# waicool20/BoofCV

Measured on AMD Instinct MI355X. Metric: 1080p frames/sec detect+describe+associate, higher is better.
Workload: dtype f32 detect / f64 describe / associate: fp16 MFMA candidate filter + exact fp64 re-score; 1 GPU; batch of 256 1920x1080 GrayF32 per GPU: Fast-Hessian detect + SURF-64 (stable) describe + greedy L2 associate with the next frame; batch_per_gpu=256, width=1920, height=1080, ranks_seen=1

## Files before the change

boofcv_amd/build.py:

```python
import glob
import os
import subprocess
import sys

HERE = os.path.dirname(os.path.abspath(__file__))
CSRC = os.path.join(HERE, "csrc")
LIB = os.path.join(HERE, "libboofhip.so")
LIB_EXPERIMENTS = os.path.join(HERE, "libboofhip_exp.so")
ARCH = "gfx950"

FLAGS = ["-O3", "-std=c++17", "-fPIC", "-ffp-contract=off", "-fhip-fp32-correctly-rounded-divide-sqrt", "-fno-fast-math",
         "-Wall", "-Wno-unused-function", "-Wno-unused-result"]


def sources():
    return sorted(glob.glob(os.path.join(CSRC, "*.hip"))) + sorted(glob.glob(os.path.join(CSRC, "*.cpp")))


def common_deps():
    return glob.glob(os.path.join(CSRC, "*.h")) + [os.path.join(HERE, "..", "include", "boofhip.h"), os.path.abspath(__file__)]


def needs_build(lib=LIB):
    if not os.path.exists(lib):
        return True
    t = os.path.getmtime(lib)
    return any(os.path.getmtime(d) > t for d in sources() + common_deps())


def build(force=False, verbose=False, experiments=False):
    lib = LIB_EXPERIMENTS if experiments else LIB
    extra = []
    if experiments and os.environ.get("BHIP_EXP_DEFS"):
        extra = os.environ["BHIP_EXP_DEFS"].split()
        lib = os.path.join(HERE, "libboofhip_exp_%s.so" % os.environ.get("BHIP_EXP_TAG", "variant"))
        force = True
    if not force and not needs_build(lib):
        return lib
    hipcc = os.environ.get("HIPCC", "/opt/rocm/bin/hipcc")
    objs = []
    objdir = os.path.join(HERE, ("build_exp_" + os.environ.get("BHIP_EXP_TAG", "variant")) if extra else "build_exp" if experiments else "build")
    os.makedirs(objdir, exist_ok=True)
    procs = []
    newest = max(os.path.getmtime(d) for d in common_deps())
    for src in sources():
        obj = os.path.join(objdir, os.path.basename(src) + ".o")
        objs.append(obj)
        if not force and os.path.exists(obj) and os.path.getmtime(obj) > max(newest, os.path.getmtime(src)):
            continue
        cmd = [hipcc, "--offload-arch=" + ARCH] + FLAGS + (["-DBHIP_EXPERIMENTS"] if experiments else []) + extra + ["-c", src, "-o", obj]
        if src.endswith(".cpp"):
            cmd.insert(1, "-x")
            cmd.insert(2, "hip")
        if verbose:
            print(" ".join(cmd), file=sys.stderr)
        procs.append((src, subprocess.Popen(cmd, stdout=subprocess.PIPE, stderr=subprocess.STDOUT)))
    for src, p in procs:
        out, _ = p.communicate()
        if p.returncode != 0:
            raise RuntimeError("hipcc failed on %s:\n%s" % (src, out.decode(errors="replace")))
        if verbose and out:
            print(out.decode(errors="replace"), file=sys.stderr)
    cmd = [hipcc, "--offload-arch=" + ARCH, "-shared", "-fPIC", "-o", lib] + objs
    subprocess.check_call(cmd)
    return lib


if __name__ == "__main__":
    print(build(force="--force" in sys.argv, verbose=True, experiments="--experiments" in sys.argv))
```

boofcv_amd/csrc/cabi.h:

```cpp
#pragma once
#include "common.h"
#include <cmath>
#include <cfloat>
#include <algorithm>
#include <atomic>
#include <memory>
#include <mutex>
#include <unordered_map>
#include <unordered_set>

#pragma GCC visibility push(hidden)

struct CtxScratch {
	DevBuf in0, in1, out0, out1, tmp0, tmp1;
	DevBuf work, assocCol, nmsBitmap, nmsPrefix, nmsPos, ipTmp, ipKernel, fast, disparity, distortMap, templ, flow, threshold;
	long long flowPixels = 0;
	DevBuf thresholdTaps;
	int thresholdTapsRadius = 0;
	AssocMfmaWork mfma;
	int assocExactOnly = -1;
};
inline CtxScratch* scratchOf(bhip_ctx* ctx);

struct bhip_ctx_full : bhip_ctx {
	CtxScratch scratch;
};
inline CtxScratch* scratchOf(bhip_ctx* ctx) { return &static_cast<bhip_ctx_full*>(ctx)->scratch; }

using OrphanFn = void (*)(void* child, bhip_ctx* ctx);
struct HandleRegistry {
	std::mutex m;
	std::unordered_set<bhip_ctx*> ctxs;
	std::unordered_map<void*, OrphanFn> children;
	std::atomic<bool> exiting{false};
};
HandleRegistry& registry();

template <class Dev>
struct CtxChild : Dev {
	using Device = Dev;
	bhip_ctx* ctx = nullptr;
	void onRelease() {}
};
template <class X>
void releaseDevice(X* x) {
	if (!x->ctx) return;
	(void)hipSetDevice(x->ctx->device);
	(void)hipStreamSynchronize(x->ctx->stream);
	x->onRelease();
	static_cast<typename X::Device&>(*x) = typename X::Device();
	x->ctx = nullptr;
}
template <class X>
void orphanIfOn(void* child, bhip_ctx* ctx) {
	if (static_cast<X*>(child)->ctx == ctx) releaseDevice(static_cast<X*>(child));
}
template <class X, class Build>
int createChild(bhip_ctx* ctx, X** out, Build build) {
	HandleRegistry& R = registry();
	std::lock_guard<std::mutex> lock(R.m);
	if (!ctx || !R.ctxs.count(ctx)) return BHIP_ERR_INVALID;
	std::unique_ptr<X> x;
	BHIP_TRY(build(x));
	R.children.emplace(x.get(), &orphanIfOn<X>);
	*out = x.release();
	return BHIP_OK;
}
template <class X>
int destroyChild(X* x) {
	if (!x) return BHIP_OK;
	HandleRegistry& R = registry();
	std::lock_guard<std::mutex> lock(R.m);
	if (R.exiting) return BHIP_OK;
	auto it = R.children.find(x);
	if (it == R.children.end() || it->second != &orphanIfOn<X>) return BHIP_ERR_INVALID;
	R.children.erase(it);
	releaseDevice(x);
	delete x;
	return BHIP_OK;
}

#define CHECK_CTX(ctx)                                   \
	do {                                                 \
		if (!(ctx)) return BHIP_ERR_INVALID;             \
		BHIP_HIP((ctx), hipSetDevice((ctx)->device));    \
	} while (0)

template <class T>
struct HostImg {
	T* data;
	int start, stride, width, height;
	static constexpr int batch = 1;
};

#define CHECK_IMG(ctx, v)                                                                                         \
	do {                                                                                                          \
		if (!(v).data || (v).width <= 0 || (v).height <= 0 || (v).batch <= 0 || (v).stride < (v).width)          \
			return bhip_fail((ctx), BHIP_ERR_INVALID, "bad image");                                               \
	} while (0)

template <class T>
int upload(bhip_ctx* ctx, T* dev, int pitch, const T* in, int start, int stride, int w, int h, hipStream_t st) {
	if (pitch == w && stride == w) BHIP_HIP(ctx, hipMemcpyAsync(dev, in + start, sizeof(T) * w * h, hipMemcpyHostToDevice, st));
	else BHIP_HIP(ctx, hipMemcpy2DAsync(dev, sizeof(T) * pitch, in + start, sizeof(T) * stride, sizeof(T) * w, h, hipMemcpyHostToDevice, st));
	return BHIP_OK;
}
template <class T>
int download(bhip_ctx* ctx, T* out, int start, int stride, const T* dev, int pitch, int w, int h, hipStream_t st) {
	if (pitch == w && stride == w) BHIP_HIP(ctx, hipMemcpyAsync(out + start, dev, sizeof(T) * w * h, hipMemcpyDeviceToHost, st));
	else BHIP_HIP(ctx, hipMemcpy2DAsync(out + start, sizeof(T) * stride, dev, sizeof(T) * pitch, sizeof(T) * w, h, hipMemcpyDeviceToHost, st));
	return BHIP_OK;
}

template <class T>
int stageIn(bhip_ctx* ctx, DevBuf& slot, HostImg<T> h, int pitch, DevImg<std::remove_const_t<T>>& dev, bool copy = true) {
	using E = std::remove_const_t<T>;
	BHIP_TRY(slot.reserve(ctx, (size_t)pitch * h.height * sizeof(E)));
	dev = bhip_img_over<E>(slot, pitch, h.width, h.height, 1);
	return copy ? upload<E>(ctx, dev.data, pitch, h.data, h.start, h.stride, h.width, h.height, ctx->stream) : BHIP_OK;
}
template <class T>
int stageOut(bhip_ctx* ctx, HostImg<T> h, DevImg<T> dev) {
	return download<T>(ctx, h.data, h.start, h.stride, dev.data, dev.stride, h.width, h.height, ctx->stream);
}
inline int pitch4(int w) { return (w + 3) & ~3; }

template <class TI, class TO, class Run>
int hostInOut(bhip_ctx* ctx, HostImg<const TI> in, HostImg<TO> out, bool pitched, bool keepOut, const char* argError, Run run) {
	CHECK_CTX(ctx);
	CHECK_IMG(ctx, in);
	CHECK_IMG(ctx, out);
	if (argError) return bhip_fail(ctx, BHIP_ERR_INVALID, argError);
	CtxScratch* sc = scratchOf(ctx);
	DevImg<TI> din;
	DevImg<TO> dout;
	BHIP_TRY(stageIn(ctx, sc->in0, in, pitched ? pitch4(in.width) : in.width, din));
	BHIP_TRY(stageIn(ctx, sc->out0, out, pitched ? pitch4(out.width) : out.width, dout, keepOut));
	BHIP_TRY(run(din, dout));
	BHIP_TRY(stageOut(ctx, out, dout));
	return bhip_ctx_synchronize(ctx);
}

int nonmaxDevice(bhip_ctx* ctx, DevImg<const float> img, int radius, float threshold, int border, int16_t* dev_xy, int cap, int* dev_n,
				 bool minimum = false);
template <class T>
int cornerImpl(bhip_ctx* ctx, bool weighted, int kind, int radius, float kappa, DevImg<const T> dx, DevImg<const T> dy, DevImg<float> intensity);
template <class T> struct PyrTraits;
template <> struct PyrTraits<float> {
	using Kernel = float;
	static constexpr bool fusedLayer = true;
	static constexpr bool clearLayer0 = true;
	static constexpr const char* copyTag = "pyramid_copy";
	static constexpr double copyBytes = 8.0;
};
template <> struct PyrTraits<uint8_t> {
	using Kernel = int32_t;
	static constexpr bool fusedLayer = false;
	static constexpr bool clearLayer0 = false;
	static constexpr const char* copyTag = "pyramid_copy_u8";
	static constexpr double copyBytes = 2.0;
};
template <class T>
int pyramidImpl(bhip_ctx* ctx, const typename PyrTraits<T>::Kernel* kernel, int kw, const int* scales, int n, DevImg<const T> in, T* out,
				bool layer0Present = false);
bool briefPatchOk(const int32_t* samplePoints, int nSamples, int radius);
int gaussianImpl(bhip_ctx* ctx, double sigma, int radius, DevImg<const float> in, DevImg<float> out);

#pragma GCC visibility pop
```

boofcv_amd/csrc/cabi.hip:

```cpp
#include "cabi.h"

HandleRegistry& registry() {
	static HandleRegistry* r = [] {
		HandleRegistry* p = new HandleRegistry();
		atexit([] { registry().exiting = true; });
		return p;
	}();
	return *r;
}

static int ctxCreate(int device, void* stream, bool useGiven, bhip_ctx** out) {
	if (!out) return BHIP_ERR_INVALID;
	*out = nullptr;
	int count = 0;
	if (hipGetDeviceCount(&count) != hipSuccess || count <= 0) return BHIP_ERR_HIP;
	if (device < 0 || device >= count) return BHIP_ERR_INVALID;
	if (hipSetDevice(device) != hipSuccess) return BHIP_ERR_HIP;
	std::unique_ptr<bhip_ctx_full> ctx(new (std::nothrow) bhip_ctx_full());
	if (!ctx) return BHIP_ERR_NOMEM;
	ctx->device = device;
	if (useGiven) {
		ctx->stream = (hipStream_t)stream;
	} else {
		if (hipStreamCreateWithFlags(&ctx->ownedStream.h, hipStreamNonBlocking) != hipSuccess) return BHIP_ERR_HIP;
		ctx->stream = ctx->ownedStream;
	}
	if (ctx->hostScratch.reserve(ctx.get(), 1 << 20) != BHIP_OK) return BHIP_ERR_HIP;
	HandleRegistry& R = registry();
	std::lock_guard<std::mutex> lock(R.m);
	R.ctxs.insert(ctx.get());
	*out = ctx.release();
	return BHIP_OK;
}

struct FhLevelPlan {
	DetectLevelParams p;
	int level;
};
struct FhOctavePlan {
	int skip, w, h, nlevels;
	int sizes[BHIP_MAX_LEVELS];
	std::vector<FhLevelPlan> mids;
	bool fused = false, fixed = false;
	int shareFrom[BHIP_MAX_LEVELS];
	bool onDemand[BHIP_MAX_LEVELS];
	int exportSlot[BHIP_MAX_LEVELS];
	int nexport = 0;
	size_t intenOff = 0, expOff = 0;
	long long intenImageStride = 0, expImageStride = 0;
};

struct FhDetector {
	bhip_fh_cfg cfg;
	int W = 0, H = 0, batch = 0, cap = 0;
	bool plannedInt = false;
	std::vector<FhOctavePlan> plan;
	int bitmapWords = 0;
	DevBuf inten, bitmap, prefix, cand, sorted, count, selKey, selIdx, selLevels;
	bool nBest() const { return cfg.maxFeaturesPerScale > 0; }
	std::vector<int> counts;
	long long total = 0;

	static bool unfusedOnly() { return bhip_env_flag("BHIP_DETECT_UNFUSED"); }
	int makePlan(bhip_ctx* ctx, int width, int height) {
		plan.clear();
		if (cfg.numberScalesPerOctave > BHIP_MAX_LEVELS || cfg.numberScalesPerOctave < 1) return bhip_fail(ctx, BHIP_ERR_UNSUPPORTED, "numberScalesPerOctave out of range");
		if (cfg.extractRadius < 1) return bhip_fail(ctx, BHIP_ERR_INVALID, "Search radius must be >= 1");
		if (cfg.initialSampleSize < 1 || cfg.initialSize < 3) return bhip_fail(ctx, BHIP_ERR_INVALID, "bad sample size / initial size");
		if (width >= 32768 || height >= 32768) return bhip_fail(ctx, BHIP_ERR_UNSUPPORTED, "image too large for Point2D_I16");
		int skip = cfg.initialSampleSize, sizeStep = cfg.scaleStepSize, octaveSize = cfg.initialSize;
		unsigned int bits = 0;
		const int step = cfg.extractRadius + 1;
		for (int octave = 0; octave < cfg.numberOfOctaves; octave++) {
			FhOctavePlan o;
			o.nlevels = cfg.numberScalesPerOctave;
			for (int i = 0; i < o.nlevels; i++) o.sizes[i] = octaveSize + i * sizeStep;
			const int maxSize = o.sizes[o.nlevels - 1];
			if (maxSize > width || maxSize > height) break;
			o.skip = skip;
			o.w = width / skip;
			o.h = height / skip;
			for (int i = 2; i < o.nlevels; i++) {
				FhLevelPlan m;
				m.level = i - 1;
				DetectLevelParams& p = m.p;
				p.skip = skip; p.w = o.w; p.h = o.h;
				p.sizeLower = o.sizes[m.level - 1]; p.sizeMid = o.sizes[m.level]; p.sizeUpper = o.sizes[m.level + 1];
				p.border = p.sizeMid / (2 * skip);
				const int rw = p.w - 2 * p.border, rh = p.h - 2 * p.border;
				p.nbx = rw > 0 ? (rw + step - 1) / step : 0;
				p.nby = rh > 0 ? (rh + step - 1) / step : 0;
				p.bitBase = bits;
				bits += (unsigned)p.nbx * (unsigned)p.nby;
				o.mids.push_back(m);
			}
			plan.push_back(o);
			skip += skip;
			octaveSize += sizeStep;
			sizeStep += sizeStep;
		}
		bitmapWords = (int)((bits + 31) / 32) + 1;
		return BHIP_OK;
	}

	static bool noShare() { return bhip_env_flag("BHIP_DETECT_NOSHARE"); }
	static bool denseOuter() { return bhip_env_flag("BHIP_DETECT_DENSE"); }
	void planExecution() {
		for (auto& o : plan) {
			int ftx, fty, flds;
			o.fused = !unfusedOnly() && !nBest() && !o.mids.empty() && bhip_fused_plan(o.skip, o.nlevels, o.sizes, cfg.extractRadius, &ftx, &fty, &flds);
			o.fixed = o.fused && bhip_fused_is_fixed(o.skip, o.nlevels, o.sizes, cfg.extractRadius);
			if (plannedInt && !o.fixed) o.fused = false;
			o.nexport = 0;
			for (int i = 0; i < BHIP_MAX_LEVELS; i++) { o.shareFrom[i] = -1; o.exportSlot[i] = -1; o.onDemand[i] = false; }
		}
		const bool sparseOuter = !denseOuter() && !nBest();
		for (size_t k = 0; k < plan.size(); k++) {
			FhOctavePlan& c = plan[k];
			if (k > 0 && !noShare()) shareLevels(c, plan[k - 1]);
			if (!c.fused && sparseOuter && c.nlevels >= 3)
				for (int i : {0, c.nlevels - 1})
					if (c.shareFrom[i] < 0) c.onDemand[i] = true;
		}
	}
	void shareLevels(FhOctavePlan& c, FhOctavePlan& p) {
		{
			if (c.fused || c.skip != 2 * p.skip) return;
			if (p.fused && !p.fixed) return;
			for (int i = 0; i < c.nlevels; i++) {
				const int size = c.sizes[i];
				if (size % 3 != 0 || size % 2 != 1) continue;
				for (int j = 0; j < p.nlevels; j++) {
					if (p.sizes[j] != size) continue;
					if (!p.fused && p.onDemand[j]) break;
					if (p.fused) {
						if (p.exportSlot[j] < 0) {
							if (p.nexport >= 2) break;
							p.exportSlot[j] = p.nexport++;
						}
					}
					c.shareFrom[i] = j;
					break;
				}
			}
		}
	}

	template <class T>
	int prepare(bhip_ctx* ctx, int width, int height, int batch_) {
		constexpr bool isInt = std::is_same<T, int32_t>::value;
		if (width != W || height != H || plannedInt != isInt) { BHIP_TRY(makePlan(ctx, width, height)); plannedInt = isInt; planExecution(); }
		W = width; H = height; batch = batch_;
		if (cap == 0) cap = BHIP_SURF_INITIAL_CAPACITY;
		return allocate(ctx);
	}
	int allocate(bhip_ctx* ctx) {
		size_t intenFloats = 0;
		for (size_t k = 0; k < plan.size(); k++) {
			FhOctavePlan& o = plan[k];
			if (!o.fused) {
				o.intenImageStride = (long long)o.nlevels * o.w * o.h;
				o.intenOff = intenFloats;
				intenFloats += (size_t)o.intenImageStride * batch;
			}
		}
		BHIP_TRY(inten.reserve(ctx, intenFloats * 4 + 16));
		BHIP_TRY(bitmap.reserve(ctx, (size_t)bitmapWords * 4 * batch));
		BHIP_TRY(prefix.reserve(ctx, (size_t)bitmapWords * 4 * batch));
		BHIP_TRY(cand.reserve(ctx, (size_t)cap * sizeof(KeyPoint) * batch));
		BHIP_TRY(sorted.reserve(ctx, (size_t)cap * sizeof(KeyPoint) * batch));
		BHIP_TRY(count.reserve(ctx, (size_t)batch * 4 * 2));
		if (nBest()) {
			size_t nlv = 0;
			for (auto& o : plan) nlv += o.mids.size();
			BHIP_TRY(selKey.reserve(ctx, (size_t)cap * 4 * batch));
			BHIP_TRY(selIdx.reserve(ctx, (size_t)cap * 4 * batch));
			BHIP_TRY(selLevels.reserve(ctx, std::max<size_t>(nlv, 1) * 4 * 2 * batch));
		}
		return BHIP_OK;
	}

	DevImg<float> level(const FhOctavePlan& o, int l) const { return {inten.as<float>() + o.intenOff + (size_t)l * o.w * o.h, o.intenImageStride, o.w, o.w, o.h, batch}; }
	template <class T>
	int runStandAlone(bhip_ctx* ctx, DevImg<const T> ii, size_t k0, size_t k1) {
		std::vector<HessLevelSource> from((k1 - k0) * BHIP_MAX_LEVELS);
		std::vector<HessOctave> octs;
		std::vector<NmsLevelArgs> nms;
		for (size_t k = k0; k < k1; k++) {
			const FhOctavePlan& o = plan[k];
			HessLevelSource* f = &from[(k - k0) * BHIP_MAX_LEVELS];
			for (int i = 0; i < o.nlevels; i++) {
				f[i] = HessLevelSource{nullptr, 0, 0, 1, 0};
				const int j = o.shareFrom[i];
				if (j < 0 || k == 0) continue;
				const FhOctavePlan& p = plan[k - 1];
				if (p.fused) f[i] = HessLevelSource{level(o, i).data, o.intenImageStride, o.w, 1, 1};
				else f[i] = HessLevelSource{level(p, j).data, p.intenImageStride, p.w, 2, 0};
			}
			unsigned int skipMask = 0;
			for (int i = 0; i < o.nlevels; i++)
				if (o.onDemand[i]) skipMask |= 1u << i;
			octs.push_back(HessOctave{o.skip, o.nlevels, o.sizes, level(o, 0), (long long)o.w * o.h, f, skipMask});
			auto held = [&](int l) { DevImg<const float> v = level(o, l); if (o.onDemand[l]) v.data = nullptr; return v; };
			for (auto& m : o.mids) nms.push_back(NmsLevelArgs{held(m.level - 1), level(o, m.level), held(m.level + 1), m.p});
		}
		BHIP_TRY(bhip_launch_hessian_octaves(ctx, ii, (int)octs.size(), octs.data()));
		if (nBest()) {
			for (auto& a : nms)
				BHIP_TRY(bhip_launch_nms_scalespace(ctx, a.lower, a.mid, a.upper, a.p, cfg.extractRadius, cfg.detectThreshold, bitmap.as<unsigned int>(), bitmapWords,
													cand.as<KeyPoint>(), count.as<int>(), cap, true, ii));
			return BHIP_OK;
		}
		return bhip_launch_nms_scalespace_levels(ctx, (int)nms.size(), nms.data(), cfg.extractRadius, cfg.detectThreshold, bitmap.as<unsigned int>(), bitmapWords,
												 cand.as<KeyPoint>(), count.as<int>(), cap, ii);
	}
	template <class T>
	int run(bhip_ctx* ctx, DevImg<const T> ii) {
		for (int attempt = 0; attempt < 8; attempt++) {
			BHIP_HIP(ctx, hipMemsetAsync(bitmap.p, 0, (size_t)bitmapWords * 4 * batch, ctx->stream));
			BHIP_HIP(ctx, hipMemsetAsync(count.p, 0, (size_t)batch * 4 * 2, ctx->stream));
			for (size_t k = 0; k < plan.size(); k++) {
				FhOctavePlan& o = plan[k];
				if (o.fused) {
					DetectLevelParams mp[BHIP_MAX_LEVELS];
					int ml[BHIP_MAX_LEVELS];
					for (size_t q = 0; q < o.mids.size(); q++) { mp[q] = o.mids[q].p; ml[q] = o.mids[q].level; }
					FusedExport ex{0, {0, 0}, nullptr, 0, 0, 0, {0, 0}};
					if (o.nexport > 0 && k + 1 < plan.size()) {
						const FhOctavePlan& c = plan[k + 1];
						ex.n = o.nexport;
						for (int j = 0; j < o.nlevels; j++) if (o.exportSlot[j] >= 0) ex.level[o.exportSlot[j]] = j;
						ex.out = level(c, 0).data; ex.w = c.w; ex.h = c.h; ex.imageStride = c.intenImageStride;
						for (int i = 0; i < c.nlevels; i++) {
							const int j = c.shareFrom[i];
							if (j >= 0 && o.exportSlot[j] >= 0) ex.slotOffset[o.exportSlot[j]] = (long long)i * c.w * c.h;
						}
					}
					BHIP_TRY(bhip_launch_detect_fused(ctx, ii, o.skip, o.nlevels, o.sizes, (int)o.mids.size(), mp, ml, cfg.extractRadius,
													  cfg.detectThreshold, bitmap.as<unsigned int>(), bitmapWords, cand.as<KeyPoint>(), count.as<int>(), cap,
													  ex.n > 0 ? &ex : nullptr));
					continue;
				}
				size_t end = k + 1;
				while (!nBest() && end < plan.size() && !plan[end].fused) end++;
				BHIP_TRY(runStandAlone(ctx, ii, k, end));
				k = end - 1;
			}
			BHIP_TRY(bhip_launch_word_prefix(ctx, bitmap.as<unsigned int>(), bitmapWords, batch, prefix.as<unsigned int>(), count.as<int>() + batch));
			counts.resize(batch);
			if ((size_t)batch * 4 <= (1u << 20)) {
				BHIP_HIP(ctx, hipMemcpyAsync(ctx->hostScratch.p, count.p, (size_t)batch * 4, hipMemcpyDeviceToHost, ctx->stream));
				BHIP_HIP(ctx, hipStreamSynchronize(ctx->stream));
				memcpy(counts.data(), ctx->hostScratch.p, (size_t)batch * 4);
			} else {
				BHIP_HIP(ctx, hipMemcpyAsync(counts.data(), count.p, (size_t)batch * 4, hipMemcpyDeviceToHost, ctx->stream));
				BHIP_HIP(ctx, hipStreamSynchronize(ctx->stream));
			}
			int maxCount = 0;
			total = 0;
			for (int c : counts) { maxCount = std::max(maxCount, c); total += c; }
			if (maxCount <= cap) {
				BHIP_TRY(bhip_launch_rank_scatter(ctx, bitmap.as<unsigned int>(), bitmapWords, prefix.as<unsigned int>(), cand.as<KeyPoint>(), count.as<int>(),
												  cap, batch, sorted.as<KeyPoint>()));
				if (nBest()) BHIP_TRY(selectNBest(ctx));
				return BHIP_OK;
			}
			cap = maxCount + maxCount / 4 + 64;
			BHIP_TRY(allocate(ctx));
		}
		return bhip_fail(ctx, BHIP_ERR_CAPACITY, "key point list kept overflowing");
	}
	int selectNBest(bhip_ctx* ctx) {
		int nlv = 0;
		for (auto& o : plan) nlv += (int)o.mids.size();
		int* levelStart = selLevels.as<int>();
		int* levelCount = levelStart + (size_t)std::max(nlv, 1) * batch;
		int li = 0;
		for (auto& o : plan)
			for (auto& m : o.mids) {
				BHIP_TRY(bhip_launch_select_nbest(ctx, level(o, m.level - 1), level(o, m.level), level(o, m.level + 1), m.p, cfg.extractRadius,
												  cfg.maxFeaturesPerScale, bitmap.as<unsigned int>(), prefix.as<unsigned int>(), bitmapWords, sorted.as<KeyPoint>(),
												  cap, selKey.as<float>(), selIdx.as<int>(), cand.as<KeyPoint>(), levelStart, levelCount, li, nlv));
				li++;
			}
		BHIP_TRY(bhip_launch_compact_levels(ctx, cand.as<KeyPoint>(), cap, levelStart, levelCount, nlv, batch, sorted.as<KeyPoint>(), count.as<int>()));
		BHIP_HIP(ctx, hipMemcpyAsync(counts.data(), count.p, (size_t)batch * 4, hipMemcpyDeviceToHost, ctx->stream));
		BHIP_HIP(ctx, hipStreamSynchronize(ctx->stream));
		total = 0;
		for (int c : counts) total += c;
		return BHIP_OK;
	}
};

struct SurfDevice {
	FhDetector det;
	DevBuf tabBuf, inBuf, iiBuf, startBuf, angBuf, descBuf, whiteBuf, xysBuf, tmpKp, tmpAng, tmpDesc, tmpWhite, permBuf;
	DevBuf briefTab, wordsBuf;
	PinnedBuf startsPinned;
	std::unique_ptr<bhip_surf> worker;
	HipStream copyStream;
	const int* briefBorrow = nullptr;
};

struct bhip_surf : CtxChild<SurfDevice> {
	void onRelease() {
		if (copyStream) (void)hipStreamSynchronize(copyStream);
		haveResult = false;
	}
	int stable = 1;
	bhip_surf_cfg sd;
	bhip_ori_cfg ori;
	SurfTables tables;
	std::vector<int> starts;
	int W = 0, H = 0, batch = 0;
	bool haveResult = false;
	bool iiInt = false;
	int planarBands = 0;
	int dofOut() const { return tables.dof * (planarBands > 0 ? planarBands : 1); }
	DescPlanar planar() const {
		const long long px = (long long)W * H;
		return planarBands > 0 ? DescPlanar{iiBuf.as<float>() + px, px * (1 + planarBands), px, planarBands} : DescPlanar{};
	}
	const DevBuf* iiOwner = nullptr; int iiFirst = 0;
	bool brief = false;
	int briefRadius = 0, briefPoints = 0, briefWords = 0;
	bool briefPatch = false;
	const int* briefSample() const { return briefBorrow ? briefBorrow : briefTab.as<int>(); }
	const int* briefCompare() const { return briefSample() + briefCompareOff; }
	size_t briefCompareOff = 0;
};

template <class F>
static int withIntegral(const bhip_surf* s, F f) {
	return s->iiInt ? f(bhip_img_over<const int32_t>(s->iiBuf, s->W, s->W, s->H, s->batch)) : f(bhip_img_over<const float>(s->iiBuf, s->W, s->W, s->H, s->batch));
}
template <class T> struct SurfTraits;
template <> struct SurfTraits<float> { using II = float; };
template <> struct SurfTraits<uint8_t> { using II = int32_t; };
constexpr int GREY = 0;
enum class SurfReturn { SYNCHRONIZED, QUEUED };

static int buildTables(bhip_surf* s) {
	bhip_ctx* ctx = s->ctx;
	SurfTables& t = s->tables;
	memset(&t, 0, sizeof(t));
	const bhip_surf_cfg& c = s->sd;
	const bhip_ori_cfg& o = s->ori;
	if (c.widthLargeGrid < 1 || c.widthSubRegion < 1 || c.widthSample < 1 || c.overLap < 0) return bhip_fail(ctx, BHIP_ERR_INVALID, "bad SURF config");
	if (o.radius < 1 || o.radius > 10) return bhip_fail(ctx, BHIP_ERR_UNSUPPORTED, "orientation radius out of range (1..10 on the GPU)");
	std::vector<double> all;
	auto push = [&](const std::vector<double>& v) { size_t off = all.size(); all.insert(all.end(), v.begin(), v.end()); return off; };
	t.oriStable = s->stable;
	t.oriRadius = o.radius;
	t.oriWidth = 2 * o.radius + 1;
	t.oriKernelWidth = o.sampleWidth;
	t.oriHasWeights = o.weightSigma != 0 ? 1 : 0;
	t.oriPeriod = o.samplePeriod;
	t.oriWindow = o.windowSize;
	t.oriRadiusToScale = o.objectRadiusToScale;
	size_t offOri = 0, offSub = 0, offGrid = 0, offFast = 0;
	if (t.oriHasWeights) offOri = push(bhip_gaussian2d_f64(o.weightSigma, o.radius));
	t.stable = s->stable;
	t.widthLargeGrid = c.widthLargeGrid; t.widthSubRegion = c.widthSubRegion; t.widthSample = c.widthSample; t.overLap = c.overLap;
	t.dof = c.widthLargeGrid * c.widthLargeGrid * 4;
	const int regionSize = c.widthLargeGrid * c.widthSubRegion;
	if (s->stable) {
		std::vector<double> wg = bhip_gaussian_width(c.sigmaLargeGrid, c.widthLargeGrid);
		std::vector<double> ws = bhip_gaussian_width(c.sigmaSubRegion, c.widthSubRegion + 2 * c.overLap);
		const int gw = c.widthLargeGrid, sw = c.widthSubRegion + 2 * c.overLap;
		double div = wg[(size_t)(gw / 2) * gw + gw / 2];
		for (double& v : wg) v /= div;
		div = ws[(size_t)(sw / 2) * sw + sw / 2];
		for (double& v : ws) v /= div;
		offGrid = push(wg);
		offSub = push(ws);
		t.radiusDescriptor = regionSize / 2 + c.overLap;
	} else {
		const int radius = regionSize / 2;
		std::vector<double> w = bhip_gaussian_width(c.weightSigma, radius * 2);
		if ((int)w.size() != regionSize * regionSize) return bhip_fail(ctx, BHIP_ERR_INVALID, "Weighting kernel has an unexpected size");
		const double div = w[(size_t)radius * (radius * 2) + radius];
		for (double& v : w) v /= div;
		offFast = push(w);
		t.radiusDescriptor = regionSize / 2;
	}
	BHIP_TRY(s->tabBuf.reserve(ctx, all.size() * 8 + 8));
	BHIP_HIP(ctx, hipMemcpyAsync(s->tabBuf.p, all.data(), all.size() * 8, hipMemcpyHostToDevice, ctx->stream));
	BHIP_HIP(ctx, hipStreamSynchronize(ctx->stream));
	const double* base = s->tabBuf.as<double>();
	t.oriWeights = t.oriHasWeights ? base + offOri : nullptr;
	t.weightSub = s->stable ? base + offSub : nullptr;
	t.weightGrid = s->stable ? base + offGrid : nullptr;
	t.weightFast = s->stable ? nullptr : base + offFast;
	return BHIP_OK;
}

template <class T>
static int surfRun(bhip_surf* s, DevImg<const T> in, int bands, SurfReturn ret) {
	using II = typename SurfTraits<T>::II;
	bhip_ctx* ctx = s->ctx;
	const int W = in.width, H = in.height, batch = bands > 0 ? 1 : in.batch;
	const long long px = (long long)W * H;
	s->haveResult = false;
	BHIP_TRY(s->det.prepare<II>(ctx, W, H, batch));
	if (!s->iiOwner) BHIP_TRY(s->iiBuf.reserve(ctx, (size_t)px * 4 * in.batch));
	II* iiBase = s->iiOwner ? s->iiOwner->as<II>() + px * s->iiFirst : s->iiBuf.as<II>();
	s->W = W; s->H = H; s->batch = batch;
	s->iiInt = std::is_same<II, int32_t>::value; s->planarBands = bands;
	const DevImg<II> iiAll{iiBase, px, W, W, H, in.batch};
	if constexpr (std::is_same<T, uint8_t>::value) BHIP_TRY(bhip_launch_integral_u8(ctx, in, iiAll));
	else BHIP_TRY(bhip_launch_integral(ctx, in, iiAll));
	const DevImg<const II> ii{iiBase, px, W, W, H, batch};
	BHIP_TRY(s->det.run(ctx, ii));
	s->starts.assign(batch + 1, 0);
	for (int i = 0; i < batch; i++) s->starts[i + 1] = s->starts[i] + s->det.counts[i];
	const long long total = s->det.total;
	if (total > 0x7fffffffLL) return bhip_fail(ctx, BHIP_ERR_CAPACITY, "more than 2^31 key points in one batch");
	BHIP_TRY(s->startBuf.reserve(ctx, (size_t)(batch + 1) * 4));
	{
		const size_t need = (size_t)(batch + 1) * 4;
		if (need > s->startsPinned.cap) BHIP_TRY(s->startsPinned.reserve(ctx, need * 2));
		memcpy(s->startsPinned.p, s->starts.data(), need);
		BHIP_HIP(ctx, hipMemcpyAsync(s->startBuf.p, s->startsPinned.p, need, hipMemcpyHostToDevice, ctx->stream));
	}
	if (s->brief) {
		if (bands > 0) return bhip_fail(ctx, BHIP_ERR_UNSUPPORTED, "BRIEF runs on single-band frames");
		BHIP_TRY(s->angBuf.reserve(ctx, (size_t)std::max<long long>(total, 1) * 8));
		BHIP_TRY(s->whiteBuf.reserve(ctx, (size_t)std::max<long long>(total, 1)));
		BHIP_TRY(s->wordsBuf.reserve(ctx, (size_t)std::max<long long>(total, 1) * 4 * s->briefWords));
		if (total > 0) {
			BHIP_HIP(ctx, hipMemsetAsync(s->angBuf.p, 0, (size_t)total * 8, ctx->stream));
			BHIP_HIP(ctx, hipMemsetAsync(s->whiteBuf.p, 0, (size_t)total, ctx->stream));
			int maxCount = 0;
			for (int c : s->det.counts) maxCount = std::max(maxCount, c);
			BHIP_TRY(bhip_launch_brief(ctx, in, s->briefRadius, s->briefPoints, s->briefSample(), s->briefCompare(), (const double*)s->det.sorted.p, (int)total,
									   s->wordsBuf.as<int>(), s->startBuf.as<int>(), maxCount, (int)(sizeof(KeyPoint) / 8),
									   (long long)s->det.cap * (long long)(sizeof(KeyPoint) / 8), s->briefPatch));
		}
		BHIP_HIP(ctx, hipStreamSynchronize(ctx->stream));
		s->haveResult = true;
		return BHIP_OK;
	}
	const int dof = s->dofOut();
	BHIP_TRY(s->angBuf.reserve(ctx, (size_t)std::max<long long>(total, 1) * 8));
	BHIP_TRY(s->descBuf.reserve(ctx, (size_t)std::max<long long>(total, 1) * 8 * dof));
	BHIP_TRY(s->whiteBuf.reserve(ctx, (size_t)std::max<long long>(total, 1)));
	const int* perm = nullptr;
	{
#ifdef BHIP_EXPERIMENTS
		const bool noOrder = bhip_env_flag("BHIP_DESCRIBE_NOORDER");
#else
		const bool noOrder = false;
#endif
		int maxCount = 0;
		for (int c : s->det.counts) maxCount = std::max(maxCount, c);
		if (!noOrder && total > 0) {
			BHIP_TRY(s->permBuf.reserve(ctx, (size_t)total * 4 + (size_t)batch * 64 * 4));
			int* hist = s->permBuf.as<int>() + total;
			BHIP_TRY(bhip_launch_kp_spatial_order(ctx, s->det.sorted.as<KeyPoint>(), s->det.cap, s->startBuf.as<int>(), batch, maxCount, W, H, hist,
												  s->permBuf.as<int>()));
			perm = s->permBuf.as<int>();
		}
	}
	BHIP_TRY(bhip_launch_describe_ex(ctx, ii, s->det.sorted.as<KeyPoint>(), s->det.cap, s->startBuf.as<int>(), 0, total, s->tables, nullptr,
									 s->angBuf.as<double>(), s->descBuf.as<double>(), s->whiteBuf.as<uint8_t>(), perm, s->planar()));
	if (ret == SurfReturn::SYNCHRONIZED) BHIP_HIP(ctx, hipStreamSynchronize(ctx->stream));
	s->haveResult = true;
	return BHIP_OK;
}

static int surfCreateUnregistered(bhip_ctx* ctx, const bhip_fh_cfg* fh, const bhip_surf_cfg* surf, const bhip_ori_cfg* ori, int stable,
								  std::unique_ptr<bhip_surf>& out);

static int growKeep(bhip_ctx* ctx, DevBuf& b, size_t bytes, size_t keep) {
	if (bytes <= b.cap) return BHIP_OK;
	DevBuf n;
	BHIP_TRY(n.reserve(ctx, bytes + bytes / 4));
	if (b.p && keep) BHIP_HIP(ctx, hipMemcpyAsync(n.p, b.p, keep, hipMemcpyDeviceToDevice, ctx->stream));
	if (b.p) BHIP_HIP(ctx, hipStreamSynchronize(ctx->stream));
	b = std::move(n);
	return BHIP_OK;
}

#define SURF_CHUNK 32

template <class T, class Upload>
static int surfRunChunked(bhip_surf* s, int width, int height, int batch, Upload upload, bool* done) {
	using II = typename SurfTraits<T>::II;
	bhip_ctx* ctx = s->ctx;
	*done = false;
	int chunk = SURF_CHUNK;
	{ const char* e = getenv("BHIP_SURF_CHUNK"); if (e && atoi(e) > 0) chunk = atoi(e); }
	if (batch < 2 * chunk) return BHIP_OK;
	if (!s->worker) {
		BHIP_TRY(surfCreateUnregistered(ctx, &s->det.cfg, &s->sd, &s->ori, s->stable, s->worker));
		if (s->brief) {
			bhip_surf* w0 = s->worker.get();
			w0->brief = true; w0->briefRadius = s->briefRadius; w0->briefPoints = s->briefPoints; w0->briefWords = s->briefWords;
			w0->briefBorrow = s->briefTab.as<int>(); w0->briefCompareOff = s->briefCompareOff; w0->briefPatch = s->briefPatch;
		}
		BHIP_HIP(ctx, hipStreamCreateWithFlags(&s->copyStream.h, hipStreamNonBlocking));
	}
	bhip_surf* w = s->worker.get();
	const size_t px = (size_t)width * height;
	s->haveResult = false;
	BHIP_TRY(s->det.prepare<II>(ctx, width, height, batch));
	BHIP_TRY(s->iiBuf.reserve(ctx, px * 4 * batch));
	const int nchunks = (batch + chunk - 1) / chunk;
	std::vector<HipEvent> events(nchunks + 1);
	HipEvent& ev = events[nchunks];
	HipEvent* arrived = events.data();
	BHIP_HIP(ctx, hipEventCreateWithFlags(&ev.h, hipEventDisableTiming));
	BHIP_HIP(ctx, hipEventRecord(ev, ctx->stream));
	BHIP_HIP(ctx, hipStreamWaitEvent(s->copyStream, ev, 0));
	int status = BHIP_OK;
	for (int c = 0; c < nchunks && status == BHIP_OK; c++) {
		const int a = c * chunk, n = std::min(chunk, batch - a);
		for (int i = a; i < a + n && status == BHIP_OK; i++) status = upload(i, s->inBuf.as<T>() + px * i, s->copyStream);
		if (status == BHIP_OK && (hipEventCreateWithFlags(&arrived[c].h, hipEventDisableTiming) != hipSuccess || hipEventRecord(arrived[c], s->copyStream) != hipSuccess))
			status = bhip_fail(ctx, BHIP_ERR_HIP, "event");
	}
	const int dof = s->tables.dof;
	s->starts.assign(batch + 1, 0);
	s->det.counts.assign(batch, 0);
	long long total = 0;
	bool fits = true;
	for (int c = 0; c < nchunks && status == BHIP_OK && fits; c++) {
		const int a = c * chunk, n = std::min(chunk, batch - a);
		if (hipStreamWaitEvent(ctx->stream, arrived[c], 0) != hipSuccess) { status = bhip_fail(ctx, BHIP_ERR_HIP, "wait"); break; }
		w->iiOwner = &s->iiBuf; w->iiFirst = a;
		status = surfRun(w, DevImg<const T>{s->inBuf.as<T>() + px * a, (long long)px, width, width, height, n}, GREY, SurfReturn::SYNCHRONIZED);
		if (status != BHIP_OK) break;
		int maxCount = 0;
		for (int i = 0; i < n; i++) maxCount = std::max(maxCount, w->det.counts[i]);
		if (maxCount > s->det.cap) { fits = false; break; }
		const long long ct = w->det.total;
		status = growKeep(ctx, s->angBuf, (size_t)std::max<long long>(total + ct, 1) * 8, (size_t)total * 8);
		if (status == BHIP_OK && !s->brief) status = growKeep(ctx, s->descBuf, (size_t)std::max<long long>(total + ct, 1) * 8 * dof, (size_t)total * 8 * dof);
		if (status == BHIP_OK) status = growKeep(ctx, s->whiteBuf, (size_t)std::max<long long>(total + ct, 1), (size_t)total);
		if (status == BHIP_OK && s->brief) status = growKeep(ctx, s->wordsBuf, (size_t)std::max<long long>(total + ct, 1) * 4 * s->briefWords, (size_t)total * 4 * s->briefWords);
		if (status != BHIP_OK) break;
		hipError_t e = hipSuccess;
		if (maxCount > 0)
			e = hipMemcpy2DAsync(s->det.sorted.as<KeyPoint>() + (long long)a * s->det.cap, (size_t)s->det.cap * sizeof(KeyPoint), w->det.sorted.p,
								 (size_t)w->det.cap * sizeof(KeyPoint), (size_t)maxCount * sizeof(KeyPoint), n, hipMemcpyDeviceToDevice, ctx->stream);
		if (e == hipSuccess && ct > 0) e = hipMemcpyAsync(s->angBuf.as<double>() + total, w->angBuf.p, (size_t)ct * 8, hipMemcpyDeviceToDevice, ctx->stream);
		if (e == hipSuccess && ct > 0 && !s->brief) e = hipMemcpyAsync(s->descBuf.as<double>() + total * dof, w->descBuf.p, (size_t)ct * 8 * dof, hipMemcpyDeviceToDevice, ctx->stream);
		if (e == hipSuccess && ct > 0 && s->brief) e = hipMemcpyAsync(s->wordsBuf.as<int>() + total * s->briefWords, w->wordsBuf.p, (size_t)ct * 4 * s->briefWords, hipMemcpyDeviceToDevice, ctx->stream);
		if (e == hipSuccess && ct > 0) e = hipMemcpyAsync(s->whiteBuf.as<uint8_t>() + total, w->whiteBuf.p, (size_t)ct, hipMemcpyDeviceToDevice, ctx->stream);
		if (e != hipSuccess) { status = bhip_fail(ctx, BHIP_ERR_HIP, hipGetErrorString(e)); break; }
		for (int i = 0; i < n; i++) {
			s->det.counts[a + i] = w->det.counts[i];
			s->starts[a + i + 1] = s->starts[a + i] + w->det.counts[i];
		}
		total += ct;
	}
	(void)hipStreamSynchronize(s->copyStream);
	(void)hipStreamSynchronize(ctx->stream);
	w->iiOwner = nullptr;
	if (status != BHIP_OK) return status;
	if (!fits) {
		*done = true;
		return surfRun(s, bhip_img_over<const T>(s->inBuf, width, width, height, batch), GREY, SurfReturn::SYNCHRONIZED);
	}
	if (total > 0x7fffffffLL) return bhip_fail(ctx, BHIP_ERR_CAPACITY, "more than 2^31 key points in one batch");
	s->det.total = total;
	s->W = width; s->H = height; s->batch = batch;
	s->iiInt = std::is_same<II, int32_t>::value;
	s->planarBands = 0;
	BHIP_TRY(s->startBuf.reserve(ctx, (size_t)(batch + 1) * 4));
	BHIP_HIP(ctx, hipMemcpyAsync(s->startBuf.p, s->starts.data(), (size_t)(batch + 1) * 4, hipMemcpyHostToDevice, ctx->stream));
	BHIP_HIP(ctx, hipStreamSynchronize(ctx->stream));
	s->haveResult = true;
	*done = true;
	return BHIP_OK;
}

static int surfCreateUnregistered(bhip_ctx* ctx, const bhip_fh_cfg* fh, const bhip_surf_cfg* surf, const bhip_ori_cfg* ori, int stable,
								  std::unique_ptr<bhip_surf>& out) {
	std::unique_ptr<bhip_surf> s(new (std::nothrow) bhip_surf());
	if (!s) return bhip_fail(ctx, BHIP_ERR_NOMEM, "out of host memory");
	s->ctx = ctx;
	s->stable = stable ? 1 : 0;
	if (fh) s->det.cfg = *fh; else bhip_fh_cfg_default(&s->det.cfg);
	if (surf) s->sd = *surf; else bhip_surf_cfg_default(&s->sd);
	if (ori) s->ori = *ori; else bhip_ori_cfg_default(&s->ori, s->stable);
	BHIP_TRY(buildTables(s.get()));
	out = std::move(s);
	return BHIP_OK;
}

template <class T>
static int surfDetectHost(bhip_surf* s, const T* const* img, const int* startIndex, const int* stride, int width, int height, int batch) {
	if (!s) return BHIP_ERR_INVALID;
	bhip_ctx* ctx = s->ctx;
	CHECK_CTX(ctx);
	if (!img || width <= 0 || height <= 0 || batch <= 0) return bhip_fail(ctx, BHIP_ERR_INVALID, "bad image batch");
	const size_t px = (size_t)width * height;
	BHIP_TRY(s->inBuf.reserve(ctx, px * sizeof(T) * batch));
	for (int i = 0; i < batch; i++)
		if (!img[i] || (stride ? stride[i] : width) < width) return bhip_fail(ctx, BHIP_ERR_INVALID, "bad image (null or stride < width)");
	auto put = [&](int i, T* dst, hipStream_t st) {
		return upload(ctx, dst, width, img[i], startIndex ? startIndex[i] : 0, stride ? stride[i] : width, width, height, st);
	};
	bool done = false;
	BHIP_TRY(surfRunChunked<T>(s, width, height, batch, put, &done));
	if (done) return BHIP_OK;
	for (int i = 0; i < batch; i++) BHIP_TRY(put(i, s->inBuf.as<T>() + px * i, ctx->stream));
	return surfRun(s, bhip_img_over<const T>(s->inBuf, width, width, height, batch), GREY, SurfReturn::SYNCHRONIZED);
}

template <class Match>
static int assocSurf(bhip_surf* s, int count, const int* srcImage, const int* dstImage, int* pairs, double* fit, Match match) {
	bhip_ctx* ctx = s->ctx;
	if (!s->haveResult) return bhip_fail(ctx, BHIP_ERR_INVALID, "no detect result");
	if (count < 0 || (count > 0 && (!srcImage || !dstImage || !pairs || !fit))) return bhip_fail(ctx, BHIP_ERR_INVALID, "bad problem table");
	if (count == 0) return BHIP_OK;
	const long long total = s->det.total;
	std::vector<long long> so(count), doff(count);
	std::vector<int> ns(count), nd(count);
	std::vector<char> used(s->batch, 0);
	for (int p = 0; p < count; p++) {
		const int a = srcImage[p], b = dstImage[p];
		if (a < 0 || a >= s->batch || b < 0 || b >= s->batch) return bhip_fail(ctx, BHIP_ERR_INVALID, "image index outside the last batch");
		if (used[a]) return bhip_fail(ctx, BHIP_ERR_INVALID, "an image may be the source of one problem per call");
		used[a] = 1;
		so[p] = s->starts[a]; ns[p] = s->det.counts[a];
		doff[p] = s->starts[b]; nd[p] = s->det.counts[b];
	}
	if (total == 0) return BHIP_OK;
	CtxScratch* sc = scratchOf(ctx);
	BHIP_TRY(sc->out0.reserve(ctx, (size_t)total * 4));
	BHIP_TRY(sc->out1.reserve(ctx, (size_t)total * 8));
	BHIP_HIP(ctx, hipMemsetAsync(sc->out0.p, 0xff, (size_t)total * 4, ctx->stream));
	BHIP_HIP(ctx, hipMemsetAsync(sc->out1.p, 0, (size_t)total * 8, ctx->stream));
	BHIP_TRY(match(so.data(), ns.data(), doff.data(), nd.data(), sc->out0.as<int>(), sc->out1.as<double>()));
	BHIP_HIP(ctx, hipMemcpyAsync(pairs, sc->out0.p, (size_t)total * 4, hipMemcpyDeviceToHost, ctx->stream));
	BHIP_HIP(ctx, hipMemcpyAsync(fit, sc->out1.p, (size_t)total * 8, hipMemcpyDeviceToHost, ctx->stream));
	return bhip_ctx_synchronize(ctx);
}

template <class T>
static int fhDetect(bhip_ctx* ctx, const bhip_fh_cfg* cfg, HostImg<const T> hin, double* xy_scale, int cap, int* n) {
	CHECK_CTX(ctx);
	CHECK_IMG(ctx, hin);
	if (!n || cap < 0 || (cap > 0 && !xy_scale)) return bhip_fail(ctx, BHIP_ERR_INVALID, "bad output");
	*n = 0;
	FhDetector det;
	if (cfg) det.cfg = *cfg; else bhip_fh_cfg_default(&det.cfg);
	CtxScratch* sc = scratchOf(ctx);
	DevImg<T> din;
	int status = stageIn(ctx, sc->in0, hin, hin.width, din);
	if (status == BHIP_OK) status = det.prepare<T>(ctx, hin.width, hin.height, 1);
	if (status == BHIP_OK) status = det.run(ctx, DevImg<const T>(din));
	if (status == BHIP_OK) {
		*n = det.counts[0];
		const int ncopy = std::min(*n, cap);
		if (ncopy > 0) {
			std::vector<KeyPoint> kps(ncopy);
			hipError_t e = hipMemcpyAsync(kps.data(), det.sorted.p, (size_t)ncopy * sizeof(KeyPoint), hipMemcpyDeviceToHost, ctx->stream);
			if (e == hipSuccess) e = hipStreamSynchronize(ctx->stream);
			if (e != hipSuccess) status = bhip_fail(ctx, BHIP_ERR_HIP, hipGetErrorString(e));
			else for (int i = 0; i < ncopy; i++) { xy_scale[3 * i] = kps[i].x; xy_scale[3 * i + 1] = kps[i].y; xy_scale[3 * i + 2] = kps[i].scale; }
		}
	}
	(void)hipStreamSynchronize(ctx->stream);
	return status;
}

extern "C" {

const char* bhip_version(void) { return "boofhip 0.1 (gfx950)"; }

void bhip_fh_cfg_default(bhip_fh_cfg* c) {
	c->detectThreshold = 1; c->extractRadius = 2; c->maxFeaturesPerScale = -1; c->initialSampleSize = 1; c->initialSize = 9;
	c->numberScalesPerOctave = 4; c->numberOfOctaves = 4; c->scaleStepSize = 6;
}
void bhip_klt_cfg_default(bhip_klt_cfg* c) {
	c->forbiddenBorder = 0; c->maxPerPixelError = 25; c->maxIterations = 15; c->minDeterminant = 0.001f; c->minPositionDelta = 0.01f;
}
void bhip_bg_basic_cfg_default(bhip_bg_basic_cfg* c) { c->learnRate = 0.05f; c->threshold = 0; c->unknownValue = 0; }
void bhip_bg_gaussian_cfg_default(bhip_bg_gaussian_cfg* c) {
	c->learnRate = 0.05f; c->threshold = 0; c->initialVariance = FLT_TRUE_MIN; c->minimumDifference = 0; c->unknownValue = 0;
}
void bhip_bg_gmm_cfg_default(bhip_bg_gmm_cfg* c) {
	c->learningPeriod = 1000.0f; c->initialVariance = 400; c->decayCoefient = 0.005f; c->maxDistance = 3; c->numberOfGaussian = 5; c->significantWeight = 0.01f;
	c->unknownValue = 0;
}
void bhip_disparity_bm_cfg_default(bhip_disparity_bm_cfg* c) {
	c->minDisparity = 0; c->rangeDisparity = 100; c->regionRadiusX = 3; c->regionRadiusY = 3; c->maxPerPixelError = 0; c->validateRtoL = 1; c->texture = 0.15;
}
void bhip_surf_cfg_default(bhip_surf_cfg* c) {
	c->widthLargeGrid = 4; c->widthSubRegion = 5; c->widthSample = 3; c->weightSigma = 4.5; c->overLap = 2; c->sigmaLargeGrid = 2.5;
	c->sigmaSubRegion = 2.5;
}
void bhip_ori_cfg_default(bhip_ori_cfg* c, int stable) {
	c->objectRadiusToScale = 1.0 / 2.0;
	c->weightSigma = -1;
	c->sampleWidth = 6;
	if (stable) { c->samplePeriod = 0.65; c->windowSize = M_PI / 3.0; c->radius = 8; }
	else { c->samplePeriod = 1; c->windowSize = 0; c->radius = 6; }
}

int bhip_ctx_create(int device, bhip_ctx** out) { return ctxCreate(device, nullptr, false, out); }
int bhip_ctx_create_on_stream(int device, void* hip_stream, bhip_ctx** out) { return ctxCreate(device, hip_stream, true, out); }
int bhip_ctx_destroy(bhip_ctx* c) {
	if (!c) return BHIP_OK;
	HandleRegistry& R = registry();
	std::lock_guard<std::mutex> lock(R.m);
	if (R.exiting) return BHIP_OK;
	if (!R.ctxs.count(c)) return BHIP_ERR_INVALID;
	R.ctxs.erase(c);
	(void)hipSetDevice(c->device);
	(void)hipStreamSynchronize(c->stream);
	for (auto& child : R.children) child.second(child.first, c);
	delete static_cast<bhip_ctx_full*>(c);
	return BHIP_OK;
}
int bhip_ctx_synchronize(bhip_ctx* ctx) {
	if (!ctx) return BHIP_ERR_INVALID;
	BHIP_HIP(ctx, hipStreamSynchronize(ctx->stream));
	return BHIP_OK;
}
const char* bhip_last_error(bhip_ctx* ctx) { return ctx ? ctx->error.c_str() : "null context"; }
int bhip_host_alloc(bhip_ctx* ctx, long long bytes, uint8_t** host_mem) {
	if (!ctx || !host_mem) return BHIP_ERR_INVALID;
	*host_mem = nullptr;
	if (bytes <= 0) return bhip_fail(ctx, BHIP_ERR_INVALID, "bhip_host_alloc: size must be positive");
	BHIP_HIP(ctx, hipSetDevice(ctx->device));
	void* p = nullptr;
	const hipError_t e = hipHostMalloc(&p, (size_t)bytes, hipHostMallocDefault);
	if (e != hipSuccess) { (void)hipGetLastError(); return bhip_fail(ctx, BHIP_ERR_NOMEM, "bhip_host_alloc: out of page-locked memory"); }
	*host_mem = (uint8_t*)p;
	return BHIP_OK;
}
int bhip_host_free(void* host_mem) {
	if (!host_mem) return BHIP_OK;
	if (registry().exiting) return BHIP_OK;
	return hipHostFree(host_mem) == hipSuccess ? BHIP_OK : BHIP_ERR_HIP;
}

int bhip_surf_create(bhip_ctx* ctx, const bhip_fh_cfg* fh, const bhip_surf_cfg* surf, const bhip_ori_cfg* ori, int stable, bhip_surf** out) {
	return createChild(ctx, out, [&](std::unique_ptr<bhip_surf>& s) -> int {
		CHECK_CTX(ctx);
		if (!out) return bhip_fail(ctx, BHIP_ERR_INVALID, "null output");
		*out = nullptr;
		return surfCreateUnregistered(ctx, fh, surf, ori, stable, s);
	});
}

int bhip_surf_destroy(bhip_surf* s) { return destroyChild(s); }

int bhip_surf_dof(bhip_surf* s) { return s ? s->dofOut() : 0; }

int bhip_surf_detect_dev_f32(bhip_surf* s, const float* dev_images, long long imageStride, int stride, int width, int height, int batch) {
	if (!s) return BHIP_ERR_INVALID;
	bhip_ctx* ctx = s->ctx;
	CHECK_CTX(ctx);
	if (!dev_images || width <= 0 || height <= 0 || batch <= 0 || stride < width) return bhip_fail(ctx, BHIP_ERR_INVALID, "bad image batch");
	return surfRun(s, DevImg<const float>{dev_images, imageStride, stride, width, height, batch}, GREY, SurfReturn::QUEUED);
}

int bhip_surf_detect_f32(bhip_surf* s, const float* const* img, const int* startIndex, const int* stride, int width, int height, int batch) {
	return surfDetectHost(s, img, startIndex, stride, width, height, batch);
}

int bhip_surf_detect_planar_f32(bhip_surf* s, const float* const* bands, int numBands, int startIndex, int stride, int width, int height) {
	if (!s) return BHIP_ERR_INVALID;
	bhip_ctx* ctx = s->ctx;
	CHECK_CTX(ctx);
	if (!bands || numBands < 1 || numBands > 16 || width <= 0 || height <= 0 || stride < width) return bhip_fail(ctx, BHIP_ERR_INVALID, "bad planar image");
	const size_t px = (size_t)width * height;
	BHIP_TRY(s->inBuf.reserve(ctx, px * 4 * (1 + numBands)));
	for (int b = 0; b < numBands; b++) {
		if (!bands[b]) return bhip_fail(ctx, BHIP_ERR_INVALID, "null band");
		BHIP_TRY(upload(ctx, s->inBuf.as<float>() + px * (1 + b), width, bands[b], startIndex, stride, width, height, ctx->stream));
	}
	BHIP_TRY(bhip_launch_planar_average(ctx, s->inBuf.as<float>() + px, (long long)px, numBands, (long long)px, s->inBuf.as<float>()));
	return surfRun(s, bhip_img_over<const float>(s->inBuf, width, width, height, 1 + numBands), numBands, SurfReturn::SYNCHRONIZED);
}

int bhip_surf_detect_u8(bhip_surf* s, const uint8_t* const* img, const int* startIndex, const int* stride, int width, int height, int batch) {
	return surfDetectHost(s, img, startIndex, stride, width, height, batch);
}

int bhip_surf_count(bhip_surf* s, int image, int* n) {
	if (!s || !n) return BHIP_ERR_INVALID;
	if (!s->haveResult || image < 0 || image >= s->batch) return bhip_fail(s->ctx, BHIP_ERR_INVALID, "no detect result for that image");
	*n = s->det.counts[image];
	return BHIP_OK;
}
int bhip_surf_counts(bhip_surf* s, int* counts, int capacity) {
	if (!s || !counts) return BHIP_ERR_INVALID;
	if (!s->haveResult || capacity < s->batch) return bhip_fail(s->ctx, BHIP_ERR_INVALID, "no detect result / counts array too short");
	for (int i = 0; i < s->batch; i++) counts[i] = s->det.counts[i];
	return BHIP_OK;
}
int bhip_surf_total(bhip_surf* s, long long* n) {
	if (!s || !n) return BHIP_ERR_INVALID;
	*n = s->haveResult ? s->det.total : 0;
	return BHIP_OK;
}

int bhip_surf_fetch(bhip_surf* s, int image, double* xy_scale, double* angle, uint8_t* white, double* desc) {
	if (!s) return BHIP_ERR_INVALID;
	bhip_ctx* ctx = s->ctx;
	CHECK_CTX(ctx);
	if (!s->haveResult || image < 0 || image >= s->batch) return bhip_fail(ctx, BHIP_ERR_INVALID, "no detect result for that image");
	if (desc && s->brief) return bhip_fail(ctx, BHIP_ERR_INVALID, "this object describes with BRIEF: fetch the words with bhip_surf_fetch_brief");
	const int n = s->det.counts[image];
	if (n == 0) return BHIP_OK;
	const long long off = s->starts[image];
	const int dof = s->dofOut();
	std::vector<KeyPoint> kps;
	if (xy_scale) {
		kps.resize(n);
		BHIP_HIP(ctx, hipMemcpyAsync(kps.data(), s->det.sorted.as<KeyPoint>() + (long long)image * s->det.cap, (size_t)n * sizeof(KeyPoint),
									 hipMemcpyDeviceToHost, ctx->stream));
	}
	if (angle) BHIP_HIP(ctx, hipMemcpyAsync(angle, s->angBuf.as<double>() + off, (size_t)n * 8, hipMemcpyDeviceToHost, ctx->stream));
	if (white) BHIP_HIP(ctx, hipMemcpyAsync(white, s->whiteBuf.as<uint8_t>() + off, (size_t)n, hipMemcpyDeviceToHost, ctx->stream));
	if (desc) BHIP_HIP(ctx, hipMemcpyAsync(desc, s->descBuf.as<double>() + off * dof, (size_t)n * 8 * dof, hipMemcpyDeviceToHost, ctx->stream));
	BHIP_HIP(ctx, hipStreamSynchronize(ctx->stream));
	if (xy_scale)
		for (int i = 0; i < n; i++) { xy_scale[3 * i] = kps[i].x; xy_scale[3 * i + 1] = kps[i].y; xy_scale[3 * i + 2] = kps[i].scale; }
	return BHIP_OK;
}

int bhip_surf_fetch_all(bhip_surf* s, double* xy_scale, double* angle, uint8_t* white, double* desc) {
	if (!s) return BHIP_ERR_INVALID;
	bhip_ctx* ctx = s->ctx;
	CHECK_CTX(ctx);
	if (!s->haveResult) return bhip_fail(ctx, BHIP_ERR_INVALID, "no detect result");
	if (desc && s->brief) return bhip_fail(ctx, BHIP_ERR_INVALID, "this object describes with BRIEF: fetch the words with bhip_surf_fetch_brief");
	const long long total = s->det.total;
	if (total == 0) return BHIP_OK;
	const int dof = s->dofOut();
	if (xy_scale) {
		BHIP_TRY(s->xysBuf.reserve(ctx, (size_t)total * 24));
		for (int i = 0; i < s->batch; i++) {
			const int n = s->det.counts[i];
			if (n > 0)
				BHIP_HIP(ctx, hipMemcpy2DAsync((char*)s->xysBuf.p + (size_t)s->starts[i] * 24, 24, s->det.sorted.as<KeyPoint>() + (long long)i * s->det.cap,
											   sizeof(KeyPoint), 24, (size_t)n, hipMemcpyDeviceToDevice, ctx->stream));
		}
		BHIP_HIP(ctx, hipMemcpyAsync(xy_scale, s->xysBuf.p, (size_t)total * 24, hipMemcpyDeviceToHost, ctx->stream));
	}
	if (angle) BHIP_HIP(ctx, hipMemcpyAsync(angle, s->angBuf.p, (size_t)total * 8, hipMemcpyDeviceToHost, ctx->stream));
	if (white) BHIP_HIP(ctx, hipMemcpyAsync(white, s->whiteBuf.p, (size_t)total, hipMemcpyDeviceToHost, ctx->stream));
	if (desc) BHIP_HIP(ctx, hipMemcpyAsync(desc, s->descBuf.p, (size_t)total * 8 * dof, hipMemcpyDeviceToHost, ctx->stream));
	BHIP_HIP(ctx, hipStreamSynchronize(ctx->stream));
	return BHIP_OK;
}

int bhip_surf_dev_view(bhip_surf* s, int image, const double** dev_desc, const double** dev_xy_scale, const uint8_t** dev_white, int* n) {
	if (!s) return BHIP_ERR_INVALID;
	if (!s->haveResult || image < 0 || image >= s->batch) return bhip_fail(s->ctx, BHIP_ERR_INVALID, "no detect result for that image");
	const long long off = s->starts[image];
	if (dev_desc) *dev_desc = s->descBuf.as<double>() + off * s->dofOut();
	if (dev_xy_scale) *dev_xy_scale = (const double*)(s->det.sorted.as<KeyPoint>() + (long long)image * s->det.cap);
	if (dev_white) *dev_white = s->whiteBuf.as<uint8_t>() + off;
	if (n) *n = s->det.counts[image];
	return BHIP_OK;
}

int bhip_surf_create_brief(bhip_ctx* ctx, const bhip_fh_cfg* fh, int radius, int numPoints, const int32_t* samplePoints, const int32_t* compare, bhip_surf** out) {
	return createChild(ctx, out, [&](std::unique_ptr<bhip_surf>& s) -> int {
		CHECK_CTX(ctx);
		if (!out) return bhip_fail(ctx, BHIP_ERR_INVALID, "null output");
		*out = nullptr;
		if (radius < 0 || numPoints <= 0 || !samplePoints || !compare) return bhip_fail(ctx, BHIP_ERR_INVALID, "bad BRIEF definition");
		int maxIdx = 0;
		for (int i = 0; i < 2 * numPoints; i++) {
			if (compare[i] < 0) return bhip_fail(ctx, BHIP_ERR_INVALID, "negative sample index");
			maxIdx = std::max(maxIdx, compare[i]);
		}
		BHIP_TRY(surfCreateUnregistered(ctx, fh, nullptr, nullptr, 0, s));
		s->brief = true;
		s->briefRadius = radius; s->briefPoints = numPoints; s->briefWords = (numPoints + 31) / 32;
		const size_t nSample = (size_t)(maxIdx + 1) * 2, nCompare = (size_t)numPoints * 2;
		s->briefCompareOff = nSample;
		s->briefPatch = briefPatchOk(samplePoints, maxIdx + 1, radius);
		BHIP_TRY(s->briefTab.reserve(ctx, (nSample + nCompare) * 4));
		if (hipMemcpy(s->briefTab.p, samplePoints, nSample * 4, hipMemcpyHostToDevice) != hipSuccess) return bhip_fail(ctx, BHIP_ERR_HIP, "BRIEF table upload");
		if (hipMemcpy(s->briefTab.as<int>() + nSample, compare, nCompare * 4, hipMemcpyHostToDevice) != hipSuccess) return bhip_fail(ctx, BHIP_ERR_HIP, "BRIEF table upload");
		return BHIP_OK;
	});
}

int bhip_surf_fetch_brief(bhip_surf* s, int image, int32_t* words) {
	if (!s || !words) return BHIP_ERR_INVALID;
	bhip_ctx* ctx = s->ctx;
	CHECK_CTX(ctx);
	if (!s->brief) return bhip_fail(ctx, BHIP_ERR_INVALID, "not a BRIEF detect+describe object");
	if (!s->haveResult || image < -1 || image >= s->batch) return bhip_fail(ctx, BHIP_ERR_INVALID, "no detect result for that image");
	const long long off = image < 0 ? 0 : s->starts[image];
	const long long n = image < 0 ? s->det.total : s->det.counts[image];
	if (n == 0) return BHIP_OK;
	BHIP_HIP(ctx, hipMemcpyAsync(words, s->wordsBuf.as<int>() + off * s->briefWords, (size_t)n * 4 * s->briefWords, hipMemcpyDeviceToHost, ctx->stream));
	BHIP_HIP(ctx, hipStreamSynchronize(ctx->stream));
	return BHIP_OK;
}
int bhip_surf_dev_view_brief(bhip_surf* s, int image, const int32_t** dev_words, int* words, int* n) {
	if (!s) return BHIP_ERR_INVALID;
	if (!s->brief) return bhip_fail(s->ctx, BHIP_ERR_INVALID, "not a BRIEF detect+describe object");
	if (!s->haveResult || image < 0 || image >= s->batch) return bhip_fail(s->ctx, BHIP_ERR_INVALID, "no detect result for that image");
	if (dev_words) *dev_words = s->wordsBuf.as<int>() + (long long)s->starts[image] * s->briefWords;
	if (words) *words = s->briefWords;
	if (n) *n = s->det.counts[image];
	return BHIP_OK;
}

int bhip_surf_fetch_integral(bhip_surf* s, int image, float* out) {
	if (!s || !out) return BHIP_ERR_INVALID;
	bhip_ctx* ctx = s->ctx;
	CHECK_CTX(ctx);
	if (!s->haveResult || image < 0 || image >= s->batch) return bhip_fail(ctx, BHIP_ERR_INVALID, "no detect result for that image");
	BHIP_HIP(ctx, hipMemcpyAsync(out, s->iiBuf.as<float>() + (long long)image * s->W * s->H, (size_t)s->W * s->H * 4, hipMemcpyDeviceToHost, ctx->stream));
	BHIP_HIP(ctx, hipStreamSynchronize(ctx->stream));
	return BHIP_OK;
}

int bhip_surf_describe_points(bhip_surf* s, int image, const double* xy_scale, int n, double* angle, uint8_t* white, double* desc) {
	if (!s) return BHIP_ERR_INVALID;
	bhip_ctx* ctx = s->ctx;
	CHECK_CTX(ctx);
	if (!s->haveResult || image < 0 || image >= s->batch) return bhip_fail(ctx, BHIP_ERR_INVALID, "no detect result for that image");
	if (s->brief) return bhip_fail(ctx, BHIP_ERR_INVALID, "this object describes with BRIEF");
	if (n < 0 || (n > 0 && !xy_scale)) return bhip_fail(ctx, BHIP_ERR_INVALID, "bad point list");
	if (n == 0) return BHIP_OK;
	std::vector<KeyPoint> kps(n);
	for (int i = 0; i < n; i++) { kps[i].x = xy_scale[3 * i]; kps[i].y = xy_scale[3 * i + 1]; kps[i].scale = xy_scale[3 * i + 2]; kps[i].key = 0; kps[i].pad = 0; }
	const int dof = s->dofOut();
	BHIP_TRY(s->tmpKp.reserve(ctx, (size_t)n * sizeof(KeyPoint)));
	BHIP_TRY(s->tmpAng.reserve(ctx, (size_t)n * 8));
	BHIP_TRY(s->tmpDesc.reserve(ctx, (size_t)n * 8 * dof));
	BHIP_TRY(s->tmpWhite.reserve(ctx, (size_t)n));
	BHIP_HIP(ctx, hipMemcpyAsync(s->tmpKp.p, kps.data(), (size_t)n * sizeof(KeyPoint), hipMemcpyHostToDevice, ctx->stream));
	BHIP_TRY(withIntegral(s, [&](auto ii) {
		return bhip_launch_describe_ex(ctx, ii, s->tmpKp.as<KeyPoint>(), 0, nullptr, image, n, s->tables, nullptr, s->tmpAng.as<double>(),
									   s->tmpDesc.as<double>(), s->tmpWhite.as<uint8_t>(), nullptr, s->planar());
	}));
	if (angle) BHIP_HIP(ctx, hipMemcpyAsync(angle, s->tmpAng.p, (size_t)n * 8, hipMemcpyDeviceToHost, ctx->stream));
	if (white) BHIP_HIP(ctx, hipMemcpyAsync(white, s->tmpWhite.p, (size_t)n, hipMemcpyDeviceToHost, ctx->stream));
	if (desc) BHIP_HIP(ctx, hipMemcpyAsync(desc, s->tmpDesc.p, (size_t)n * 8 * dof, hipMemcpyDeviceToHost, ctx->stream));
	BHIP_HIP(ctx, hipStreamSynchronize(ctx->stream));
	return BHIP_OK;
}

int bhip_fh_detect_f32(bhip_ctx* ctx, const bhip_fh_cfg* cfg, const float* ii, int iiStart, int iiStride, int width, int height, double* xy_scale,
					   int cap, int* n) {
	return fhDetect<float>(ctx, cfg, {ii, iiStart, iiStride, width, height}, xy_scale, cap, n);
}
int bhip_fh_detect_s32(bhip_ctx* ctx, const bhip_fh_cfg* cfg, const int32_t* ii, int iiStart, int iiStride, int width, int height, double* xy_scale,
					   int cap, int* n) {
	return fhDetect<int32_t>(ctx, cfg, {ii, iiStart, iiStride, width, height}, xy_scale, cap, n);
}

int bhip_assoc_hamming_surf(bhip_surf* s, int count, const int* srcImage, const int* dstImage, double maxErr, int backwards, int* pairs, double* fit) {
	if (!s) return BHIP_ERR_INVALID;
	bhip_ctx* ctx = s->ctx;
	CHECK_CTX(ctx);
	if (!s->brief) return bhip_fail(ctx, BHIP_ERR_INVALID, "not a BRIEF detect+describe object");
	const int32_t* W = s->wordsBuf.as<int32_t>();
	return assocSurf(s, count, srcImage, dstImage, pairs, fit, [&](const long long* so, const int* ns, const long long* doff, const int* nd, int* dp, double* df) {
		return bhip_assoc_hamming_batched(ctx, W, W, s->briefWords, count, so, ns, doff, nd, maxErr, backwards, dp, df, scratchOf(ctx)->work);
	});
}

int bhip_assoc_l2_surf(bhip_surf* s, int count, const int* srcImage, const int* dstImage, double maxErr, int backwards, int* pairs, double* fit) {
	if (!s) return BHIP_ERR_INVALID;
	bhip_ctx* ctx = s->ctx;
	CHECK_CTX(ctx);
	if (s->brief) return bhip_fail(ctx, BHIP_ERR_INVALID, "this object describes with BRIEF: use bhip_assoc_hamming_surf");
	const double* D = s->descBuf.as<double>();
	return assocSurf(s, count, srcImage, dstImage, pairs, fit, [&](const long long* so, const int* ns, const long long* doff, const int* nd, int* dp, double* df) {
		return bhip_assoc_l2_dev_batched(ctx, D, D, s->dofOut(), count, so, ns, doff, nd, maxErr, backwards, dp, df);
	});
}

}
```

boofcv_amd/csrc/common.h:

```cpp
#pragma once
#include <hip/hip_runtime.h>
#include <cstdint>
#include <cstdio>
#include <cstring>
#include <cstdlib>
#include <string>
#include <type_traits>
#include <vector>
#include <new>
#include <utility>
#include "../../include/boofhip.h"

#define BHIP_WAVE 64

static inline bool bhip_env_flag(const char* name) {
	const char* e = getenv(name);
	return e && e[0] == '1';
}
#ifdef BHIP_EXPERIMENTS
#define BHIP_ABLATE(P, bits) ((P).ablate & (bits))
#else
#define BHIP_ABLATE(P, bits) 0
#endif


template <class H, hipError_t (*Destroy)(H)>
struct HipHandle {
	H h = nullptr;
	HipHandle() = default;
	HipHandle(HipHandle&& o) noexcept : h(o.h) { o.h = nullptr; }
	HipHandle& operator=(HipHandle&& o) noexcept { std::swap(h, o.h); return *this; }
	~HipHandle() { if (h) (void)Destroy(h); }
	operator H() const { return h; }
};
using HipStream = HipHandle<hipStream_t, hipStreamDestroy>;
using HipEvent = HipHandle<hipEvent_t, hipEventDestroy>;

struct PinnedBuf {
	void* p = nullptr;
	size_t cap = 0;
	PinnedBuf() = default;
	PinnedBuf(PinnedBuf&& o) noexcept : p(o.p), cap(o.cap) { o.p = nullptr; o.cap = 0; }
	PinnedBuf& operator=(PinnedBuf&& o) noexcept { std::swap(p, o.p); std::swap(cap, o.cap); return *this; }
	~PinnedBuf() { if (p) (void)hipHostFree(p); }
	int reserve(bhip_ctx* ctx, size_t bytes);
	template <class T> T* as() const { return (T*)p; }
};

struct ProfRecord {
	const char* tag;
	double algBytes;
	double algFlops;
	HipEvent start, stop;
};

struct bhip_ctx {
	int device = 0;
	hipStream_t stream = nullptr;
	HipStream ownedStream;
	std::string error;
	PinnedBuf hostScratch;
	bool profiling = false;
	std::vector<ProfRecord> profRecords;
	std::vector<HipEvent> eventPool;
	size_t integralLdsAttr = 0;
};

struct ProfScope {
	bhip_ctx* ctx;
	int idx = -1;
	ProfScope(bhip_ctx* c, const char* tag, double algBytes = 0, double algFlops = 0);
	~ProfScope();
};

static inline int bhip_fail(bhip_ctx* ctx, int code, const std::string& msg) {
	if (ctx) ctx->error = msg;
	return code;
}

#define BHIP_HIP(ctx, expr)                                                                                                      \
	do {                                                                                                                         \
		hipError_t _e = (expr);                                                                                                  \
		if (_e != hipSuccess) return bhip_fail((ctx), _e == hipErrorOutOfMemory ? BHIP_ERR_NOMEM : BHIP_ERR_HIP,                 \
											   std::string(#expr) + ": " + hipGetErrorString(_e));                               \
	} while (0)

#define BHIP_TRY(expr)                 \
	do {                               \
		int _s = (expr);               \
		if (_s != BHIP_OK) return _s;  \
	} while (0)

struct DevBuf {
	void* p = nullptr;
	size_t cap = 0;
	DevBuf() = default;
	DevBuf(DevBuf&& o) noexcept : p(o.p), cap(o.cap) { o.p = nullptr; o.cap = 0; }
	DevBuf& operator=(DevBuf&& o) noexcept { std::swap(p, o.p); std::swap(cap, o.cap); return *this; }
	~DevBuf() { if (p) (void)hipFree(p); }
	int reserve(bhip_ctx* ctx, size_t bytes) {
		if (bytes <= cap) return BHIP_OK;
		if (p) { BHIP_HIP(ctx, hipStreamSynchronize(ctx->stream)); BHIP_HIP(ctx, hipFree(p)); p = nullptr; cap = 0; }
		size_t want = bytes + bytes / 8;
		BHIP_HIP(ctx, hipMalloc(&p, want));
		cap = want;
		return BHIP_OK;
	}
	template <class T> T* as() const { return (T*)p; }
};

inline int PinnedBuf::reserve(bhip_ctx* ctx, size_t bytes) {
	if (bytes <= cap) return BHIP_OK;
	if (p) { BHIP_HIP(ctx, hipStreamSynchronize(ctx->stream)); (void)hipHostFree(p); p = nullptr; cap = 0; }
	if (hipHostMalloc(&p, bytes, hipHostMallocDefault) != hipSuccess) { (void)hipGetLastError(); p = nullptr; return bhip_fail(ctx, BHIP_ERR_NOMEM, "page-locked staging buffer"); }
	cap = bytes;
	return BHIP_OK;
}

struct AssocMfmaWork {
	DevBuf Fs, Fd, nrmS, nrmD, probs, blocks, keys, thr, best, args, cand, flags;
};

struct ImgView {
	const float* data;
	long long imageStride;
	int stride;
	int width, height;
};
struct ImgViewW {
	float* data;
	long long imageStride;
	int stride;
	int width, height;
};

template <class T>
struct DevImg {
	T* data;
	long long imageStride;
	int stride, width, height, batch;
	operator DevImg<const T>() const { return {data, imageStride, stride, width, height, batch}; }
};
template <class T>
static inline ImgView bhip_kernel_view(DevImg<const T> v) {
	static_assert(sizeof(T) == 4, "ImgView carries 32-bit elements");
	return {reinterpret_cast<const float*>(v.data), v.imageStride, v.stride, v.width, v.height};
}
template <class T>
static inline DevImg<T> bhip_img_over(const DevBuf& buf, int pitch, int width, int height, int batch) {
	return {buf.as<T>(), (long long)pitch * height, pitch, width, height, batch};
}
template <class T>
static inline DevImg<T> bhip_pyr_layer(T* base, long long total, const int* dims, const long long* offs, int l, int batch) {
	return {base + offs[l], total, dims[2 * l], dims[2 * l], dims[2 * l + 1], batch};
}

#define BHIP_MAX_OCTAVES 8
#define BHIP_MAX_LEVELS 8

struct KeyPoint {
	double x, y, scale;
	unsigned int key;
	unsigned int pad;
};

struct SurfTables {
	int oriStable;
	int oriRadius;
	int oriWidth;
	int oriKernelWidth;
	int oriHasWeights;
	double oriPeriod;
	double oriWindow;
	double oriRadiusToScale;
	const double* oriWeights;
	int stable;
	int widthLargeGrid, widthSubRegion, widthSample, overLap;
	int dof;
	int radiusDescriptor;
	const double* weightSub;
	const double* weightGrid;
	const double* weightFast;
};

std::vector<double> bhip_gaussian2d_f64(double sigma, int radius);
std::vector<double> bhip_gaussian_width(double sigma, int width);
std::vector<float> bhip_gaussian1d_f32(double sigma, int radius);
std::vector<int32_t> bhip_gaussian1d_s32(int radius);

int bhip_launch_integral(bhip_ctx* ctx, DevImg<const float> in, DevImg<float> out);
struct FusedExport {
	int n;
	int level[2];
	float* out;
	int w, h;
	long long imageStride;
	long long slotOffset[2];
};
struct HessLevelSource {
	const float* src;
	long long imageStride;
	int stride;
	int step;
	int inPlace;
};
template <class T>
int bhip_launch_hessian(bhip_ctx* ctx, DevImg<const T> ii, int skip, int nlevels, const int* sizes, DevImg<float> level0, long long levelStride,
						const HessLevelSource* from, unsigned int skipMask);
struct HessOctave {
	int skip, nlevels;
	const int* sizes;
	DevImg<float> level0;
	long long levelStride;
	const HessLevelSource* from;
	unsigned int skipMask;
};
template <class T>
int bhip_launch_hessian_octaves(bhip_ctx* ctx, DevImg<const T> ii, int noct, const HessOctave* octs);

struct DescPlanar {
	const float* data;
	long long imageStride, bandStride;
	int nBands;
};
struct DetectLevelParams {
	int skip, w, h;
	int sizeLower, sizeMid, sizeUpper;
	int border;
	int nbx, nby;
	unsigned int bitBase;
};
template <class T>
int bhip_launch_nms_scalespace(bhip_ctx* ctx, DevImg<const float> lower, DevImg<const float> mid, DevImg<const float> upper, DetectLevelParams p, int radius,
							   float threshold, unsigned int* bitmap, int bitmapWords, KeyPoint* cand, int* candCount, int cap, bool listOnly,
							   DevImg<const T> ii);
struct NmsLevelArgs {
	DevImg<const float> lower, mid, upper;
	DetectLevelParams p;
};
template <class T>
int bhip_launch_nms_scalespace_levels(bhip_ctx* ctx, int n, const NmsLevelArgs* lv, int radius, float threshold, unsigned int* bitmap, int bitmapWords,
									  KeyPoint* cand, int* candCount, int cap, DevImg<const T> ii);
int bhip_launch_select_nbest(bhip_ctx* ctx, DevImg<const float> lower, DevImg<const float> mid, DevImg<const float> upper, DetectLevelParams p, int radius,
							 int target, const unsigned int* bitmap, const unsigned int* prefix, int bitmapWords, const KeyPoint* nms, int cap, float* keyBuf,
							 int* idxBuf, KeyPoint* out, int* levelStart, int* levelCount, int levelIndex, int nlv);
int bhip_launch_select_nbest_xy(bhip_ctx* ctx, DevImg<const float> img, const int16_t* xy, int n, int target, bool positive, float* key, int* idx, int16_t* out);
int bhip_launch_compact_levels(bhip_ctx* ctx, const KeyPoint* src, int cap, const int* levelStart, const int* levelCount, int nlv, int batch, KeyPoint* dst,
							   int* totals);
int bhip_launch_rank_scatter(bhip_ctx* ctx, const unsigned int* bitmap, int bitmapWords, unsigned int* wordPrefix, const KeyPoint* cand,
							 const int* candCount, int cap, int batch, KeyPoint* sorted);
int bhip_launch_word_prefix(bhip_ctx* ctx, const unsigned int* bitmap, int bitmapWords, int batch, unsigned int* wordPrefix, int* totals);

template <class T>
int bhip_launch_describe_ex(bhip_ctx* ctx, DevImg<const T> ii, const KeyPoint* kps, int cap, const int* imageStart, int singleImage, long long total,
							SurfTables t, const double* anglesIn, double* angles, double* desc, uint8_t* white, const int* perm, DescPlanar planar);
int bhip_launch_kp_spatial_order(bhip_ctx* ctx, const KeyPoint* kps, int cap, const int* start, int batch, int maxCount, int W, int H, int* hist, int* perm);
struct ColTop {
	double min1, min2;
	int idx1, pad;
};
struct RowBest {
	double best;
	int idx, pad;
};
int bhip_assoc_phase1_l2(bhip_ctx* ctx, const double* src, int nsLocal, int srcBegin, const double* dst, int nd, int dof, double maxErr, int sqrtScore,
						 int* pairs, double* fit, void* colTop, DevBuf& work);
int bhip_assoc_phase1_ham(bhip_ctx* ctx, const int32_t* src, int nsLocal, int srcBegin, const int32_t* dst, int nd, int words, double maxErr, int* pairs,
						  double* fit, void* colTop, DevBuf& work);
int bhip_assoc_phase2(bhip_ctx* ctx, const void* colAll, int nranks, int nd, int nsLocal, int srcBegin, int* pairs, double* fit);
int bhip_assoc_coltop_size();
int bhip_ham_expand(bhip_ctx* ctx, const int* D, long long rows, int words, unsigned char* bytes, int* pop);
int bhip_ham_mfma_splits(int nU, int nV);
int bhip_ham_mfma_scan(bhip_ctx* ctx, bool colMode, const unsigned char* Ub, const int* Up, int nU, const unsigned char* Vb, const int* Vp, int nV, int words,
						 int vBase, double maxErr, void* partial, int splits);
int bhip_assoc_hamming_batched(bhip_ctx* ctx, const int32_t* src, const int32_t* dst, int words, int count, const long long* srcOff, const int* ns,
							   const long long* dstOff, const int* nd, double maxErr, int backwards, int* pairs, double* fit, DevBuf& work);

int bhip_assoc_l2_mfma_batched(bhip_ctx* ctx, AssocMfmaWork& W, const double* dev_src, const double* dev_dst, int count, const long long* srcOff,
								 const int* ns, const long long* dstOff, const int* nd, double maxErr, int backwards, int* dev_pairs, double* dev_fit,
								 int* usedMfma);

bool bhip_fused_plan(int skip, int nlevels, const int* sizes, int radius, int* TX, int* TY, int* ldsBytes);
bool bhip_fused_is_fixed(int skip, int nlevels, const int* sizes, int radius);
template <class T>
int bhip_launch_detect_fused(bhip_ctx* ctx, DevImg<const T> ii, int skip, int nlevels, const int* sizes, int nmid, const DetectLevelParams* mids,
							 const int* midLevels, int radius, float threshold, unsigned int* bitmap, int bitmapWords, KeyPoint* cand, int* candCount,
							 int cap, const FusedExport* exp);

int bhip_launch_conv(bhip_ctx* ctx, bool vertical, bool normalized, const float* kernel, int kw, int koff, DevImg<const float> in, DevImg<float> out);
int bhip_launch_blur_fused(bhip_ctx* ctx, const float* kernel, int kw, DevImg<const float> in, DevImg<float> out, bool* done);
int bhip_launch_pyr_layer_fused(bhip_ctx* ctx, const float* kernel, int kw, DevImg<const float> in, DevImg<float> out, int skip, bool* done);
int bhip_launch_conv_down(bhip_ctx* ctx, bool vertical, const float* kernel, int kw, DevImg<const float> in, DevImg<float> out, int skip);
int bhip_launch_conv_down(bhip_ctx* ctx, bool vertical, const int32_t* kernel, int kw, DevImg<const uint8_t> in, DevImg<uint8_t> out, int skip);
int bhip_launch_copy_images(bhip_ctx* ctx, DevImg<const float> in, DevImg<float> out);
int bhip_launch_copy_images(bhip_ctx* ctx, DevImg<const uint8_t> in, DevImg<uint8_t> out);
int bhip_launch_planar_average(bhip_ctx* ctx, const float* bands, long long bandStride, int numBands, long long n, float* out);
int bhip_launch_gradient(bhip_ctx* ctx, int kind, DevImg<const float> in, DevImg<float> dx, DevImg<float> dy, int border);
int bhip_launch_gradient(bhip_ctx* ctx, int kind, DevImg<const uint8_t> in, DevImg<int16_t> dx, DevImg<int16_t> dy, int border);
int bhip_launch_grad_intensity(bhip_ctx* ctx, int kind, DevImg<const float> dx, DevImg<const float> dy, DevImg<float> out);
int bhip_launch_corner_intensity(bhip_ctx* ctx, int kind, int radius, float kappa, DevImg<const float> dx, DevImg<const float> dy, DevImg<float> intensity,
								 float* scratch);
size_t bhip_corner_box_s16_scratch(int radius, int width, int height, int batch);
int bhip_launch_corner_box_s16(bhip_ctx* ctx, int kind, int radius, float kappa, DevImg<const int16_t> dx, DevImg<const int16_t> dy, DevImg<float> intensity,
							   void* scratch);
int bhip_corner_weighted_max_radius();
int bhip_launch_corner_weighted(bhip_ctx* ctx, int kind, int radius, float kappa, DevImg<const float> dx, DevImg<const float> dy, DevImg<float> intensity);
int bhip_launch_corner_weighted(bhip_ctx* ctx, int kind, int radius, float kappa, DevImg<const int16_t> dx, DevImg<const int16_t> dy, DevImg<float> intensity);
int bhip_launch_brief(bhip_ctx* ctx, DevImg<const float> img, int radius, int numPoints, const int* samplePoints, const int* compare, const double* xy, int n,
					  int* out, const int* start, int maxCount, int xyStride, long long xyImageStride, bool patchOk);
int bhip_launch_brief(bhip_ctx* ctx, DevImg<const uint8_t> img, int radius, int numPoints, const int* samplePoints, const int* compare, const double* xy, int n,
					  int* out, const int* start, int maxCount, int xyStride, long long xyImageStride, bool patchOk);
int bhip_launch_mean(bhip_ctx* ctx, bool vertical, DevImg<const float> in, DevImg<float> out, int radius);
int bhip_launch_conv2d(bhip_ctx* ctx, const float* kernel, int kw, int koff, DevImg<const float> in, DevImg<float> out);
int bhip_launch_median(bhip_ctx* ctx, DevImg<const float> in, DevImg<float> out, int radius);
int bhip_launch_integral_u8(bhip_ctx* ctx, DevImg<const uint8_t> in, DevImg<int32_t> out);
int bhip_launch_nonmax_blocks(bhip_ctx* ctx, DevImg<const float> img, int radius, float threshold, int border, unsigned int* bitmap, int bitmapWords,
							  unsigned short* posInBlock, int nbx, int nby);
int bhip_launch_blocks_to_xy(bhip_ctx* ctx, const unsigned int* bitmap, const unsigned int* wordPrefix, int bitmapWords, const unsigned short* posInBlock,
							 int nbx, int nby, int batch, int radius, int border, int16_t* xy, int cap);
int bhip_launch_nonmin_blocks(bhip_ctx* ctx, DevImg<const float> img, int radius, float threshold, int border, unsigned int* bitmap, int bitmapWords,
							  unsigned short* posInBlock, int nbx, int nby);

template <class T> struct FastTol;
template <> struct FastTol<uint8_t> { using type = int; };
template <> struct FastTol<float> { using type = float; };
size_t bhip_fast_scratch(int width, int height, int batch);
template <class T>
int bhip_launch_fast(bhip_ctx* ctx, DevImg<const T> img, typename FastTol<T>::type tol, int minContinuous, int maxFeatures, DevImg<float> inten, void* scratch,
					 int16_t* xyLow, int* nLow, int16_t* xyHigh, int* nHigh, int cap);

#define BHIP_DISP_MAX_RADIUS 7
#define BHIP_DISP_MAX_RANGE 256
struct DispBmParams {
	int minD, range, rx, ry;
	int maxError, rtolTol, textureThr;
};
size_t bhip_disparity_scratch(int width, int height, int batch);
template <class OutT>
int bhip_launch_disparity_bm(bhip_ctx* ctx, DevImg<const uint8_t> left, DevImg<const uint8_t> right, const DispBmParams& c, uint8_t* scratch, DevImg<OutT> out);

#define BHIP_CENSUS_MAX_SAMPLES 64
#define BHIP_CENSUS_MAX_OFFSET 7
struct CensusSamples {
	int n = 0, radius = 0;
	signed char dx[32] = {}, dy[32] = {};
};
int bhip_census_samples(const int* samplesXY, int nSamples, CensusSamples& s);
int bhip_census_variant_list(int variant, int* samplesXY);
template <class OutT>
int bhip_launch_census(bhip_ctx* ctx, DevImg<const uint8_t> in, int denseRadius, const CensusSamples* s, DevImg<OutT> out);
size_t bhip_disparity_census_scratch(int width, int height, int batch, int wordBytes);
template <class OutT>
int bhip_launch_disparity_bm_census(bhip_ctx* ctx, DevImg<const uint8_t> left, DevImg<const uint8_t> right, const DispBmParams& c, int wordBytes,
									const CensusSamples* s, uint8_t* scratch, DevImg<OutT> out);
template <class OutT>
int bhip_launch_disparity_bm5(bhip_ctx* ctx, DevImg<const uint8_t> left, DevImg<const uint8_t> right, const DispBmParams& c, uint8_t* scratch, DevImg<OutT> out);
template <class OutT>
int bhip_launch_disparity_bm5_census(bhip_ctx* ctx, DevImg<const uint8_t> left, DevImg<const uint8_t> right, const DispBmParams& c, int wordBytes,
									 const CensusSamples* s, uint8_t* scratch, DevImg<OutT> out);

struct DistortCoords {
	int model;
	const float* map;
	long long mapImageStride;
	const float* coeff;
};
struct DistortCrop {
	int x0, y0, x1, y1;
};
template <class T>
int bhip_launch_distort(bhip_ctx* ctx, DevImg<const T> src, const DistortCoords& co, const DistortCrop& crop, int interp, int border, int renderAll, DevImg<T> dst,
						DevImg<uint8_t> mask);
int bhip_launch_distort_build_map(bhip_ctx* ctx, int model, const float* coeff, int dw, int dh, float* map);

#define BHIP_BG_MAX_BANDS 4
#define BHIP_BG_MAX_GAUSSIANS 8
struct BgShape {
	int alg, bands, maxGaussians, width, height, streams;
};
struct BgConfig {
	float learnRate, threshold, initialVariance, minimumDifference;
	float learningPeriod, decay, maxDistance, significantWeight;
	int unknownValue;
};
template <class T>
struct BgFrames {
	T* data;
	long long streamStride, frameStride, bandStride;
	int stride, numFrames;
};
int bhip_bg_components(const BgShape& sh);
double bhip_bg_bytes(const BgShape& sh, int pixelBytes, int numFrames, bool masks, bool segment);
template <class T>
int bhip_launch_background(bhip_ctx* ctx, const BgShape& sh, const BgConfig& cfg, const BgFrames<const T>& f, const BgFrames<uint8_t>& m, float* model,
						   const int* state, bool segment);

size_t bhip_template_scratch(int batch);
template <class T>
int bhip_launch_template_intensity(bhip_ctx* ctx, int score, DevImg<const T> img, DevImg<const T> tpl, DevImg<const T> mask, float* stats, DevImg<float> out);
int bhip_launch_template_select(bhip_ctx* ctx, DevImg<const float> img, const int16_t* xy, const int* n, int cap, int maxMatches, bool maximize, float* key,
								int* idx, int16_t* outXY, float* outScore, int* outN);

#define BHIP_KLT_MAX_LAYERS 8
#define BHIP_KLT_MAX_RADIUS 7
#define BHIP_KLT_MAX_LEN ((2 * BHIP_KLT_MAX_RADIUS + 1) * (2 * BHIP_KLT_MAX_RADIUS + 1))

template <class TI, class TD>
struct KltPyrT {
	const TI* img;
	const TD* dx;
	const TD* dy;
	long long frameStride;
	long long off[BHIP_KLT_MAX_LAYERS];
	int w[BHIP_KLT_MAX_LAYERS], h[BHIP_KLT_MAX_LAYERS], stride[BHIP_KLT_MAX_LAYERS];
	float scale[BHIP_KLT_MAX_LAYERS];
	int numLayers;
	int frameW, frameH;
};
using KltPyr = KltPyrT<float, float>;
using KltPyrU8 = KltPyrT<uint8_t, int16_t>;

struct KltTab {
	int cap, batch, L, r, len;
	int *act, *drp, *spw, *freeL;
	int *nAct, *nDrp, *nSpw, *nFree;
	long long* total;
	long long* id;
	float *x, *y;
	float *tx, *ty;
	float* err;
	int* fault;
	int* keep;
	int* iters;
	float *lx, *ly, *gxx, *gxy, *gyy;
	float* tmpl;
};

int bhip_launch_klt_init(bhip_ctx* ctx, KltTab T, int firstSlot);
int bhip_launch_klt_begin(bhip_ctx* ctx, KltTab T);
int bhip_launch_klt_track(bhip_ctx* ctx, KltPyr P, KltTab T, bhip_klt_cfg cfg, int maxActive);
int bhip_launch_klt_describe(bhip_ctx* ctx, KltPyr P, KltTab T, bhip_klt_cfg cfg, int mode, const int* count, int maxCount);
int bhip_launch_klt_track(bhip_ctx* ctx, KltPyrU8 P, KltTab T, bhip_klt_cfg cfg, int maxActive);
int bhip_launch_klt_describe(bhip_ctx* ctx, KltPyrU8 P, KltTab T, bhip_klt_cfg cfg, int mode, const int* count, int maxCount);
int bhip_launch_klt_compact(bhip_ctx* ctx, KltTab T, int toUnused);
int bhip_launch_klt_mark_exclude(bhip_ctx* ctx, KltTab T, float scale0, DevImg<float> intensity, int maxActive);
int bhip_launch_klt_spawn_place(bhip_ctx* ctx, KltTab T, const int16_t* xy, int xyCap, const int* count, float scale0, int maxCount);
int bhip_launch_klt_spawn_commit(bhip_ctx* ctx, KltTab T, const int* count);
int bhip_launch_klt_add(bhip_ctx* ctx, KltTab T, const int* seq, const double* xy, int n, int frameW, int frameH, unsigned char* ok, int* list);
int bhip_launch_klt_match_drop(bhip_ctx* ctx, KltTab T, const int* seq, const long long* id, int n, unsigned char* ok, int maxActive);
int bhip_launch_klt_drop_all(bhip_ctx* ctx, KltTab T, int resetTotal);
int bhip_launch_klt_stats(bhip_ctx* ctx, KltTab T, unsigned long long* out);
int bhip_launch_klt_gather(bhip_ctx* ctx, KltTab T, int which, int seq, int n, long long* id, float* xy, int* fault, float* err);
int bhip_launch_klt_gather_templates(bhip_ctx* ctx, KltTab T, int which, int seq, int layer, int n, float* tmpl, float* G);

struct FlowRec {
	int fault;
	float error, dx, dy;
};
#define BHIP_FLOW_LANE_MAX_RADIUS 3
int bhip_launch_flow_track_wave(bhip_ctx* ctx, KltPyr P, const float* dst, int r, bhip_klt_cfg cfg, int batch, FlowRec* rec, unsigned long long* stats);
int bhip_launch_flow_track_wave(bhip_ctx* ctx, KltPyrU8 P, const uint8_t* dst, int r, bhip_klt_cfg cfg, int batch, FlowRec* rec, unsigned long long* stats);
int bhip_launch_flow_track_lane(bhip_ctx* ctx, KltPyr P, const float* dst, int r, bhip_klt_cfg cfg, int batch, FlowRec* rec, unsigned long long* stats);
int bhip_launch_flow_track_lane(bhip_ctx* ctx, KltPyrU8 P, const uint8_t* dst, int r, bhip_klt_cfg cfg, int batch, FlowRec* rec, unsigned long long* stats);
int bhip_launch_flow_reduce(bhip_ctx* ctx, const FlowRec* rec, int r, DevImg<float> flow);

#define BHIP_THRESH_FUSED_MAX_RADIUS 16
enum { BHIP_CMP_LE = 0, BHIP_CMP_GT = 1, BHIP_CMP_NOT_LE = 2 };
int bhip_launch_threshold_global(bhip_ctx* ctx, DevImg<const uint8_t> in, DevImg<uint8_t> out, int thr, const int* imageThr, int mode);
int bhip_launch_threshold_global(bhip_ctx* ctx, DevImg<const float> in, DevImg<uint8_t> out, float thr, const int* imageThr, int mode);
int bhip_launch_hist_u8(bhip_ctx* ctx, DevImg<const uint8_t> in, int* hist);
int bhip_launch_otsu_global(bhip_ctx* ctx, const int* hist, int batch, int totalPixels, double scale, int* thr);
template <class T>
int bhip_launch_local_compare(bhip_ctx* ctx, DevImg<const T> in, DevImg<const T> blur, DevImg<uint8_t> out, float scale, bool down);
int bhip_launch_blur_u8_pass(bhip_ctx* ctx, bool vertical, const int32_t* devTaps, int radius, DevImg<const uint8_t> in, DevImg<uint8_t> out);
int bhip_launch_blur_u8_fused(bhip_ctx* ctx, const int32_t* hostTaps, int radius, DevImg<const uint8_t> in, DevImg<uint8_t> out, bool compare, float scale, bool down);
struct ThreshBlocks {
	int kind;
	int bw, bh, nbx, nby;
	int local, down, useOtsu2;
	double scale, minimumSpread, tuning;
};
size_t bhip_block_threshold_scratch(int kind, int nbx, int nby, int images);
template <class T>
int bhip_launch_block_threshold(bhip_ctx* ctx, const ThreshBlocks& c, DevImg<const T> in, DevImg<uint8_t> out, void* scratch, int chunk);
```

boofcv_amd/csrc/describe.hip:

```cpp
#include "common.h"
#include <algorithm>
#include <type_traits>

struct DescParams {
	ImgView ii;
	const KeyPoint* kps;
	int cap;
	const int* imageStart;
	int batch;
	int singleImage;
	long long total;
	SurfTables t;
	const double* anglesIn;
	double* angles;
	double* desc;
	uint8_t* white;
	const int* perm;
	const float* bandData;
	long long bandImageStride, bandStride;
	int nBands;
	double oriRadiusFactor;
	int ldsPerWave;
	unsigned long long* stamps;
	int sort64;
	int serialOnly;
#ifdef BHIP_EXPERIMENTS
	int stopAfter;
	int windowStop;
#endif
};

#define ORI_EPL_MAX 8
#define DESC_ROW_MAX 16
#define DESC_BATCH 3

__device__ __forceinline__ int gradRadius(double width) {
	int r = ((int)(width + 0.5)) / 2;
	if (r <= 0) r = 1;
	return r;
}
template <class T>
struct __attribute__((packed, aligned(4))) Pair2 { T x, y; };
template <class T>
struct TapBases {
	const char *a0, *a1, *a3, *c10, *c13, *c20, *c23, *b0, *b1, *b3;
	unsigned int r1;
	unsigned int spanX;
	unsigned int spanY;
	unsigned int pitch4;
	bool anyInside;
};
__device__ __forceinline__ unsigned int uniformU32(unsigned int v) { return (unsigned int)__builtin_amdgcn_readfirstlane((int)v); }
template <class T>
__device__ __forceinline__ TapBases<T> makeBases(const T* d, int r, int stride, int W, int H, const void* safe8) {
	TapBases<T> B;
	r = (int)uniformU32((unsigned)r);
	B.anyInside = (2 * r + 2 <= W) && (2 * r + 2 <= H);
	const long long st = B.anyInside ? stride : 0, rr = B.anyInside ? r : 0, w = B.anyInside ? 2 * r + 1 : 0;
	const T* a = d;
	const T* c1 = a + rr * st;
	const T* c2 = c1 + st;
	const T* b = c2 + rr * st;
	B.a0 = (const char*)a; B.a1 = B.anyInside ? (const char*)(a + rr) : (const char*)safe8; B.a3 = (const char*)(a + w);
	B.c10 = (const char*)c1; B.c13 = (const char*)(c1 + w);
	B.c20 = (const char*)c2; B.c23 = (const char*)(c2 + w);
	B.b0 = (const char*)b; B.b1 = B.anyInside ? (const char*)(b + rr) : (const char*)safe8; B.b3 = (const char*)(b + w);
	B.r1 = (unsigned)(r + 1);
	B.spanX = B.anyInside ? (unsigned)(W - 2 * r - 1) : 0u;
	B.spanY = B.anyInside ? (unsigned)(H - 2 * r - 1) : 0u;
	B.pitch4 = (unsigned)st * 4u;
	return B;
}
template <class T>
struct GradTaps {
	T p0, p1, p2, p3, p4, p5, p6, p7, p8, p9, p10, p11;
	bool inb;
};
template <class T>
__device__ __forceinline__ T tapAt(const char* base, unsigned int off) { return *(const T*)(base + off); }
template <class T>
__device__ __forceinline__ void gradFetch(const TapBases<T>& B, int x, int y, bool on, GradTaps<T>& t) {
	const unsigned int ux = (unsigned)x - B.r1, uy = (unsigned)y - B.r1;
	const bool inb = on && ux < B.spanX && uy < B.spanY;
	unsigned int off = inb ? __umul24(uy, B.pitch4) + ux * 4u : 0u;
	asm volatile("" : "+v"(off));
	t.p0 = tapAt<T>(B.a0, off);
	const Pair2<T> a = *(const Pair2<T>*)(B.a1 + off);
	t.p1 = a.x; t.p2 = a.y;
	t.p3 = tapAt<T>(B.a3, off);
	__builtin_amdgcn_sched_barrier(0);
	t.p11 = tapAt<T>(B.c10, off); t.p4 = tapAt<T>(B.c13, off);
	__builtin_amdgcn_sched_barrier(0);
	t.p10 = tapAt<T>(B.c20, off); t.p5 = tapAt<T>(B.c23, off);
	__builtin_amdgcn_sched_barrier(0);
	t.p9 = tapAt<T>(B.b0, off);
	const Pair2<T> b = *(const Pair2<T>*)(B.b1 + off);
	t.p8 = b.x; t.p7 = b.y;
	t.p6 = tapAt<T>(B.b3, off);
	t.inb = inb;
}
template <class T>
__device__ __forceinline__ void gradFinish(const GradTaps<T>& t, T& gx, T& gy) {
	const T left = t.p8 - t.p9 - t.p1 + t.p0;
	const T right = t.p6 - t.p7 - t.p3 + t.p2;
	const T top = t.p4 - t.p11 - t.p3 + t.p0;
	const T bottom = t.p6 - t.p9 - t.p5 + t.p10;
	gx = t.inb ? right - left : T(0);
	gy = t.inb ? bottom - top : T(0);
}

__device__ __forceinline__ double angleDist(double a, double b) {
	double diff = a - b;
	if (diff > M_PI) diff = diff - 2.0 * M_PI;
	else if (diff < -M_PI) diff = 2.0 * M_PI + diff;
	return fabs(diff);
}

__device__ __forceinline__ void waveSync() {
	__builtin_amdgcn_fence(__ATOMIC_RELEASE, "wavefront");
	__builtin_amdgcn_wave_barrier();
	__builtin_amdgcn_fence(__ATOMIC_ACQUIRE, "wavefront");
}

struct OriSortOut {
	double* dX; double* dY; double* sA;
	float* sF;
};
template <int EPLT, class T>
__device__ __forceinline__ void permuteSorted(const T* gX, const T* gY, const unsigned short* srcI, const double (&a)[EPLT], const double* weights,
											   OriSortOut o, int p0, int cnt) {
	double x[EPLT], y[EPLT];
#pragma unroll
	for (int e = 0; e < EPLT; e++) {
		x[e] = 0.0; y[e] = 0.0;
		if (e < cnt) {
			const int i = srcI[p0 + e];
			x[e] = (double)gX[i]; y[e] = (double)gY[i];
			if (weights) { const double w = weights[i]; x[e] *= w; y[e] *= w; }
		}
	}
	waveSync();
#pragma unroll
	for (int e = 0; e < EPLT; e++)
		if (e < cnt) { o.dX[p0 + e] = x[e]; o.dY[p0 + e] = y[e]; o.sA[p0 + e] = a[e]; o.sF[p0 + e] = (float)a[e]; }
	waveSync();
}

template <int EPLT, class T>
__device__ __forceinline__ void sortSamplesByAngle(const T* gX, const T* gY, double* keyA, double* keyB, unsigned short* idxA, unsigned short* idxB,
													const double* weights, OriSortOut out, int n, int lane) {
	const int EPL = (n + 63) >> 6;
	const int p0 = lane * EPL;
	const int cnt = max(0, min(EPL, n - p0));
	{
		double k[EPLT];
		unsigned short id[EPLT];
#pragma unroll
		for (int e = 0; e < EPLT; e++) {
			k[e] = e < cnt ? keyA[p0 + e] : 0.0;
			id[e] = (unsigned short)(p0 + e);
		}
#pragma unroll
		for (int e = 1; e < EPLT; e++) {
#pragma unroll
			for (int f = e; f >= 1; f--) {
				if (f < cnt && k[f - 1] > k[f]) {
					const double tk = k[f]; k[f] = k[f - 1]; k[f - 1] = tk;
					const unsigned short ti = id[f]; id[f] = id[f - 1]; id[f - 1] = ti;
				}
			}
		}
		waveSync();
#pragma unroll
		for (int e = 0; e < EPLT; e++)
			if (e < cnt) { keyA[p0 + e] = k[e]; idxA[p0 + e] = id[e]; }
	}
	waveSync();
	double* srcK = keyA; double* dstK = keyB;
	unsigned short* srcI = idxA; unsigned short* dstI = idxB;
	for (int L = EPL; L < n; L <<= 1) {
		double key[EPLT];
		int lo[EPLT], hi[EPLT], base[EPLT];
		bool right[EPLT];
#pragma unroll
		for (int e = 0; e < EPLT; e++) {
			const int p = p0 + e;
			const int q = p / L;
			const int runStart = q * L;
			right[e] = q & 1;
			const int sibStart = right[e] ? runStart - L : runStart + L;
			lo[e] = min(sibStart, n);
			hi[e] = min(sibStart + L, n);
			key[e] = e < cnt ? srcK[p] : 0.0;
			base[e] = (right[e] ? sibStart : runStart) + (p - runStart) - min(sibStart, n);
			if (e >= cnt) hi[e] = lo[e];
		}
		for (int span = L; span > 0; span >>= 1) {
			double v[EPLT];
#pragma unroll
			for (int e = 0; e < EPLT; e++) {
				const int mid = (lo[e] + hi[e]) >> 1;
				v[e] = lo[e] < hi[e] ? srcK[mid] : 0.0;
			}
#pragma unroll
			for (int e = 0; e < EPLT; e++) {
				if (lo[e] < hi[e]) {
					const int mid = (lo[e] + hi[e]) >> 1;
					const bool before = right[e] ? (v[e] <= key[e]) : (v[e] < key[e]);
					if (before) lo[e] = mid + 1; else hi[e] = mid;
				}
			}
		}
#pragma unroll
		for (int e = 0; e < EPLT; e++) {
			if (e < cnt) {
				const int dst = base[e] + lo[e];
				dstK[dst] = key[e];
				dstI[dst] = srcI[p0 + e];
			}
		}
		waveSync();
		double* tk = srcK; srcK = dstK; dstK = tk;
		unsigned short* ti = srcI; srcI = dstI; dstI = ti;
	}
	{
		double a[EPLT];
#pragma unroll
		for (int e = 0; e < EPLT; e++) a[e] = e < cnt ? srcK[p0 + e] : 0.0;
		permuteSorted<EPLT, T>(gX, gY, srcI, a, weights, out, p0, cnt);
	}
}

__device__ __forceinline__ unsigned int angleKey32(double a) {
	const float f = (float)a + 0.0f;
	const unsigned int u = __float_as_uint(f);
	return (u & 0x80000000u) ? ~u : (u | 0x80000000u);
}
template <int EPLT, class T>
__device__ __forceinline__ bool sortSamplesFast32(const T* gX, const T* gY, const double* ang, unsigned int* keyA, unsigned int* keyB,
												   unsigned short* idxA, unsigned short* idxB, const double* weights, OriSortOut out, int n, int lane) {
	const int EPL = (n + 63) >> 6;
	const int p0 = lane * EPL;
	const int cnt = max(0, min(EPL, n - p0));
	{
		unsigned int k[EPLT];
		unsigned short id[EPLT];
#pragma unroll
		for (int e = 0; e < EPLT; e++) {
			k[e] = e < cnt ? angleKey32(ang[p0 + e]) : 0xffffffffu;
			id[e] = (unsigned short)(p0 + e);
		}
#pragma unroll
		for (int e = 1; e < EPLT; e++) {
#pragma unroll
			for (int f = e; f >= 1; f--) {
				if (f < cnt && k[f - 1] > k[f]) {
					const unsigned int tk = k[f]; k[f] = k[f - 1]; k[f - 1] = tk;
					const unsigned short ti = id[f]; id[f] = id[f - 1]; id[f - 1] = ti;
				}
			}
		}
#pragma unroll
		for (int e = 0; e < EPLT; e++)
			if (e < cnt) { keyA[p0 + e] = k[e]; idxA[p0 + e] = id[e]; }
	}
	waveSync();
	unsigned int* srcK = keyA; unsigned int* dstK = keyB;
	unsigned short* srcI = idxA; unsigned short* dstI = idxB;
	for (int L = EPL; L < n; L <<= 1) {
		const int s = (p0 / (2 * L)) * (2 * L);
		const int a0 = s, b0 = s + L;
		const int lenA = cnt > 0 ? min(L, n - s) : 0;
		const int lenB = cnt > 0 ? max(0, min(L, n - b0)) : 0;
		const int d = p0 - s;
		int lo = max(0, d - lenB), hi = min(d, lenA);
		for (int span = L; span > 0; span >>= 1) {
			const int mid = (lo + hi) >> 1;
			const bool on = lo < hi;
			const unsigned int ka = on ? srcK[a0 + mid] : 0u;
			const unsigned int kb = on ? srcK[b0 + d - 1 - mid] : 0u;
			if (on) { if (ka <= kb) lo = mid + 1; else hi = mid; }
		}
		int i = lo, j = d - lo;
		unsigned int ka = i < lenA ? srcK[a0 + i] : 0xffffffffu;
		unsigned int kb = j < lenB ? srcK[b0 + j] : 0xffffffffu;
		unsigned int outK[EPLT];
		int sp[EPLT];
#pragma unroll
		for (int e = 0; e < EPLT; e++) {
			const bool takeA = ka <= kb;
			outK[e] = takeA ? ka : kb;
			sp[e] = takeA ? a0 + i : b0 + j;
			i += takeA ? 1 : 0;
			j += takeA ? 0 : 1;
			const int nxt = takeA ? a0 + i : b0 + j;
			const int lim = takeA ? a0 + lenA : b0 + lenB;
			const unsigned int nk = (e + 1 < EPLT && nxt < lim) ? srcK[nxt] : 0xffffffffu;
			if (takeA) ka = nk; else kb = nk;
		}
		unsigned short outI[EPLT];
#pragma unroll
		for (int e = 0; e < EPLT; e++) outI[e] = e < cnt ? srcI[sp[e]] : (unsigned short)0;
#pragma unroll
		for (int e = 0; e < EPLT; e++)
			if (e < cnt) { dstK[p0 + e] = outK[e]; dstI[p0 + e] = outI[e]; }
		waveSync();
		unsigned int* tk = srcK; srcK = dstK; dstK = tk;
		unsigned short* ti = srcI; srcI = dstI; dstI = ti;
	}
	double a[EPLT];
	bool bad = false;
	{
		int id[EPLT], idn[EPLT];
		double an[EPLT];
#pragma unroll
		for (int e = 0; e < EPLT; e++) {
			id[e] = e < cnt ? srcI[p0 + e] : 0;
			idn[e] = (e < cnt && p0 + e + 1 < n) ? srcI[p0 + e + 1] : -1;
		}
#pragma unroll
		for (int e = 0; e < EPLT; e++) {
			a[e] = ang[id[e]];
			an[e] = idn[e] >= 0 ? ang[idn[e]] : 0.0;
		}
#pragma unroll
		for (int e = 0; e < EPLT; e++)
			if (idn[e] >= 0 && (a[e] > an[e] || (a[e] == an[e] && id[e] > idn[e]))) bad = true;
	}
	if (__any(bad)) return false;
	permuteSorted<EPLT, T>(gX, gY, srcI, a, weights, out, p0, cnt);
	return true;
}

#define ORI_BINS 1024
#define ORI_BIN_MAX 8
__device__ __forceinline__ int angleBin(double a) {
	const float f = ((float)a + 3.14159274f) * ((float)ORI_BINS / 6.28318548f);
	return min(max((int)f, 0), ORI_BINS - 1);
}
__device__ __forceinline__ int binOffset(const unsigned int* bins, int b) { return (int)((bins[b >> 1] >> ((b & 1) * 16)) & 0xffffu); }

template <int EPLT>
__device__ __forceinline__ bool countingSortScatter(const double (&a)[EPLT], const double (&dx)[EPLT], const double (&dy)[EPLT], int n, int lane,
													 unsigned int* bins, double* tmpA, unsigned short* tmpI, double* dX, double* dY, double* sA) {
	static_assert(ORI_BINS == 1024, "two 16-byte stores per lane clear the counters");
	{
		const uint4 z = make_uint4(0, 0, 0, 0);
		reinterpret_cast<uint4*>(bins)[2 * lane] = z;
		reinterpret_cast<uint4*>(bins)[2 * lane + 1] = z;
	}
	waveSync();
	int bin[EPLT], r[EPLT];
#pragma unroll
	for (int e = 0; e < EPLT; e++) {
		bin[e] = angleBin(a[e]);
		r[e] = 0;
		if (lane + 64 * e < n) {
			const int sh = (bin[e] & 1) * 16;
			const unsigned int old = atomicAdd(&bins[bin[e] >> 1], 1u << sh);
			r[e] = (int)((old >> sh) & 0xffffu);
		}
	}
	waveSync();
	int cnt[EPLT];
	int mx = 0;
#pragma unroll
	for (int e = 0; e < EPLT; e++) {
		cnt[e] = lane + 64 * e < n ? binOffset(bins, bin[e]) : 0;
		mx = max(mx, cnt[e]);
	}
#pragma unroll
	for (int o = 32; o >= 1; o >>= 1) mx = max(mx, __shfl_xor(mx, o, 64));
	if (mx > ORI_BIN_MAX) return false;
	waveSync();
	{
		const uint4 w0 = reinterpret_cast<const uint4*>(bins)[2 * lane], w1 = reinterpret_cast<const uint4*>(bins)[2 * lane + 1];
		const unsigned int w[8] = {w0.x, w0.y, w0.z, w0.w, w1.x, w1.y, w1.z, w1.w};
		unsigned int pre[16];
		unsigned int run = 0;
#pragma unroll
		for (int i = 0; i < 8; i++) {
			pre[2 * i] = run; run += w[i] & 0xffffu;
			pre[2 * i + 1] = run; run += w[i] >> 16;
		}
		unsigned int sc = run;
#pragma unroll
		for (int o = 1; o < 64; o <<= 1) {
			const unsigned int t = __shfl_up(sc, o, 64);
			if (lane >= o) sc += t;
		}
		const unsigned int base = sc - run;
		unsigned int ow[8];
#pragma unroll
		for (int i = 0; i < 8; i++) ow[i] = (base + pre[2 * i]) | ((base + pre[2 * i + 1]) << 16);
		reinterpret_cast<uint4*>(bins)[2 * lane] = make_uint4(ow[0], ow[1], ow[2], ow[3]);
		reinterpret_cast<uint4*>(bins)[2 * lane + 1] = make_uint4(ow[4], ow[5], ow[6], ow[7]);
	}
	waveSync();
	int off[EPLT];
#pragma unroll
	for (int e = 0; e < EPLT; e++) {
		off[e] = 0;
		if (lane + 64 * e < n) {
			off[e] = binOffset(bins, bin[e]);
			tmpA[off[e] + r[e]] = a[e];
			tmpI[off[e] + r[e]] = (unsigned short)(lane + 64 * e);
		}
	}
	waveSync();
	int rank[EPLT];
#pragma unroll
	for (int e = 0; e < EPLT; e++) rank[e] = 0;
	if (mx > 1) {
		for (int k = 0; k < mx; k++) {
			double ak[EPLT];
			int ik[EPLT];
#pragma unroll
			for (int e = 0; e < EPLT; e++) {
				const bool on = k < cnt[e];
				ak[e] = on ? tmpA[off[e] + k] : 0.0;
				ik[e] = on ? (int)tmpI[off[e] + k] : 0;
			}
#pragma unroll
			for (int e = 0; e < EPLT; e++)
				if (k < cnt[e] && (ak[e] < a[e] || (ak[e] == a[e] && ik[e] < lane + 64 * e))) rank[e]++;
		}
	}
	waveSync();
#pragma unroll
	for (int e = 0; e < EPLT; e++)
		if (lane + 64 * e < n) {
			const int f = off[e] + rank[e];
			dX[f] = dx[e]; dY[f] = dy[e]; sA[f] = a[e];
		}
	waveSync();
	return true;
}

template <int EPLT>
__device__ __forceinline__ bool slidingWindowFast(double* dX, double* dY, const double* sA, const float* sF, const unsigned int* bins, unsigned int* marks, int n,
												   double window, int lane, double& bestX, double& bestY, unsigned long long* st , int wstop = -1) {
#ifdef BHIP_EXPERIMENTS
#define WSTAMP(i) do { if (st && lane == 0) st[i] = __builtin_readcyclecounter(); if (wstop == (i)) { bestX = 1.0; bestY = 0.0; return true; } } while (0)
#else
#define WSTAMP(i) do { if (st && lane == 0) st[i] = __builtin_readcyclecounter(); } while (0)
#endif
	const int EPL = (n + 63) >> 6;
	const int p0 = lane * EPL;
	const int cnt = max(0, min(EPL, n - p0));
	bool abnormal = false;
	int valE[EPLT];
	int runMax = 0;
	{
		const float winLo = (float)window - 4.0e-6f;
		const float twoPiF = 6.28318530717958647692f;
		if (!(winLo > 0.0f)) return false;
		float fa[EPLT];
		int lo[EPLT], hi[EPLT];
		if (bins) {
#pragma unroll
			for (int e = 0; e < EPLT; e++) {
				lo[e] = 0;
				if (e < cnt) {
					const int a = p0 + e;
					const double T = sA[a] + (window - 1.0e-9);
					const bool wrap = T >= M_PI;
					const int below = binOffset(bins, angleBin(wrap ? T - 2.0 * M_PI : T));
					const int c0 = (wrap ? n + below : below) - (a + 1);
					lo[e] = min(max(c0, 0), n - 1);
				}
			}
		} else {
#pragma unroll
		for (int e = 0; e < EPLT; e++) {
			fa[e] = e < cnt ? sF[p0 + e] : 0.0f;
			lo[e] = 0;
			hi[e] = e < cnt ? n : 1;
		}
		for (int span = n; span > 1; span = (span + 1) >> 1) {
			float fk[EPLT];
#pragma unroll
			for (int e = 0; e < EPLT; e++) {
				const int mid = (lo[e] + hi[e]) >> 1;
				const int kabs = p0 + e + mid;
				const int k = kabs >= n ? kabs - n : kabs;
				fk[e] = (hi[e] - lo[e] > 1) ? sF[k] : 0.0f;
			}
#pragma unroll
			for (int e = 0; e < EPLT; e++) {
				if (hi[e] - lo[e] > 1) {
					const int mid = (lo[e] + hi[e]) >> 1;
					const int kabs = p0 + e + mid;
					const float fo = (fk[e] - fa[e]) + (kabs >= n ? twoPiF : 0.0f);
					if (fo <= winLo) lo[e] = mid; else hi[e] = mid;
				}
			}
		}
		}
		double ta[EPLT], nxt[EPLT];
		int cc[EPLT];
		bool act[EPLT];
#pragma unroll
		for (int e = 0; e < EPLT; e++) {
			ta[e] = e < cnt ? sA[p0 + e] : 0.0;
			cc[e] = lo[e];
			act[e] = e < cnt && lo[e] < n - 1;
			const int kabs = p0 + e + lo[e] + 1;
			const int k = kabs >= n ? kabs - n : kabs;
			nxt[e] = act[e] ? sA[k] : 0.0;
			if (e < cnt && !act[e]) abnormal = true;
		}
		for (int guard = 0; guard < 18; guard++) {
			bool any = false;
#pragma unroll
			for (int e = 0; e < EPLT; e++) {
				if (act[e]) {
					const bool wrapped = p0 + e + cc[e] + 1 >= n;
					const double d1 = nxt[e] - ta[e];
					const double fo = wrapped ? d1 + 2.0 * M_PI : d1;
					if (!(fo <= window)) {
						const double behind = wrapped ? -d1 : fabs(2.0 * M_PI + (-d1));
						if (behind <= window) abnormal = true;
						act[e] = false;
					} else {
						cc[e]++;
						if (cc[e] >= n - 1) { abnormal = true; act[e] = false; }
						else if (guard == 17) { abnormal = true; act[e] = false; }
					}
				}
			}
#pragma unroll
			for (int e = 0; e < EPLT; e++) {
				if (act[e]) {
					const int k2abs = p0 + e + cc[e] + 1;
					nxt[e] = sA[k2abs >= n ? k2abs - n : k2abs];
					any = true;
				}
			}
			if (!__any(any)) break;
		}
#pragma unroll
		for (int e = 0; e < EPLT; e++) {
			valE[e] = 0;
			if (e < cnt) {
				valE[e] = p0 + e + cc[e] + 1;
				runMax = max(runMax, valE[e]);
			}
		}
	}
	WSTAMP(8);
	int scan = runMax;
#pragma unroll
	for (int o = 1; o < 64; o <<= 1) {
		const int t = __shfl_up(scan, o, 64);
		if (lane >= o) scan = max(scan, t);
	}
	int prevE = __shfl_up(scan, 1, 64);
	if (lane == 0) prevE = 1;
	prevE = max(prevE, 1);
	int lastE = 1;
	int Ereg[EPLT];
	{
		int pe = prevE;
		double chk[EPLT];
		bool need[EPLT];
#pragma unroll
		for (int e = 0; e < EPLT; e++) {
			need[e] = false;
			chk[e] = 0.0;
			Ereg[e] = 0;
			if (e < cnt) {
				const int a = p0 + e;
				const int Ea = max(pe, valE[e]);
				if (pe > valE[e] - 1 && pe > a && pe < a + n) {
					const int k = pe >= n ? pe - n : pe;
					need[e] = true;
					chk[e] = sA[k];
				}
				if (Ea >= a + n) abnormal = true;
				pe = Ea;
				Ereg[e] = Ea;
			}
		}
#pragma unroll
		for (int e = 0; e < EPLT; e++)
			if (need[e] && angleDist(sA[p0 + e], chk[e]) <= window) abnormal = true;
		lastE = pe;
	}
	if (__any(abnormal)) return false;
	lastE = __shfl(lastE, (n - 1) / EPL, 64);
	WSTAMP(9);
	double vx[EPLT], vy[EPLT];
	{
		double lx[EPLT], ly[EPLT];
#pragma unroll
		for (int e = 0; e < EPLT; e++) {
			vx[e] = e < cnt ? dX[p0 + e] : 0.0;
			vy[e] = e < cnt ? dY[p0 + e] : 0.0;
		}
		double tx = 0, ty = 0;
#pragma unroll
		for (int e = 0; e < EPLT; e++) {
			tx += vx[e]; ty += vy[e];
			lx[e] = tx; ly[e] = ty;
		}
		double ox = tx, oy = ty;
#pragma unroll
		for (int o = 1; o < 64; o <<= 1) {
			const double ux = __shfl_up(ox, o, 64), uy = __shfl_up(oy, o, 64);
			if (lane >= o) { ox += ux; oy += uy; }
		}
		ox -= tx; oy -= ty;
		waveSync();
#pragma unroll
		for (int e = 0; e < EPLT; e++)
			if (e < cnt) { dX[p0 + e] = ox + lx[e]; dY[p0 + e] = oy + ly[e]; }
	}
	waveSync();
	const double totX = dX[n - 1], totY = dY[n - 1];
	WSTAMP(10);
	double bMag = -1.0, bMag2 = -1.0, bX = 0, bY = 0;
	int bPos = 0x7fffffff;
	if (lane == 0) { bX = dX[0]; bY = dY[0]; bMag = bX * bX + bY * bY; bPos = 0; }
	{
#pragma unroll
		for (int e = 0; e < EPLT; e++) marks[lane * EPLT + e] = 0u;
		waveSync();
#pragma unroll
		for (int e = 0; e < EPLT; e++)
			if (e < cnt && p0 + e <= n - 2) atomicAdd(&marks[Ereg[e] >> 1], 1u << ((Ereg[e] & 1) * 16));
		waveSync();
		{
			unsigned int w[EPLT], pre[2 * EPLT];
			unsigned int run = 0;
#pragma unroll
			for (int e = 0; e < EPLT; e++) w[e] = marks[lane * EPLT + e];
#pragma unroll
			for (int e = 0; e < EPLT; e++) {
				run += w[e] & 0xffffu; pre[2 * e] = run;
				run += w[e] >> 16; pre[2 * e + 1] = run;
			}
			unsigned int sc = run;
#pragma unroll
			for (int o = 1; o < 64; o <<= 1) {
				const unsigned int t = __shfl_up(sc, o, 64);
				if (lane >= o) sc += t;
			}
			const unsigned int base = sc - run;
#pragma unroll
			for (int e = 0; e < EPLT; e++) marks[lane * EPLT + e] = (base + pre[2 * e]) | ((base + pre[2 * e + 1]) << 16);
		}
		waveSync();
		const unsigned short* owner = (const unsigned short*)marks;
		for (int E0 = 1; E0 < lastE; E0 += 64) {
			const int E = E0 + lane;
			if (E < lastE) {
				const int a = owner[E];
				const int ke = E >= n ? E - n : E;
				const double ax = a > 0 ? dX[a - 1] : 0.0, ay = a > 0 ? dY[a - 1] : 0.0;
				const double ex = dX[ke], ey = dY[ke];
				double sx, sy;
				if (E < n) { sx = ex - ax; sy = ey - ay; }
				else { sx = (totX - ax) + ex; sy = (totY - ay) + ey; }
				const double mag = sx * sx + sy * sy;
				if (mag > bMag) { bMag2 = bMag; bMag = mag; bX = sx; bY = sy; bPos = E; }
				else if (mag > bMag2) bMag2 = mag;
			}
		}
	}
	WSTAMP(11);
	double m = bMag;
#pragma unroll
	for (int o = 32; o >= 1; o >>= 1) m = fmax(m, __shfl_xor(m, o, 64));
	int pos = (bMag == m) ? bPos : 0x7fffffff;
#pragma unroll
	for (int o = 32; o >= 1; o >>= 1) pos = min(pos, __shfl_xor(pos, o, 64));
	const unsigned long long owner = __ballot(bMag == m && bPos == pos);
	const int src = __ffsll((long long)owner) - 1;
	bestX = __shfl(bX, src, 64);
	bestY = __shfl(bY, src, 64);
	const double tieFloor = m - m * 1.0e-9;
	if (__popcll(__ballot(bMag >= tieFloor)) + __popcll(__ballot(bMag2 >= tieFloor)) > 1) {
		waveSync();
#pragma unroll
		for (int e = 0; e < EPLT; e++)
			if (e < cnt) { dX[p0 + e] = vx[e]; dY[p0 + e] = vy[e]; }
		waveSync();
		return false;
	}
	WSTAMP(12);
	return true;
#undef WSTAMP
}

#ifdef BHIP_EXPERIMENTS
#define DSTAMP(i) do { if (STAMP && lane == 0) P.stamps[g * 16 + (i)] = __builtin_readcyclecounter(); if (P.stopAfter == (i)) return; } while (0)
#else
#define DSTAMP(i) do { if (STAMP && lane == 0) P.stamps[g * 16 + (i)] = __builtin_readcyclecounter(); } while (0)
#endif

template <bool STAMP, int EPLT, int TWT, class TAP, int CFG = 0>
__global__ __launch_bounds__(256) void k_describe(DescParams P) {
	extern __shared__ __attribute__((aligned(16))) unsigned char ldsAll[];
	const int wave = __builtin_amdgcn_readfirstlane((int)(threadIdx.x >> 6));
	const int lane = threadIdx.x & 63;
	const long long nblk = (P.total + 3) >> 2;
	const long long chunk = (nblk + 7) >> 3;
	const long long blk = (long long)(blockIdx.x & 7) * chunk + (blockIdx.x >> 3);
	if ((long long)(blockIdx.x >> 3) >= chunk) return;
	const long long slot = blk * 4 + wave;
	if (slot >= P.total) return;
	const long long g = P.perm ? (long long)P.perm[slot] : slot;
	unsigned char* lds = ldsAll + (size_t)wave * P.ldsPerWave;

	int img, local;
	if (P.imageStart) {
		int lo = 0, hi = P.batch;
		while (hi - lo > 1) {
			const int m = (lo + hi) >> 1;
			if ((long long)P.imageStart[m] <= g) lo = m; else hi = m;
		}
		img = lo;
		local = (int)(g - P.imageStart[img]);
	} else {
		img = P.singleImage;
		local = (int)g;
	}
	img = (int)uniformU32((unsigned)img);
	local = (int)uniformU32((unsigned)local);
	const KeyPoint kp = P.imageStart ? P.kps[(long long)img * P.cap + local] : P.kps[local];
	const TAP* __restrict__ d = (const TAP*)P.ii.data + (long long)img * P.ii.imageStride;
	const int stride = P.ii.stride, W = P.ii.width, H = P.ii.height;
	const SurfTables& T = P.t;

	DSTAMP(0);
	double angle;
	double dirX = 0.0, dirY = 0.0;
	if (P.anglesIn) {
		angle = P.anglesIn[g];
	} else {
		const double radius = kp.scale * P.oriRadiusFactor;
		const double oscale = radius * T.oriRadiusToScale;
		const TapBases<TAP> G = makeBases<TAP>(d, gradRadius(oscale * T.oriKernelWidth), stride, W, H, P.kps);
		const double period = oscale * T.oriPeriod;
		double tl_x = kp.x - T.oriRadius * period;
		double tl_y = kp.y - T.oriRadius * period;
		tl_x += 0.5;
		tl_y += 0.5;
		const bool oriSliding = CFG == 1 ? true : CFG == 2 ? false : (T.oriStable != 0);
		const int sw = CFG == 1 ? 17 : CFG == 2 ? 13 : T.oriWidth, n = sw * sw;
		TAP* gX = (TAP*)lds;
		TAP* gY = gX + n;
		double* ang = (double*)(lds + (size_t)8 * n);
		double* keyB = (double*)(lds + (size_t)16 * n);
		double* dX = (double*)lds;
		double* dY = dX + n;
		TAP gx[EPLT], gy[EPLT];
		double dxr[EPLT], dyr[EPLT], ar[EPLT];
		{
			GradTaps<TAP> tp[EPLT];
#pragma unroll
			for (int e = 0; e < EPLT; e++) {
				const int idx = lane + 64 * e;
				const int sy = idx / sw, sx = idx - sy * sw;
				const int xx = (int)(tl_x + sx * period);
				const int yy = (int)(tl_y + sy * period);
				gradFetch<TAP>(G, xx, yy, idx < n, tp[e]);
			}
#pragma unroll
			for (int e = 0; e < EPLT; e++) gradFinish<TAP>(tp[e], gx[e], gy[e]);
		}
#pragma unroll
		for (int e = 0; e < EPLT; e++) {
			const int idx = lane + 64 * e;
			dxr[e] = 0.0; dyr[e] = 0.0; ar[e] = 0.0;
			if (idx < n) {
				double dx = (double)gx[e], dy = (double)gy[e];
				if (oriSliding) {
					if (T.oriHasWeights) {
						const double w = T.oriWeights[idx];
						dx *= w;
						dy *= w;
					}
					dxr[e] = dx; dyr[e] = dy;
					ar[e] = atan2(dy, dx);
				} else {
					if (T.oriHasWeights) {
						const double w = T.oriWeights[idx];
						dX[idx] = w * dx;
						dY[idx] = w * dy;
					} else {
						dX[idx] = dx;
						dY[idx] = dy;
					}
				}
			}
		}
		waveSync();
		DSTAMP(1);
		if (oriSliding) {
			unsigned short* idxA = (unsigned short*)(lds + (size_t)24 * n);
			unsigned short* idxB = idxA + n;
			double bestX = 0, bestY = 0;
			bool needSerial = true;
			const OriSortOut so{dX, dY, dY + n, (float*)(lds + (size_t)28 * n)};
			const double* wts = T.oriHasWeights ? T.oriWeights : nullptr;
			unsigned int* bins = (unsigned int*)(lds + (((size_t)28 * n + 15) & ~(size_t)15));
			const bool counted = !P.sort64 && countingSortScatter<EPLT>(ar, dxr, dyr, n, lane, bins, (double*)lds, (unsigned short*)(lds + (size_t)8 * n), dX, dY, dY + n);
			if (!counted) {
#pragma unroll
				for (int e = 0; e < EPLT; e++) {
					const int idx = lane + 64 * e;
					if (idx < n) { gX[idx] = gx[e]; gY[idx] = gy[e]; ang[idx] = ar[e]; }
				}
				waveSync();
				bool sorted = false;
				if (!P.sort64) sorted = sortSamplesFast32<EPLT, TAP>(gX, gY, ang, (unsigned int*)keyB, (unsigned int*)keyB + n, idxA, idxB, wts, so, n, lane);
				if (!sorted) sortSamplesByAngle<EPLT, TAP>(gX, gY, ang, keyB, idxA, idxB, wts, so, n, lane);
			}
			ang = so.sA;
			DSTAMP(2);
			if (T.oriWindow < 3.0 && !P.serialOnly) needSerial = !slidingWindowFast<EPLT>(dX, dY, ang, so.sF, counted ? bins : nullptr, (unsigned int*)(lds + (size_t)24 * n), n, T.oriWindow, lane, bestX, bestY, STAMP ? P.stamps + g * 16 : nullptr
#ifdef BHIP_EXPERIMENTS
																				  , P.windowStop
#endif
																				  );
			if (needSerial) {
				if (lane == 0) {
					const int total = n;
					int start = 0, end = 1;
					double sumX = dX[0], sumY = dY[0];
					double best = sumX * sumX + sumY * sumY;
					bestX = sumX;
					bestY = sumY;
					double endAngle = ang[end];
					const double window = T.oriWindow;
					while (start != total) {
						const double startAngle = ang[start];
						while (angleDist(startAngle, endAngle) <= window) {
							sumX += dX[end];
							sumY += dY[end];
							const double mag = sumX * sumX + sumY * sumY;
							if (mag > best) { best = mag; bestX = sumX; bestY = sumY; }
							end++;
							if (end >= total) end = 0;
							endAngle = ang[end];
							if (end == start) break;
						}
						sumX -= dX[start];
						sumY -= dY[start];
						start++;
					}
				}
				bestX = __shfl(bestX, 0, 64);
				bestY = __shfl(bestY, 0, 64);
			}
			angle = atan2(bestY, bestX);
			dirX = bestX; dirY = bestY;
		} else {
			double Dx = 0, Dy = 0;
			if (lane == 0) {
				for (int i = 0; i < n; i++) { Dx += dX[i]; Dy += dY[i]; }
			}
			Dx = __shfl(Dx, 0, 64);
			Dy = __shfl(Dy, 0, 64);
			angle = atan2(Dy, Dx);
			dirX = Dx; dirY = Dy;
		}
		waveSync();
	}
	DSTAMP(3);
	if (lane == 0 && P.angles) P.angles[g] = angle;
	if (!P.desc) return;

	double c, s;
	{
		const double h2 = dirX * dirX + dirY * dirY;
		if (h2 > 1.0e-200 && h2 < 1.0e200) {
			const double h = sqrt(h2);
			c = dirX / h; s = dirY / h;
		} else {
			c = cos(angle); s = sin(angle);
		}
	}
	const double scale = kp.scale;
	const int descR = gradRadius(T.widthSample * scale);
	const int widthLargeGrid = CFG ? 4 : T.widthLargeGrid, widthSubRegion = CFG ? 5 : T.widthSubRegion;
	const bool stableDesc = CFG == 1 ? true : CFG == 2 ? false : (T.stable != 0);
	const int regionSize = widthLargeGrid * widthSubRegion;
	const int regionR = regionSize / 2;
	const int overLap = CFG == 1 ? 2 : CFG == 2 ? 0 : (T.stable ? T.overLap : 0);
	const int gridW = regionSize + 2 * overLap;
	const int nsamp = gridW * gridW;
	typedef typename std::conditional<CFG != 0, TAP, double>::type SampT;
	SampT* sX = (SampT*)lds;
	SampT* sY = sX + nsamp;
	double* feat = (double*)(sY + nsamp);
	TAP lapTap = TAP(0);
	if (P.white && lane < 16) {
		const int x = (int)(kp.x + 0.5), y = (int)(kp.y + 0.5);
		const int si = (int)ceil(scale);
		const int size = 9 * si;
		const int blockW = size / 3, blockH = size - blockW - 1;
		const int r1 = blockW / 2, r2 = blockW + r1, r3 = blockH / 2;
		const int box = lane >> 2, corner = lane & 3;
		const int rx = box == 0 ? r2 : box == 1 ? r1 : r3;
		const int ry = box == 0 ? r3 : box == 1 ? r3 : box == 2 ? r2 : r1;
		int bx0 = x - rx - 1, by0 = y - ry - 1, bx1 = x + rx, by1 = y + ry;
		bx0 = min(bx0, W - 1); by0 = min(by0, H - 1); bx1 = min(bx1, W - 1); by1 = min(by1, H - 1);
		const int cx = (corner == 0 || corner == 1) ? bx1 : bx0;
		const int cy = (corner == 0 || corner == 2) ? by1 : by0;
		if (cx >= 0 && cy >= 0) lapTap = d[(long long)cy * stride + cx];
	}
	const int dof = CFG ? 64 : T.dof;
	const int nb = P.nBands > 0 ? P.nBands : 1;
#pragma unroll 1
	for (int band = 0; band < nb; band++) {
	const TAP* __restrict__ db = P.nBands > 0 ? (const TAP*)P.bandData + (long long)img * P.bandImageStride + (long long)band * P.bandStride : d;
	if (band > 0) waveSync();
	const TapBases<TAP> G = makeBases<TAP>(db, descR, stride, W, H, P.kps);
	{
		const double c_x = kp.x + 0.5, c_y = kp.y + 0.5;
		const int blocksPerSide = (gridW + 7) >> 3;
		const int nblocks = blocksPerSide * blocksPerSide;
		const int ly = lane >> 3, lx = lane & 7;
		const int gridOff = regionR + overLap;
		if (CFG != 0) {
			static_assert(DESC_BATCH == 3, "one batch = one row of three blocks");
			double PX[3], PY[3];
#pragma unroll
			for (int u = 0; u < 3; u++) {
				const int rX = 8 * u + lx - gridOff;
				const double regionX = rX * scale;
				PX[u] = c_x + c * regionX;
				PY[u] = c_y + s * regionX;
			}
#pragma unroll 1
			for (int by = 0; by < 3; by++) {
				GradTaps<TAP> tp[3];
				const int iy = 8 * by + ly;
				const double regionY = (iy - gridOff) * scale;
				const double qx = s * regionY, qy = c * regionY;
#pragma unroll
				for (int u = 0; u < 3; u++) {
					const bool on = iy < gridW && 8 * u + lx < gridW;
					gradFetch<TAP>(G, (int)(PX[u] - qx), (int)(PY[u] + qy), on, tp[u]);
				}
#pragma unroll
				for (int u = 0; u < 3; u++) {
					TAP gx, gy;
					gradFinish<TAP>(tp[u], gx, gy);
					const int ix = 8 * u + lx;
					if (iy < gridW && ix < gridW) { sX[iy * gridW + ix] = (SampT)gx; sY[iy * gridW + ix] = (SampT)gy; }
				}
			}
		} else {
#pragma unroll 1
		for (int b0 = 0; b0 < nblocks; b0 += DESC_BATCH) {
			GradTaps<TAP> tp[DESC_BATCH];
			int at[DESC_BATCH];
#pragma unroll
			for (int u = 0; u < DESC_BATCH; u++) {
				const int b = b0 + u;
				const int by = b / blocksPerSide, bx = b - by * blocksPerSide;
				const int iy = 8 * by + ly, ix = 8 * bx + lx;
				const bool on = b < nblocks && iy < gridW && ix < gridW;
				at[u] = on ? iy * gridW + ix : -1;
				const int rY = iy - gridOff, rX = ix - gridOff;
				const double regionY = rY * scale;
				const double regionX = rX * scale;
				const int pixelX = (int)(c_x + c * regionX - s * regionY);
				const int pixelY = (int)(c_y + s * regionX + c * regionY);
				gradFetch<TAP>(G, pixelX, pixelY, on, tp[u]);
			}
#pragma unroll
			for (int u = 0; u < DESC_BATCH; u++) {
				TAP gx, gy;
				gradFinish<TAP>(tp[u], gx, gy);
				if (at[u] >= 0) { sX[at[u]] = (SampT)gx; sY[at[u]] = (SampT)gy; }
			}
		}
		}
	}
	waveSync();
	DSTAMP(4);
	const int T_w = widthSubRegion + 2 * overLap;
	if (widthLargeGrid == 4) {
		const int sub = lane >> 2, q = lane & 3;
		const int suby = sub >> 2, subx = sub & 3;
		const int rY = -regionR + suby * widthSubRegion, rX = -regionR + subx * widthSubRegion;
		const int base = (rY + regionR) * gridW + rX + regionR;
		const int nT = T_w * T_w;
		const double ms = -s;
		double a0 = 0, a1 = 0, a2 = 0, a3 = 0;
#pragma unroll 3
		for (int t = q; t < nT; t += 4) {
			const int i = t / T_w, j = t - i * T_w;
			const double vx = (double)sX[base + i * gridW + j], vy = (double)sY[base + i * gridW + j];
			const double w = stableDesc ? T.weightSub[t] : T.weightFast[(regionR + rY + i) * regionSize + regionR + rX + j];
			const double dx = w * vx, dy = w * vy;
			const double pdx = c * dx + s * dy;
			const double pdy = ms * dx + c * dy;
			a0 += pdx; a1 += fabs(pdx); a2 += pdy; a3 += fabs(pdy);
		}
#pragma unroll
		for (int o = 1; o <= 2; o <<= 1) {
			a0 += __shfl_xor(a0, o, 64); a1 += __shfl_xor(a1, o, 64); a2 += __shfl_xor(a2, o, 64); a3 += __shfl_xor(a3, o, 64);
		}
		double sum = q == 0 ? a0 : q == 1 ? a1 : q == 2 ? a2 : a3;
		if (stableDesc) sum = T.weightGrid[sub] * sum;
		feat[band * dof + lane] = sum;
	} else
#pragma unroll 1
	for (int f = lane; f < dof; f += 64) {
		const int sub = f >> 2, comp = f & 3;
		const int suby = sub / widthLargeGrid, subx = sub - suby * widthLargeGrid;
		const int rY = -regionR + suby * widthSubRegion, rX = -regionR + subx * widthSubRegion;
		const double cA = comp < 2 ? c : -s, cB = comp < 2 ? s : c;
		const unsigned long long absMask = (comp & 1) ? 0x7fffffffffffffffull : 0xffffffffffffffffull;
		double sum = 0;
#pragma unroll 1
		for (int i = 0; i < T_w; i++) {
			const int index = (rY + regionR + i) * gridW + rX + regionR;
			double vx[TWT], vy[TWT];
			double w[TWT];
#pragma unroll
			for (int j = 0; j < TWT; j++) {
				const bool on = j < T_w;
				vx[j] = on ? (double)sX[index + j] : 0.0;
				vy[j] = on ? (double)sY[index + j] : 0.0;
				w[j] = !on ? 0.0 : stableDesc ? T.weightSub[i * T_w + j] : T.weightFast[(regionR + rY + i) * regionSize + regionR + rX + j];
			}
#pragma unroll
			for (int j = 0; j < TWT; j++) {
				if (j < T_w) {
					const double dx = w[j] * vx[j];
					const double dy = w[j] * vy[j];
					const double v = cA * dx + cB * dy;
					sum += __longlong_as_double((long long)((unsigned long long)__double_as_longlong(v) & absMask));
				}
			}
		}
		if (stableDesc) sum = T.weightGrid[sub] * sum;
		feat[band * dof + f] = sum;
	}
	}
	waveSync();
	DSTAMP(5);
	const int dofAll = dof * nb;
	double norm = 0;
	for (int f = lane; f < dofAll; f += 64) { const double v = feat[f]; norm += v * v; }
#pragma unroll
	for (int o = 32; o >= 1; o >>= 1) norm += __shfl_xor(norm, o, 64);
	double* out = P.desc + g * dofAll;
	if (norm == 0) {
		for (int f = lane; f < dofAll; f += 64) out[f] = feat[f];
	} else {
		norm = sqrt(norm);
		for (int f = lane; f < dofAll; f += 64) out[f] = feat[f] / norm;
	}
	if (P.white) {
		TAP bs[4];
#pragma unroll
		for (int b = 0; b < 4; b++) {
			const TAP br = __shfl(lapTap, 4 * b, 64), tr = __shfl(lapTap, 4 * b + 1, 64), bl = __shfl(lapTap, 4 * b + 2, 64), tl = __shfl(lapTap, 4 * b + 3, 64);
			bs[b] = br - tr - bl + tl;
		}
		TAP xx = 0;
		xx += bs[0] * TAP(1);
		xx += bs[1] * TAP(-3);
		TAP yy = 0;
		yy += bs[2] * TAP(1);
		yy += bs[3] * TAP(-3);
		double lap = (double)xx;
		lap += (double)yy;
		if (lane == 0) P.white[g] = lap > 0 ? 1 : 0;
	}
	DSTAMP(6);
}

static int bhip_describe_default_cfg(const SurfTables& t) {
	const bool defGrid = t.widthLargeGrid == 4 && t.widthSubRegion == 5 && t.dof == 64;
	if (defGrid && t.stable && t.overLap == 2 && t.oriStable && t.oriWidth == 17) return 1;
	if (defGrid && !t.stable && !t.oriStable && t.oriWidth == 13) return 2;
	return 0;
}

int bhip_describe_lds_bytes(const SurfTables& t, int nBands) {
	const int n = t.oriWidth * t.oriWidth;
	const int ori = std::max(n * 32 + 16, ((28 * n + 15) & ~15) + 2048);
	const int overLap = t.stable ? t.overLap : 0;
	const int gridW = t.widthLargeGrid * t.widthSubRegion + 2 * overLap;
	const int ns = gridW * gridW;
	const int sampBytes = bhip_describe_default_cfg(t) ? 4 : 8;
	const int desc = 2 * ns * sampBytes + t.dof * 8 * (nBands > 0 ? nBands : 1);
	int b = ori > desc ? ori : desc;
	return (b + 15) & ~15;
}

template <class T>
int bhip_launch_describe_ex(bhip_ctx* ctx, DevImg<const T> ii, const KeyPoint* kps, int cap, const int* imageStart, int singleImage, long long total,
							SurfTables t, const double* anglesIn, double* angles, double* desc, uint8_t* white, const int* perm, DescPlanar planar) {
	if (total <= 0) return BHIP_OK;
	DescParams P;
	P.ii = bhip_kernel_view(ii); P.kps = kps; P.cap = cap; P.imageStart = imageStart; P.batch = ii.batch; P.singleImage = singleImage; P.total = total; P.t = t;
	P.anglesIn = anglesIn; P.angles = angles; P.desc = desc; P.white = white; P.perm = perm;
	P.bandData = nullptr; P.bandImageStride = P.bandStride = 0; P.nBands = 0;
	if (planar.nBands > 0) {
		if (!planar.data) return bhip_fail(ctx, BHIP_ERR_INVALID, "bad planar description request");
		P.bandData = planar.data; P.bandImageStride = planar.imageStride; P.bandStride = planar.bandStride; P.nBands = planar.nBands;
	}
	P.oriRadiusFactor = planar.nBands > 0 ? 1.0 : 2.0;
	P.ldsPerWave = bhip_describe_lds_bytes(t, P.nBands);
	P.stamps = nullptr;
	P.serialOnly = bhip_env_flag("BHIP_DESCRIBE_SERIAL") ? 1 : 0;
	P.sort64 = bhip_env_flag("BHIP_DESCRIBE_SORT64") ? 1 : 0;
#ifdef BHIP_EXPERIMENTS
	{ const char* e = getenv("BHIP_DESCRIBE_STOP"); P.stopAfter = e ? atoi(e) : -1; }
	{ const char* e = getenv("BHIP_DESCRIBE_WSTOP"); P.windowStop = e ? atoi(e) : -1; }
#endif
	if (t.oriWidth * t.oriWidth > 64 * ORI_EPL_MAX) return bhip_fail(ctx, BHIP_ERR_UNSUPPORTED, "orientation sample grid too large for the GPU path");
	if (t.widthSubRegion + 2 * (t.stable ? t.overLap : 0) > DESC_ROW_MAX) return bhip_fail(ctx, BHIP_ERR_UNSUPPORTED, "SURF sub-region too wide for the GPU path");
	if (P.ldsPerWave * 4 > 160 * 1024) return bhip_fail(ctx, BHIP_ERR_UNSUPPORTED, "orientation/descriptor sample grid too large for LDS");
	const long long blocks = ((((total + 3) / 4) + 7) / 8) * 8;
	if (blocks > 0x7fffffffLL) return bhip_fail(ctx, BHIP_ERR_INVALID, "too many key points");
	if ((long long)ii.stride * ii.height > 0x3fffffffLL || ii.stride >= (1 << 17)) return bhip_fail(ctx, BHIP_ERR_UNSUPPORTED, "integral image too large for 32-bit tap offsets");
#ifdef BHIP_EXPERIMENTS
	const char* stampPath = getenv("BHIP_DESCRIBE_STAMPS");
	if (stampPath && total > 1000 && std::is_same<T, float>::value) {
		unsigned long long* dev = nullptr;
		if (hipMalloc(&dev, (size_t)total * 128) == hipSuccess) {
			(void)hipMemsetAsync(dev, 0, (size_t)total * 128, ctx->stream);
			P.stamps = dev;
			{
				const int epl = (t.oriWidth * t.oriWidth + 63) / 64;
				const int tw = t.widthSubRegion + 2 * (t.stable ? t.overLap : 0);
				if (bhip_describe_default_cfg(t) == 1) hipLaunchKernelGGL((k_describe<true, 5, 9, float, 1>), dim3((unsigned)blocks), dim3(256), (size_t)P.ldsPerWave * 4, ctx->stream, P);
				else hipLaunchKernelGGL((k_describe<true, 8, 16, float>), dim3((unsigned)blocks), dim3(256), (size_t)P.ldsPerWave * 4, ctx->stream, P);
			}
			std::vector<unsigned long long> h((size_t)total * 16);
			(void)hipMemcpyAsync(h.data(), dev, (size_t)total * 128, hipMemcpyDeviceToHost, ctx->stream);
			(void)hipStreamSynchronize(ctx->stream);
			(void)hipFree(dev);
			double sum[7] = {0}, wsum[6] = {0};
			long long cnt = 0;
			for (long long k = 0; k < total; k++) {
				const unsigned long long* tt = &h[(size_t)k * 16];
				if (!tt[6] || !tt[0]) continue;
				for (int i = 1; i <= 6; i++) sum[i] += (double)(tt[i] - tt[i - 1]);
				if (tt[8] && tt[12]) { wsum[0] += (double)(tt[8] - tt[2]); for (int i = 1; i <= 4; i++) wsum[i] += (double)(tt[8 + i] - tt[7 + i]); wsum[5] += (double)(tt[3] - tt[12]); }
				cnt++;
			}
			FILE* f = fopen(stampPath, "a");
			if (f && cnt) {
				fprintf(f, "waves %lld  avg cycles: samples %.0f  sort %.0f  window+atan2 %.0f  descSamples %.0f  sums %.0f  norm+laplace %.0f\n", cnt,
						sum[1] / cnt, sum[2] / cnt, sum[3] / cnt, sum[4] / cnt, sum[5] / cnt, sum[6] / cnt);
			}
			if (f && cnt) fprintf(f, "   window split: c(a) %.0f  scan+validate %.0f  prefix %.0f  candidates %.0f  reduce %.0f  atan2+rest %.0f\n", wsum[0] / cnt, wsum[1] / cnt,
								  wsum[2] / cnt, wsum[3] / cnt, wsum[4] / cnt, wsum[5] / cnt);
			if (f) fclose(f);
			BHIP_HIP(ctx, hipGetLastError());
			return BHIP_OK;
		}
	}
#endif
	{
		const int gridWv = t.widthLargeGrid * t.widthSubRegion + 2 * (t.stable ? t.overLap : 0);
		const int nbv = P.nBands > 0 ? P.nBands : 1;
		const double perKp = (double)(t.oriWidth * t.oriWidth + nbv * gridWv * gridWv) * 12 * 4 + 8.0 * t.dof * nbv + 8 + 1;
		ProfScope ps(ctx, "k_describe", perKp * (double)total);
		const int epl = (t.oriWidth * t.oriWidth + 63) / 64;
		const int tw = t.widthSubRegion + 2 * (t.stable ? t.overLap : 0);
		const dim3 grid((unsigned)blocks), block(256);
		size_t ldsBytes = (size_t)P.ldsPerWave * 4;
#ifdef BHIP_EXPERIMENTS
		{ const char* e = getenv("BHIP_DESCRIBE_LDSPAD"); if (e) ldsBytes += (size_t)atoi(e); }
#endif
		const bool cfgStable = bhip_describe_default_cfg(t) == 1, cfgFast = bhip_describe_default_cfg(t) == 2;
		constexpr bool ints = std::is_same<T, int32_t>::value;
		const void* fn;
		if (cfgStable) fn = ints ? (const void*)k_describe<false, 5, 9, int, 1> : (const void*)k_describe<false, 5, 9, float, 1>;
		else if (cfgFast) fn = ints ? (const void*)k_describe<false, 3, 5, int, 2> : (const void*)k_describe<false, 3, 5, float, 2>;
		else if (epl == 5 && tw == 9) fn = ints ? (const void*)k_describe<false, 5, 9, int> : (const void*)k_describe<false, 5, 9, float>;
		else if (epl == 3 && tw == 5) fn = ints ? (const void*)k_describe<false, 3, 5, int> : (const void*)k_describe<false, 3, 5, float>;
		else fn = ints ? (const void*)k_describe<false, 8, 16, int> : (const void*)k_describe<false, 8, 16, float>;
		if (ldsBytes > 65536) BHIP_HIP(ctx, hipFuncSetAttribute(fn, hipFuncAttributeMaxDynamicSharedMemorySize, (int)ldsBytes));
		void* args[] = {(void*)&P};
#ifdef BHIP_EXPERIMENTS
		{
			const char* e = getenv("BHIP_DESCRIBE_SPLIT");
			if (e && e[0] == '1' && P.angles && P.desc && !P.anglesIn) {
				DescParams Po = P, Pd = P;
				Po.desc = nullptr; Po.white = nullptr;
				Pd.anglesIn = P.angles;
				void* ao[] = {(void*)&Po};
				void* ad[] = {(void*)&Pd};
				{ ProfScope p1(ctx, "k_describe_ori"); BHIP_HIP(ctx, hipLaunchKernel(fn, grid, block, ao, ldsBytes, ctx->stream)); }
				{ ProfScope p2(ctx, "k_describe_desc"); BHIP_HIP(ctx, hipLaunchKernel(fn, grid, block, ad, ldsBytes, ctx->stream)); }
				return BHIP_OK;
			}
			if (e && e[0] == '2' && P.angles && P.desc && !P.anglesIn) {
				static hipStream_t side = nullptr;
				static hipEvent_t evFork = nullptr, evJoin = nullptr;
				if (!side) { (void)hipStreamCreateWithFlags(&side, hipStreamNonBlocking); (void)hipEventCreateWithFlags(&evFork, hipEventDisableTiming); (void)hipEventCreateWithFlags(&evJoin, hipEventDisableTiming); }
				DescParams Po = P, Pd = P;
				Po.desc = nullptr; Po.white = nullptr;
				static double* staleAngles = nullptr; static long long staleN = 0;
				if (staleN < P.total) { if (staleAngles) (void)hipFree(staleAngles); (void)hipMalloc(&staleAngles, (size_t)P.total * 8); (void)hipMemsetAsync(staleAngles, 0, (size_t)P.total * 8, ctx->stream); staleN = P.total; }
				Pd.anglesIn = staleAngles; Pd.angles = nullptr;
				void* ao[] = {(void*)&Po};
				void* ad[] = {(void*)&Pd};
				BHIP_HIP(ctx, hipEventRecord(evFork, ctx->stream));
				BHIP_HIP(ctx, hipStreamWaitEvent(side, evFork, 0));
				BHIP_HIP(ctx, hipLaunchKernel(fn, grid, block, ad, ldsBytes, side));
				BHIP_HIP(ctx, hipLaunchKernel(fn, grid, block, ao, ldsBytes, ctx->stream));
				BHIP_HIP(ctx, hipEventRecord(evJoin, side));
				BHIP_HIP(ctx, hipStreamWaitEvent(ctx->stream, evJoin, 0));
				BHIP_HIP(ctx, hipMemcpyAsync(staleAngles, P.angles, (size_t)P.total * 8, hipMemcpyDeviceToDevice, ctx->stream));
				return BHIP_OK;
			}
		}
#endif
		BHIP_HIP(ctx, hipLaunchKernel(fn, grid, block, args, ldsBytes, ctx->stream));
	}
	BHIP_HIP(ctx, hipGetLastError());
	return BHIP_OK;
}
template int bhip_launch_describe_ex(bhip_ctx*, DevImg<const float>, const KeyPoint*, int, const int*, int, long long, SurfTables, const double*, double*, double*,  uint8_t*, const int*, DescPlanar);
template int bhip_launch_describe_ex(bhip_ctx*, DevImg<const int32_t>, const KeyPoint*, int, const int*, int, long long, SurfTables, const double*, double*, double*,  uint8_t*, const int*, DescPlanar);
```

boofcv_amd/csrc/detect.hip:

```cpp
#include "hessian_dev.h"
#include <cfloat>

template <bool MIN> __device__ __forceinline__ bool nmsBeats(float a, float b) { return MIN ? a <= b : a >= b; }
template <bool MIN> __device__ __forceinline__ float nmsPad() { return MIN ? INFINITY : -INFINITY; }
template <bool MIN> __device__ __forceinline__ float nmsMarker() { return MIN ? -FLT_MAX : FLT_MAX; }
template <int RT, bool MIN = false>
__device__ __forceinline__ bool strictLocalMax(const float* __restrict__ img, int stride, int w, int h, int x, int y, int r, float v, float thr) {
	if (!nmsBeats<MIN>(v, thr) || v == nmsMarker<MIN>()) return false;
	bool isMax = true;
	if (RT > 0) {
		float nb[(2 * RT + 1) * (2 * RT + 1)];
#pragma unroll
		for (int j = -RT; j <= RT; j++)
#pragma unroll
			for (int i = -RT; i <= RT; i++) {
				const int xx = x + i, yy = y + j;
				const bool in = xx >= 0 && xx < w && yy >= 0 && yy < h && !(i == 0 && j == 0);
				nb[(j + RT) * (2 * RT + 1) + i + RT] = in ? img[(long long)yy * stride + xx] : nmsPad<MIN>();
			}
#pragma unroll
		for (int k = 0; k < (2 * RT + 1) * (2 * RT + 1); k++)
			if (nmsBeats<MIN>(nb[k], v)) isMax = false;
	} else {
		const int x0 = max(x - r, 0), x1 = min(x + r, w - 1), y0 = max(y - r, 0), y1 = min(y + r, h - 1);
// ... 433 lines not shown
	const int start = bitRank(bm, pf, P.p.bitBase);
	const int end = bitRank(bm, pf, P.p.bitBase + (unsigned)P.p.nbx * (unsigned)P.p.nby);
	const int n = end - start;
	const KeyPoint* list = P.nms + (long long)img * P.cap + start;
	KeyPoint* out = P.out + (long long)img * P.cap + start;
	const bool select = n > P.target;
	const int m = select ? P.target : n;
	const bool inLds = n <= SEL_LDS;
	float* key = inLds ? ldsKey : P.keyBuf + (long long)img * P.cap + start;
	int* idx = inLds ? ldsIdx : P.idxBuf + (long long)img * P.cap + start;
	if (select) {
		for (int i = lane; i < n; i += 64) {
			key[i] = -(float)list[i].scale;
			idx[i] = i;
		}
		__threadfence_block();
		__builtin_amdgcn_wave_barrier();
		if (lane == 0) quickSelectIndexSeq(key, P.target, n, idx);
		__threadfence_block();
		__builtin_amdgcn_wave_barrier();
	}
	const float* lower = P.lower + (long long)img * P.imageStride;
	const float* mid = P.mid + (long long)img * P.imageStride;
	const float* upper = P.upper + (long long)img * P.imageStride;
	int base = 0;
	for (int j0 = 0; j0 < m; j0 += 64) {
		const int j = j0 + lane;
		bool ok = false;
		KeyPoint kp;
		kp.x = kp.y = kp.scale = 0; kp.key = 0; kp.pad = 0;
		if (j < m) {
			const KeyPoint src = list[select ? idx[j] : j];
			const int x = (int)src.x, y = (int)src.y;
			ok = scaleSpaceKeyPoint(lower, mid, upper, P.stride, P.p, P.radius, x, y, (float)src.scale, kp);
		}
		const unsigned long long vote = __ballot(ok);
		if (ok) out[base + __popcll(vote & ((1ull << lane) - 1ull))] = kp;
		base += __popcll(vote);
	}
	if (lane == 0) {
		P.levelStart[(long long)img * P.nlv + P.levelIndex] = start;
		P.levelCount[(long long)img * P.nlv + P.levelIndex] = base;
	}
}

__global__ __launch_bounds__(64) void k_compact_levels(const KeyPoint* __restrict__ src, int cap, const int* __restrict__ levelStart, const int* __restrict__ levelCount,
														int nlv, KeyPoint* __restrict__ dst, int* __restrict__ totals) {
	const int img = blockIdx.x, lane = threadIdx.x;
	int off = 0;
	for (int l = 0; l < nlv; l++) {
		const int s = levelStart[(long long)img * nlv + l], c = levelCount[(long long)img * nlv + l];
		for (int i = lane; i < c; i += 64) dst[(long long)img * cap + off + i] = src[(long long)img * cap + s + i];
		off += c;
	}
	if (lane == 0) totals[img] = off;
}

int bhip_launch_select_nbest(bhip_ctx* ctx, DevImg<const float> lower, DevImg<const float> mid, DevImg<const float> upper, DetectLevelParams p, int radius,
							 int target, const unsigned int* bitmap, const unsigned int* prefix, int bitmapWords, const KeyPoint* nms, int cap, float* keyBuf,
							 int* idxBuf, KeyPoint* out, int* levelStart, int* levelCount, int levelIndex, int nlv) {
	if (mid.batch <= 0) return BHIP_OK;
	SelectParams P{lower.data, mid.data, upper.data, mid.imageStride, mid.stride, p, radius, target, bitmap, prefix, bitmapWords, nms, cap, keyBuf, idxBuf, out,
				   levelStart, levelCount, levelIndex, nlv};
	{
		ProfScope ps(ctx, "k_select_nbest");
		hipLaunchKernelGGL(k_select_nbest, dim3(mid.batch), dim3(64), 0, ctx->stream, P);
	}
	BHIP_HIP(ctx, hipGetLastError());
	return BHIP_OK;
}

int bhip_launch_compact_levels(bhip_ctx* ctx, const KeyPoint* src, int cap, const int* levelStart, const int* levelCount, int nlv, int batch, KeyPoint* dst,
							   int* totals) {
	if (batch <= 0) return BHIP_OK;
	{
		ProfScope ps(ctx, "k_compact_levels");
		hipLaunchKernelGGL(k_compact_levels, dim3(batch), dim3(64), 0, ctx->stream, src, cap, levelStart, levelCount, nlv, dst, totals);
	}
	BHIP_HIP(ctx, hipGetLastError());
	return BHIP_OK;
}

__global__ __launch_bounds__(64) void k_select_nbest_xy(const float* __restrict__ img, int stride, const int16_t* __restrict__ xy, int n, int target, int positive,
														 float* key, int* idx, int16_t* __restrict__ out) {
	const int lane = threadIdx.x;
	for (int i = lane; i < n; i += 64) {
		const float v = img[(long long)xy[2 * i + 1] * stride + xy[2 * i]];
		key[i] = positive ? -v : v;
		idx[i] = i;
	}
	__threadfence_block();
	__builtin_amdgcn_wave_barrier();
	if (lane == 0) quickSelectIndexSeq(key, target, n, idx);
	__threadfence_block();
	__builtin_amdgcn_wave_barrier();
	for (int i = lane; i < target; i += 64) {
		out[2 * i] = xy[2 * idx[i]];
		out[2 * i + 1] = xy[2 * idx[i] + 1];
	}
}

int bhip_launch_select_nbest_xy(bhip_ctx* ctx, DevImg<const float> img, const int16_t* xy, int n, int target, bool positive, float* key, int* idx, int16_t* out) {
	hipLaunchKernelGGL(k_select_nbest_xy, dim3(1), dim3(64), 0, ctx->stream, img.data, img.stride, xy, n, target, positive ? 1 : 0, key, idx, out);
	BHIP_HIP(ctx, hipGetLastError());
	return BHIP_OK;
}

struct TemplateSelectParams {
	const float* img;
	long long imageStride;
	int stride, w, h;
	const int16_t* xy;
	const int* n;
	int cap, maxMatches, maximize;
	float* key;
	int* idx;
	int16_t* outXY;
	float* outScore;
	int* outN;
};
__global__ __launch_bounds__(64) void k_template_select(TemplateSelectParams P) {
	const int lane = threadIdx.x;
	const long long b = blockIdx.x;
	const int n = P.n ? min(max(P.n[b], 0), P.cap) : P.cap;
	const int N = min(P.maxMatches, n);
	const float* img = P.img + b * P.imageStride;
	const int16_t* xy = P.xy + b * P.cap * 2;
	float* key = P.key + b * P.cap;
	int* idx = P.idx + b * P.cap;
	for (int i = lane; i < n; i += 64) {
		const int x = xy[2 * i], y = xy[2 * i + 1];
		const float v = (x >= 0 && x < P.w && y >= 0 && y < P.h) ? img[(long long)y * P.stride + x] : 0.f;
		key[i] = P.maximize ? -v : v;
		idx[i] = i;
	}
	__threadfence_block();
	__builtin_amdgcn_wave_barrier();
	if (lane == 0 && n > 0) quickSelectIndexSeq(key, N, n, idx);
	__threadfence_block();
	__builtin_amdgcn_wave_barrier();
	for (int i = lane; i < N; i += 64) {
		const int c = idx[i];
		P.outXY[(b * P.maxMatches + i) * 2] = xy[2 * c];
		P.outXY[(b * P.maxMatches + i) * 2 + 1] = xy[2 * c + 1];
		const int x = xy[2 * c], y = xy[2 * c + 1];
		const float v = (x >= 0 && x < P.w && y >= 0 && y < P.h) ? img[(long long)y * P.stride + x] : 0.f;
		P.outScore[b * P.maxMatches + i] = P.maximize ? v : -v;
	}
	if (lane == 0) P.outN[b] = N;
}

int bhip_launch_template_select(bhip_ctx* ctx, DevImg<const float> img, const int16_t* xy, const int* n, int cap, int maxMatches, bool maximize, float* key,
								int* idx, int16_t* outXY, float* outScore, int* outN) {
	if (img.batch <= 0) return BHIP_OK;
	TemplateSelectParams P{img.data, img.imageStride, img.stride, img.width, img.height, xy, n, cap, maxMatches, maximize ? 1 : 0, key, idx, outXY, outScore, outN};
	{
		ProfScope ps(ctx, "k_template_select");
		hipLaunchKernelGGL(k_template_select, dim3(img.batch), dim3(64), 0, ctx->stream, P);
	}
	BHIP_HIP(ctx, hipGetLastError());
	return BHIP_OK;
}

struct NonmaxParams {
	const float* img;
	long long imageStride;
	int stride, w, h, radius, border, nbx, bitmapWords;
	float threshold;
	unsigned int* bitmap;
	unsigned short* posInBlock;
	long long blocksPerImage;
};
template <bool MIN>
__global__ __launch_bounds__(256) void k_nonmax_blocks(NonmaxParams P) {
	const int b = P.border, w = P.w, h = P.h, r = P.radius, stride = P.stride;
	const int x = b + blockIdx.x * blockDim.x + threadIdx.x;
	const int yBase = b + blockIdx.y * NMS_ROWS;
	const float* img = P.img + (long long)blockIdx.z * P.imageStride;
	float col[NMS_ROWS + 2], lf[NMS_ROWS], rt[NMS_ROWS];
#pragma unroll
	for (int k = 0; k < NMS_ROWS + 2; k++) {
		const int yy = yBase - 1 + k;
		col[k] = (yy >= 0 && yy < h && x < w - b) ? img[(long long)yy * stride + x] : nmsPad<MIN>();
	}
#pragma unroll
	for (int k = 0; k < NMS_ROWS; k++) {
		const int yy = yBase + k;
		const bool rowIn = yy < h && x < w - b;
		lf[k] = (rowIn && x >= 1) ? img[(long long)yy * stride + x - 1] : nmsPad<MIN>();
		rt[k] = (rowIn && x + 1 < w) ? img[(long long)yy * stride + x + 1] : nmsPad<MIN>();
	}
	__shared__ int candList[256 * NMS_ROWS];
	__shared__ int candCount;
	if (threadIdx.x == 0) candCount = 0;
	__syncthreads();
	if (x < w - b) {
#pragma unroll
		for (int k = 0; k < NMS_ROWS; k++) {
			const int y = yBase + k;
			const float val = col[k + 1];
			const bool pass = y < h - b && nmsBeats<MIN>(val, P.threshold) && val != nmsMarker<MIN>() &&
							  !(nmsBeats<MIN>(lf[k], val) || nmsBeats<MIN>(rt[k], val) || nmsBeats<MIN>(col[k], val) || nmsBeats<MIN>(col[k + 2], val));
			if (pass) candList[atomicAdd(&candCount, 1)] = (k << 16) | (int)threadIdx.x;
		}
	}
	__syncthreads();
	const int ncand = candCount;
	const int step = r + 1;
	for (int ci = threadIdx.x; ci < ncand; ci += blockDim.x) {
		const int code = candList[ci];
		const int cx = b + blockIdx.x * blockDim.x + (code & 0xFFFF);
		const int cy = yBase + (code >> 16);
		const float val = img[(long long)cy * stride + cx];
		if (!(r == 2 ? strictLocalMax<2, MIN>(img, stride, w, h, cx, cy, r, val, P.threshold) : strictLocalMax<0, MIN>(img, stride, w, h, cx, cy, r, val, P.threshold)))
			continue;
		const int bx = (cx - b) / step, by = (cy - b) / step;
		const unsigned int bit = (unsigned)by * (unsigned)P.nbx + (unsigned)bx;
		atomicOr(&P.bitmap[(long long)blockIdx.z * P.bitmapWords + (bit >> 5)], 1u << (bit & 31));
		P.posInBlock[(long long)blockIdx.z * P.blocksPerImage + bit] = (unsigned short)((cy - b - by * step) * step + (cx - b - bx * step));
	}
}

template <bool MIN>
static int launchNonmaxBlocks(bhip_ctx* ctx, DevImg<const float> img, int radius, float threshold, int border, unsigned int* bitmap, int bitmapWords,
							  unsigned short* posInBlock, int nbx, int nby) {
	const int w = img.width, h = img.height, batch = img.batch;
	const int rw = w - 2 * border, rh = h - 2 * border;
	if (rw <= 0 || rh <= 0 || batch <= 0) return BHIP_OK;
	if (radius > 254) return bhip_fail(ctx, BHIP_ERR_UNSUPPORTED, "NMS radius too large");
	NonmaxParams P{img.data, img.imageStride, img.stride, w, h, radius, border, nbx, bitmapWords, threshold, bitmap, posInBlock, (long long)nbx * nby};
	dim3 grid((rw + 255) / 256, (rh + NMS_ROWS - 1) / NMS_ROWS, batch);
	{
		ProfScope ps(ctx, MIN ? "k_nonmin_blocks" : "k_nonmax_blocks", 4.0 * w * h * batch);
		hipLaunchKernelGGL(k_nonmax_blocks<MIN>, grid, dim3(256), 0, ctx->stream, P);
	}
	BHIP_HIP(ctx, hipGetLastError());
	return BHIP_OK;
}
int bhip_launch_nonmax_blocks(bhip_ctx* ctx, DevImg<const float> img, int radius, float threshold, int border, unsigned int* bitmap, int bitmapWords,
							  unsigned short* posInBlock, int nbx, int nby) {
	return launchNonmaxBlocks<false>(ctx, img, radius, threshold, border, bitmap, bitmapWords, posInBlock, nbx, nby);
}
int bhip_launch_nonmin_blocks(bhip_ctx* ctx, DevImg<const float> img, int radius, float threshold, int border, unsigned int* bitmap, int bitmapWords,
							  unsigned short* posInBlock, int nbx, int nby) {
	return launchNonmaxBlocks<true>(ctx, img, radius, threshold, border, bitmap, bitmapWords, posInBlock, nbx, nby);
}

__global__ __launch_bounds__(256) void k_blocks_to_xy(const unsigned int* __restrict__ bitmap, const unsigned int* __restrict__ prefix, int words,
													   const unsigned short* __restrict__ posInBlock, long long blocksPerImage, int nbx, int step, int border,
													   int16_t* __restrict__ xy, int cap) {
	const int word = blockIdx.x * blockDim.x + threadIdx.x;
	if (word >= words) return;
	const long long img = blockIdx.y;
	unsigned int bits = bitmap[img * words + word];
	unsigned int rank = prefix[img * words + word];
	while (bits) {
		const int bit = __ffs(bits) - 1;
		bits &= bits - 1;
		const long long idx = (long long)word * 32 + bit;
		const int by = (int)(idx / nbx), bx = (int)(idx - (long long)by * nbx);
		const int pos = posInBlock[img * blocksPerImage + idx];
		if ((int)rank < cap) {
			xy[(img * cap + rank) * 2] = (int16_t)(border + bx * step + pos % step);
			xy[(img * cap + rank) * 2 + 1] = (int16_t)(border + by * step + pos / step);
		}
		rank++;
	}
}

int bhip_launch_blocks_to_xy(bhip_ctx* ctx, const unsigned int* bitmap, const unsigned int* wordPrefix, int bitmapWords, const unsigned short* posInBlock,
							 int nbx, int nby, int batch, int radius, int border, int16_t* xy, int cap) {
	if (batch <= 0 || bitmapWords <= 0 || cap <= 0) return BHIP_OK;
	ProfScope ps(ctx, "k_blocks_to_xy");
	hipLaunchKernelGGL(k_blocks_to_xy, dim3((bitmapWords + 255) / 256, batch), dim3(256), 0, ctx->stream, bitmap, wordPrefix, bitmapWords, posInBlock,
					   (long long)nbx * nby, nbx, radius + 1, border, xy, cap);
	BHIP_HIP(ctx, hipGetLastError());
	return BHIP_OK;
}


#define KPT 8
__global__ __launch_bounds__(256) void k_kp_tile_count(const KeyPoint* __restrict__ kps, int cap, const int* __restrict__ start, int W, int H,
													   int* __restrict__ hist) {
	const int img = blockIdx.y;
	const int n = start[img + 1] - start[img];
	const int i = blockIdx.x * blockDim.x + threadIdx.x;
	if (i >= n) return;
	const KeyPoint kp = kps[(long long)img * cap + i];
	const int tx = min(KPT - 1, max(0, (int)(kp.x * KPT / W))), ty = min(KPT - 1, max(0, (int)(kp.y * KPT / H)));
	atomicAdd(&hist[img * (KPT * KPT) + ty * KPT + tx], 1);
}
__global__ __launch_bounds__(64) void k_kp_tile_scan(int* __restrict__ hist) {
	const int img = blockIdx.x, lane = threadIdx.x;
	const int c = hist[img * 64 + lane];
	int sc = c;
#pragma unroll
	for (int o = 1; o < 64; o <<= 1) {
		const int t = __shfl_up(sc, o, 64);
		if (lane >= o) sc += t;
	}
	hist[img * 64 + lane] = sc - c;
}
__global__ __launch_bounds__(256) void k_kp_tile_scatter(const KeyPoint* __restrict__ kps, int cap, const int* __restrict__ start, int W, int H,
														 int* __restrict__ cursor, int* __restrict__ perm) {
	const int img = blockIdx.y;
	const int s0 = start[img];
	const int n = start[img + 1] - s0;
	const int i = blockIdx.x * blockDim.x + threadIdx.x;
	if (i >= n) return;
	const KeyPoint kp = kps[(long long)img * cap + i];
	const int tx = min(KPT - 1, max(0, (int)(kp.x * KPT / W))), ty = min(KPT - 1, max(0, (int)(kp.y * KPT / H)));
	const int pos = atomicAdd(&cursor[img * (KPT * KPT) + ty * KPT + tx], 1);
	perm[s0 + pos] = s0 + i;
}

int bhip_launch_kp_spatial_order(bhip_ctx* ctx, const KeyPoint* kps, int cap, const int* start, int batch, int maxCount, int W, int H, int* hist ,
								 int* perm) {
	if (batch <= 0 || maxCount <= 0) return BHIP_OK;
	static_assert(KPT * KPT == 64, "k_kp_tile_scan assumes 64 tiles");
	BHIP_HIP(ctx, hipMemsetAsync(hist, 0, (size_t)batch * 64 * 4, ctx->stream));
	ProfScope ps(ctx, "k_kp_spatial_order", 0);
	dim3 grid((maxCount + 255) / 256, batch);
	hipLaunchKernelGGL(k_kp_tile_count, grid, dim3(256), 0, ctx->stream, kps, cap, start, W, H, hist);
	hipLaunchKernelGGL(k_kp_tile_scan, dim3(batch), dim3(64), 0, ctx->stream, hist);
	hipLaunchKernelGGL(k_kp_tile_scatter, grid, dim3(256), 0, ctx->stream, kps, cap, start, W, H, hist, perm);
	BHIP_HIP(ctx, hipGetLastError());
	return BHIP_OK;
}
```

Before: 15660 frames/s.

## Use persistent describe waves pulling keypoints from atomic work queues

The describe kernel now launches a grid sized to resident capacity. Each wave repeatedly takes the next keypoint slot from one of eight atomic counters, stealing from other chunks once its own runs dry, instead of handling exactly one keypoint per wave. The spatial permutation now stores image and local index alongside the global index, which removes the binary search over image starts. Shuffles become explicit ds_bpermute calls, and describe.hip is compiled with machine LICM disabled. The aim is to cut tail imbalance from uneven per-keypoint cost, at the price of per-item atomics and a queue memset.

```diff
diff --git a/boofcv_amd/build.py b/boofcv_amd/build.py
--- a/boofcv_amd/build.py
+++ b/boofcv_amd/build.py
@@ -11,6 +11,7 @@
 
 FLAGS = ["-O3", "-std=c++17", "-fPIC", "-ffp-contract=off", "-fhip-fp32-correctly-rounded-divide-sqrt", "-fno-fast-math",
          "-Wall", "-Wno-unused-function", "-Wno-unused-result"]
+SOURCE_FLAGS = {"describe.hip": ["-mllvm", "-disable-machine-licm"]}
 
 
 def sources():
@@ -48,7 +49,7 @@
         objs.append(obj)
         if not force and os.path.exists(obj) and os.path.getmtime(obj) > max(newest, os.path.getmtime(src)):
             continue
-        cmd = [hipcc, "--offload-arch=" + ARCH] + FLAGS + (["-DBHIP_EXPERIMENTS"] if experiments else []) + extra + ["-c", src, "-o", obj]
+        cmd = [hipcc, "--offload-arch=" + ARCH] + FLAGS + (["-DBHIP_EXPERIMENTS"] if experiments else []) + extra + SOURCE_FLAGS.get(os.path.basename(src), []) + ["-c", src, "-o", obj]
         if src.endswith(".cpp"):
             cmd.insert(1, "-x")
             cmd.insert(2, "hip")
diff --git a/boofcv_amd/csrc/cabi.h b/boofcv_amd/csrc/cabi.h
--- a/boofcv_amd/csrc/cabi.h
+++ b/boofcv_amd/csrc/cabi.h
@@ -19,6 +19,7 @@
 	int thresholdTapsRadius = 0;
 	AssocMfmaWork mfma;
 	int assocExactOnly = -1;
+	DevBuf describeQueue;
 };
 inline CtxScratch* scratchOf(bhip_ctx* ctx);
 
diff --git a/boofcv_amd/csrc/cabi.hip b/boofcv_amd/csrc/cabi.hip
--- a/boofcv_amd/csrc/cabi.hip
+++ b/boofcv_amd/csrc/cabi.hip
@@ -19,6 +19,7 @@
 	std::unique_ptr<bhip_ctx_full> ctx(new (std::nothrow) bhip_ctx_full());
 	if (!ctx) return BHIP_ERR_NOMEM;
 	ctx->device = device;
+	if (hipDeviceGetAttribute(&ctx->cuCount, hipDeviceAttributeMultiprocessorCount, device) != hipSuccess || ctx->cuCount <= 0) return BHIP_ERR_HIP;
 	if (useGiven) {
 		ctx->stream = (hipStream_t)stream;
 	} else {
@@ -445,7 +446,8 @@
 	BHIP_TRY(s->angBuf.reserve(ctx, (size_t)std::max<long long>(total, 1) * 8));
 	BHIP_TRY(s->descBuf.reserve(ctx, (size_t)std::max<long long>(total, 1) * 8 * dof));
 	BHIP_TRY(s->whiteBuf.reserve(ctx, (size_t)std::max<long long>(total, 1)));
-	const int* perm = nullptr;
+	const KpOrder* perm = nullptr;
+	BHIP_TRY(scratchOf(ctx)->describeQueue.reserve(ctx, BHIP_DESCRIBE_QUEUE_BYTES));
 	{
 #ifdef BHIP_EXPERIMENTS
 		const bool noOrder = bhip_env_flag("BHIP_DESCRIBE_NOORDER");
@@ -455,15 +457,16 @@
 		int maxCount = 0;
 		for (int c : s->det.counts) maxCount = std::max(maxCount, c);
 		if (!noOrder && total > 0) {
-			BHIP_TRY(s->permBuf.reserve(ctx, (size_t)total * 4 + (size_t)batch * 64 * 4));
-			int* hist = s->permBuf.as<int>() + total;
+			BHIP_TRY(s->permBuf.reserve(ctx, (size_t)total * sizeof(KpOrder) + (size_t)batch * 64 * 4));
+			int* hist = (int*)(s->permBuf.as<KpOrder>() + total);
 			BHIP_TRY(bhip_launch_kp_spatial_order(ctx, s->det.sorted.as<KeyPoint>(), s->det.cap, s->startBuf.as<int>(), batch, maxCount, W, H, hist,
-												  s->permBuf.as<int>()));
-			perm = s->permBuf.as<int>();
+												  s->permBuf.as<KpOrder>()));
+			perm = s->permBuf.as<KpOrder>();
 		}
 	}
 	BHIP_TRY(bhip_launch_describe_ex(ctx, ii, s->det.sorted.as<KeyPoint>(), s->det.cap, s->startBuf.as<int>(), 0, total, s->tables, nullptr,
-									 s->angBuf.as<double>(), s->descBuf.as<double>(), s->whiteBuf.as<uint8_t>(), perm, s->planar()));
+									 s->angBuf.as<double>(), s->descBuf.as<double>(), s->whiteBuf.as<uint8_t>(), perm, scratchOf(ctx)->describeQueue.as<int>(),
+									 s->planar()));
 	if (ret == SurfReturn::SYNCHRONIZED) BHIP_HIP(ctx, hipStreamSynchronize(ctx->stream));
 	s->haveResult = true;
 	return BHIP_OK;
@@ -936,10 +939,11 @@
 	BHIP_TRY(s->tmpAng.reserve(ctx, (size_t)n * 8));
 	BHIP_TRY(s->tmpDesc.reserve(ctx, (size_t)n * 8 * dof));
 	BHIP_TRY(s->tmpWhite.reserve(ctx, (size_t)n));
+	BHIP_TRY(scratchOf(ctx)->describeQueue.reserve(ctx, BHIP_DESCRIBE_QUEUE_BYTES));
 	BHIP_HIP(ctx, hipMemcpyAsync(s->tmpKp.p, kps.data(), (size_t)n * sizeof(KeyPoint), hipMemcpyHostToDevice, ctx->stream));
 	BHIP_TRY(withIntegral(s, [&](auto ii) {
 		return bhip_launch_describe_ex(ctx, ii, s->tmpKp.as<KeyPoint>(), 0, nullptr, image, n, s->tables, nullptr, s->tmpAng.as<double>(),
-									   s->tmpDesc.as<double>(), s->tmpWhite.as<uint8_t>(), nullptr, s->planar());
+									   s->tmpDesc.as<double>(), s->tmpWhite.as<uint8_t>(), nullptr, scratchOf(ctx)->describeQueue.as<int>(), s->planar());
 	}));
 	if (angle) BHIP_HIP(ctx, hipMemcpyAsync(angle, s->tmpAng.p, (size_t)n * 8, hipMemcpyDeviceToHost, ctx->stream));
 	if (white) BHIP_HIP(ctx, hipMemcpyAsync(white, s->tmpWhite.p, (size_t)n, hipMemcpyDeviceToHost, ctx->stream));
diff --git a/boofcv_amd/csrc/common.h b/boofcv_amd/csrc/common.h
--- a/boofcv_amd/csrc/common.h
+++ b/boofcv_amd/csrc/common.h
@@ -64,6 +64,7 @@
 	std::vector<ProfRecord> profRecords;
 	std::vector<HipEvent> eventPool;
 	size_t integralLdsAttr = 0;
+	int cuCount = 0;
 };
 
 struct ProfScope {
@@ -251,10 +252,14 @@
 							 const int* candCount, int cap, int batch, KeyPoint* sorted);
 int bhip_launch_word_prefix(bhip_ctx* ctx, const unsigned int* bitmap, int bitmapWords, int batch, unsigned int* wordPrefix, int* totals);
 
+struct __attribute__((aligned(16))) KpOrder { int g, img, local, pad; };
+#define BHIP_DESCRIBE_QUEUE_BYTES (8 * 128)
 template <class T>
 int bhip_launch_describe_ex(bhip_ctx* ctx, DevImg<const T> ii, const KeyPoint* kps, int cap, const int* imageStart, int singleImage, long long total,
-							SurfTables t, const double* anglesIn, double* angles, double* desc, uint8_t* white, const int* perm, DescPlanar planar);
-int bhip_launch_kp_spatial_order(bhip_ctx* ctx, const KeyPoint* kps, int cap, const int* start, int batch, int maxCount, int W, int H, int* hist, int* perm);
+							SurfTables t, const double* anglesIn, double* angles, double* desc, uint8_t* white, const KpOrder* perm, int* queue,
+							DescPlanar planar);
+int bhip_launch_kp_spatial_order(bhip_ctx* ctx, const KeyPoint* kps, int cap, const int* start, int batch, int maxCount, int W, int H, int* hist,
+								 KpOrder* perm);
 struct ColTop {
 	double min1, min2;
 	int idx1, pad;
diff --git a/boofcv_amd/csrc/describe.hip b/boofcv_amd/csrc/describe.hip
--- a/boofcv_amd/csrc/describe.hip
+++ b/boofcv_amd/csrc/describe.hip
@@ -15,7 +15,8 @@
 	double* angles;
 	double* desc;
 	uint8_t* white;
-	const int* perm;
+	const KpOrder* perm;
+	int* queue;
 	const float* bandData;
 	long long bandImageStride, bandStride;
 	int nBands;
@@ -27,6 +28,7 @@
 #ifdef BHIP_EXPERIMENTS
 	int stopAfter;
 	int windowStop;
+	int variant;
 #endif
 };
 
@@ -122,6 +124,23 @@
 	__builtin_amdgcn_fence(__ATOMIC_ACQUIRE, "wavefront");
 }
 
+template <class T>
+__device__ __forceinline__ T wavePermute(T v, int srcLane) {
+	static_assert(sizeof(T) == 4 || sizeof(T) == 8, "32- or 64-bit values");
+	const int addr = srcLane << 2;
+	if constexpr (sizeof(T) == 4) {
+		return __builtin_bit_cast(T, __builtin_amdgcn_ds_bpermute(addr, __builtin_bit_cast(int, v)));
+	} else {
+		const unsigned long long b = __builtin_bit_cast(unsigned long long, v);
+		const unsigned int lo = (unsigned int)__builtin_amdgcn_ds_bpermute(addr, (int)(unsigned int)b);
+		const unsigned int hi = (unsigned int)__builtin_amdgcn_ds_bpermute(addr, (int)(unsigned int)(b >> 32));
+		return __builtin_bit_cast(T, ((unsigned long long)hi << 32) | lo);
+	}
+}
+template <class T> __device__ __forceinline__ T laneShfl(T v, int src, int lane) { return wavePermute(v, (src & 63) | (lane & ~63)); }
+template <class T> __device__ __forceinline__ T laneShflXor(T v, int mask, int lane) { return wavePermute(v, lane ^ mask); }
+template <class T> __device__ __forceinline__ T laneShflUp(T v, int delta, int lane) { return wavePermute(v, lane >= delta ? lane - delta : lane); }
+
 struct OriSortOut {
 	double* dX; double* dY; double* sA;
 	float* sF;
@@ -370,7 +389,7 @@
 		mx = max(mx, cnt[e]);
 	}
 #pragma unroll
-	for (int o = 32; o >= 1; o >>= 1) mx = max(mx, __shfl_xor(mx, o, 64));
+	for (int o = 32; o >= 1; o >>= 1) mx = max(mx, laneShflXor(mx, o, lane));
 	if (mx > ORI_BIN_MAX) return false;
 	waveSync();
 	{
@@ -386,7 +405,7 @@
 		unsigned int sc = run;
 #pragma unroll
 		for (int o = 1; o < 64; o <<= 1) {
-			const unsigned int t = __shfl_up(sc, o, 64);
+			const unsigned int t = laneShflUp(sc, o, lane);
 			if (lane >= o) sc += t;
 		}
 		const unsigned int base = sc - run;
@@ -552,10 +571,10 @@
 	int scan = runMax;
 #pragma unroll
 	for (int o = 1; o < 64; o <<= 1) {
-		const int t = __shfl_up(scan, o, 64);
+		const int t = laneShflUp(scan, o, lane);
 		if (lane >= o) scan = max(scan, t);
 	}
-	int prevE = __shfl_up(scan, 1, 64);
+	int prevE = laneShflUp(scan, 1, lane);
 	if (lane == 0) prevE = 1;
 	prevE = max(prevE, 1);
 	int lastE = 1;
@@ -588,7 +607,7 @@
 		lastE = pe;
 	}
 	if (__any(abnormal)) return false;
-	lastE = __shfl(lastE, (n - 1) / EPL, 64);
+	lastE = laneShfl(lastE, (n - 1) / EPL, lane);
 	WSTAMP(9);
 	double vx[EPLT], vy[EPLT];
 	{
@@ -607,7 +626,7 @@
 		double ox = tx, oy = ty;
 #pragma unroll
 		for (int o = 1; o < 64; o <<= 1) {
-			const double ux = __shfl_up(ox, o, 64), uy = __shfl_up(oy, o, 64);
+			const double ux = laneShflUp(ox, o, lane), uy = laneShflUp(oy, o, lane);
 			if (lane >= o) { ox += ux; oy += uy; }
 		}
 		ox -= tx; oy -= ty;
@@ -643,7 +662,7 @@
 			unsigned int sc = run;
 #pragma unroll
 			for (int o = 1; o < 64; o <<= 1) {
-				const unsigned int t = __shfl_up(sc, o, 64);
+				const unsigned int t = laneShflUp(sc, o, lane);
 				if (lane >= o) sc += t;
 			}
 			const unsigned int base = sc - run;
@@ -671,14 +690,14 @@
 	WSTAMP(11);
 	double m = bMag;
 #pragma unroll
-	for (int o = 32; o >= 1; o >>= 1) m = fmax(m, __shfl_xor(m, o, 64));
+	for (int o = 32; o >= 1; o >>= 1) m = fmax(m, laneShflXor(m, o, lane));
 	int pos = (bMag == m) ? bPos : 0x7fffffff;
 #pragma unroll
-	for (int o = 32; o >= 1; o >>= 1) pos = min(pos, __shfl_xor(pos, o, 64));
+	for (int o = 32; o >= 1; o >>= 1) pos = min(pos, laneShflXor(pos, o, lane));
 	const unsigned long long owner = __ballot(bMag == m && bPos == pos);
 	const int src = __ffsll((long long)owner) - 1;
-	bestX = __shfl(bX, src, 64);
-	bestY = __shfl(bY, src, 64);
+	bestX = laneShfl(bX, src, lane);
+	bestY = laneShfl(bY, src, lane);
 	const double tieFloor = m - m * 1.0e-9;
 	if (__popcll(__ballot(bMag >= tieFloor)) + __popcll(__ballot(bMag2 >= tieFloor)) > 1) {
 		waveSync();
@@ -699,39 +718,52 @@
 #define DSTAMP(i) do { if (STAMP && lane == 0) P.stamps[g * 16 + (i)] = __builtin_readcyclecounter(); } while (0)
 #endif
 
-template <bool STAMP, int EPLT, int TWT, class TAP, int CFG = 0>
-__global__ __launch_bounds__(256) void k_describe(DescParams P) {
-	extern __shared__ __attribute__((aligned(16))) unsigned char ldsAll[];
-	const int wave = __builtin_amdgcn_readfirstlane((int)(threadIdx.x >> 6));
-	const int lane = threadIdx.x & 63;
-	const long long nblk = (P.total + 3) >> 2;
-	const long long chunk = (nblk + 7) >> 3;
-	const long long blk = (long long)(blockIdx.x & 7) * chunk + (blockIdx.x >> 3);
-	if ((long long)(blockIdx.x >> 3) >= chunk) return;
-	const long long slot = blk * 4 + wave;
-	if (slot >= P.total) return;
-	const long long g = P.perm ? (long long)P.perm[slot] : slot;
-	unsigned char* lds = ldsAll + (size_t)wave * P.ldsPerWave;
-
-	int img, local;
-	if (P.imageStart) {
-		int lo = 0, hi = P.batch;
-		while (hi - lo > 1) {
-			const int m = (lo + hi) >> 1;
-			if ((long long)P.imageStart[m] <= g) lo = m; else hi = m;
-		}
-		img = lo;
-		local = (int)(g - P.imageStart[img]);
+#define DESC_VAR_ONESHOT 1
+#define DESC_VAR_SEARCH 2
+__device__ __forceinline__ bool queueNext(const DescParams& P, int lane, int& cur, int& tried, long long& slot) {
+	const long long chunkSlots = ((((P.total + 3) >> 2) + 7) >> 3) * 4;
+	while (tried < 8) {
+		int t = 0;
+		if (lane == 0) t = __hip_atomic_fetch_add(P.queue + cur * 32, 1, __ATOMIC_RELAXED, __HIP_MEMORY_SCOPE_AGENT);
+		t = __builtin_amdgcn_readfirstlane(t);
+		const long long len = P.total - cur * chunkSlots;
+		if (t < chunkSlots && t < len) { slot = cur * chunkSlots + t; return true; }
+		tried++;
+		cur = (cur + 1) & 7;
+	}
+	return false;
+}
+__device__ __forceinline__ void loadSlot(const DescParams& P, long long slot, int variant, long long& g, int& img, KeyPoint& kp) {
+	int local;
+	if (P.perm && !(variant & DESC_VAR_SEARCH)) {
+		const KpOrder r = P.perm[slot];
+		g = r.g; img = r.img; local = r.local;
 	} else {
-		img = P.singleImage;
-		local = (int)g;
+		g = P.perm ? (long long)P.perm[slot].g : slot;
+		if (P.imageStart) {
+			int lo = 0, hi = P.batch;
+			while (hi - lo > 1) {
+				const int m = (lo + hi) >> 1;
+				if ((long long)P.imageStart[m] <= g) lo = m; else hi = m;
+			}
+			img = lo;
+			local = (int)(g - P.imageStart[img]);
+		} else {
+			img = P.singleImage;
+			local = (int)g;
+		}
 	}
 	img = (int)uniformU32((unsigned)img);
 	local = (int)uniformU32((unsigned)local);
-	const KeyPoint kp = P.imageStart ? P.kps[(long long)img * P.cap + local] : P.kps[local];
+	kp = P.imageStart ? P.kps[(long long)img * P.cap + local] : P.kps[local];
+}
+
+template <bool STAMP, int EPLT, int TWT, class TAP, int CFG>
+__device__ __forceinline__ void describeOne(const DescParams& P, const long long g, const int img, const KeyPoint kp, unsigned char* lds, const int lane) {
 	const TAP* __restrict__ d = (const TAP*)P.ii.data + (long long)img * P.ii.imageStride;
 	const int stride = P.ii.stride, W = P.ii.width, H = P.ii.height;
-	const SurfTables& T = P.t;
+	SurfTables T = P.t;
+	asm volatile("" : "+s"(T.oriRadius), "+s"(T.oriKernelWidth), "+s"(T.widthSample), "+s"(T.oriWindow));
 
 	DSTAMP(0);
 	double angle;
@@ -852,8 +884,8 @@
 						start++;
 					}
 				}
-				bestX = __shfl(bestX, 0, 64);
-				bestY = __shfl(bestY, 0, 64);
+				bestX = laneShfl(bestX, 0, lane);
+				bestY = laneShfl(bestY, 0, lane);
 			}
 			angle = atan2(bestY, bestX);
 			dirX = bestX; dirY = bestY;
@@ -862,8 +894,8 @@
 			if (lane == 0) {
 				for (int i = 0; i < n; i++) { Dx += dX[i]; Dy += dY[i]; }
 			}
-			Dx = __shfl(Dx, 0, 64);
-			Dy = __shfl(Dy, 0, 64);
+			Dx = laneShfl(Dx, 0, lane);
+			Dy = laneShfl(Dy, 0, lane);
 			angle = atan2(Dy, Dx);
 			dirX = Dx; dirY = Dy;
 		}
@@ -1005,7 +1037,7 @@
 		}
 #pragma unroll
 		for (int o = 1; o <= 2; o <<= 1) {
-			a0 += __shfl_xor(a0, o, 64); a1 += __shfl_xor(a1, o, 64); a2 += __shfl_xor(a2, o, 64); a3 += __shfl_xor(a3, o, 64);
+			a0 += laneShflXor(a0, o, lane); a1 += laneShflXor(a1, o, lane); a2 += laneShflXor(a2, o, lane); a3 += laneShflXor(a3, o, lane);
 		}
 		double sum = q == 0 ? a0 : q == 1 ? a1 : q == 2 ? a2 : a3;
 		if (stableDesc) sum = T.weightGrid[sub] * sum;
@@ -1051,7 +1083,7 @@
 	double norm = 0;
 	for (int f = lane; f < dofAll; f += 64) { const double v = feat[f]; norm += v * v; }
 #pragma unroll
-	for (int o = 32; o >= 1; o >>= 1) norm += __shfl_xor(norm, o, 64);
+	for (int o = 32; o >= 1; o >>= 1) norm += laneShflXor(norm, o, lane);
 	double* out = P.desc + g * dofAll;
 	if (norm == 0) {
 		for (int f = lane; f < dofAll; f += 64) out[f] = feat[f];
@@ -1063,7 +1095,7 @@
 		TAP bs[4];
 #pragma unroll
 		for (int b = 0; b < 4; b++) {
-			const TAP br = __shfl(lapTap, 4 * b, 64), tr = __shfl(lapTap, 4 * b + 1, 64), bl = __shfl(lapTap, 4 * b + 2, 64), tl = __shfl(lapTap, 4 * b + 3, 64);
+			const TAP br = laneShfl(lapTap, 4 * b, lane), tr = laneShfl(lapTap, 4 * b + 1, lane), bl = laneShfl(lapTap, 4 * b + 2, lane), tl = laneShfl(lapTap, 4 * b + 3, lane);
 			bs[b] = br - tr - bl + tl;
 		}
 		TAP xx = 0;
@@ -1077,6 +1109,46 @@
 		if (lane == 0) P.white[g] = lap > 0 ? 1 : 0;
 	}
 	DSTAMP(6);
+}
+
+template <bool STAMP, int EPLT, int TWT, class TAP, int CFG = 0>
+__global__ __launch_bounds__(256) void k_describe(DescParams P) {
+	extern __shared__ __attribute__((aligned(16))) unsigned char ldsAll[];
+	const int wave = __builtin_amdgcn_readfirstlane((int)(threadIdx.x >> 6));
+	const int lane0 = threadIdx.x & 63;
+	unsigned char* lds = ldsAll + (size_t)wave * P.ldsPerWave;
+#ifdef BHIP_EXPERIMENTS
+	const int variant = P.variant;
+#else
+	constexpr int variant = 0;
+#endif
+	unsigned long long waveStart = STAMP ? __builtin_readcyclecounter() : 0;
+	int cur = blockIdx.x & 7, tried = 0;
+	long long slot = 0;
+	if (variant & DESC_VAR_ONESHOT) {
+		const long long nblk = (P.total + 3) >> 2;
+		const long long chunk = (nblk + 7) >> 3;
+		const long long blk = (long long)(blockIdx.x & 7) * chunk + (blockIdx.x >> 3);
+		if ((long long)(blockIdx.x >> 3) >= chunk) return;
+		slot = blk * 4 + wave;
+		if (slot >= P.total) return;
+	} else if (!queueNext(P, lane0, cur, tried, slot)) {
+		return;
+	}
+	for (;;) {
+		int lane = lane0;
+		asm volatile("" : "+v"(lane));
+		long long g;
+		int img;
+		KeyPoint kp;
+		loadSlot(P, slot, variant, g, img, kp);
+		if (STAMP && lane == 0) P.stamps[g * 16 + 7] = waveStart;
+		describeOne<STAMP, EPLT, TWT, TAP, CFG>(P, g, img, kp, lds, lane);
+		if (variant & DESC_VAR_ONESHOT) break;
+		if (STAMP) waveStart = __builtin_readcyclecounter();
+		if (!queueNext(P, lane, cur, tried, slot)) break;
+		waveSync();
+	}
 }
 
 static int bhip_describe_default_cfg(const SurfTables& t) {
@@ -1098,13 +1170,63 @@
 	return (b + 15) & ~15;
 }
 
+static unsigned bhip_describe_grid(bhip_ctx* ctx, const void* fn, size_t ldsBytes, long long blocks, const DescParams& P) {
+#ifdef BHIP_EXPERIMENTS
+	if (P.variant & DESC_VAR_ONESHOT) return (unsigned)blocks;
+#endif
+	int perCU = 0;
+	if (hipOccupancyMaxActiveBlocksPerMultiprocessor(&perCU, fn, 256, ldsBytes) != hipSuccess || perCU <= 0) { (void)hipGetLastError(); return 0; }
+	return (unsigned)std::min<long long>(blocks, (long long)perCU * ctx->cuCount);
+}
+
+#ifdef BHIP_EXPERIMENTS
+static void bhip_describe_stamp_queue_summary(FILE* f, const std::vector<unsigned long long>& h, const std::vector<KpOrder>& hp, long long total, int variant,
+											  int batch) {
+	double chain = 0, life = 0;
+	long long cnt = 0;
+	for (long long k = 0; k < total; k++) {
+		const unsigned long long* tt = &h[(size_t)k * 16];
+		if (!tt[6] || !tt[0] || !tt[7]) continue;
+		chain += (double)(tt[0] - tt[7]); life += (double)(tt[6] - tt[7]); cnt++;
+	}
+	if (!cnt) return;
+	fprintf(f, "batch %d  key points %lld  variant bits %d  avg cycles: wave start (or end of the previous key point) to stamp 0 %.0f  key point in all %.0f\n", batch, total,
+			variant, chain / cnt, life / cnt);
+	if (!(variant & DESC_VAR_ONESHOT)) return;
+	double ratio = 0, parked = 0, held = 0;
+	long long groups = 0;
+	for (long long s0 = 0; s0 < total; s0 += 4) {
+		unsigned long long first = ~0ull, last = 0;
+		double lifeMax = 0, lifeSum = 0, endSum = 0;
+		int n = 0;
+		for (long long s = s0; s < std::min(total, s0 + 4); s++) {
+			const long long g = hp.empty() ? s : hp[(size_t)s].g;
+			const unsigned long long* tt = &h[(size_t)g * 16];
+			if (!tt[6] || !tt[7]) continue;
+			first = std::min(first, tt[7]); last = std::max(last, tt[6]);
+			const double l = (double)(tt[6] - tt[7]);
+			lifeMax = std::max(lifeMax, l); lifeSum += l; endSum += (double)tt[6];
+			n++;
+		}
+		if (n < 4) continue;
+		ratio += lifeMax / (lifeSum / n);
+		parked += n * (double)last - endSum;
+		held += n * (double)(last - first);
+		groups++;
+	}
+	if (groups) fprintf(f, "   workgroups %lld  mean of max(life)/mean(life) %.3f  parked share of the held wave slots %.1f %%\n", groups, ratio / groups, 100.0 * parked / held);
+}
+#endif
+
 template <class T>
 int bhip_launch_describe_ex(bhip_ctx* ctx, DevImg<const T> ii, const KeyPoint* kps, int cap, const int* imageStart, int singleImage, long long total,
-							SurfTables t, const double* anglesIn, double* angles, double* desc, uint8_t* white, const int* perm, DescPlanar planar) {
+							SurfTables t, const double* anglesIn, double* angles, double* desc, uint8_t* white, const KpOrder* perm, int* queue,
+							DescPlanar planar) {
 	if (total <= 0) return BHIP_OK;
+	if (!queue || ctx->cuCount <= 0) return bhip_fail(ctx, BHIP_ERR_INVALID, "describe: no slot counters");
 	DescParams P;
 	P.ii = bhip_kernel_view(ii); P.kps = kps; P.cap = cap; P.imageStart = imageStart; P.batch = ii.batch; P.singleImage = singleImage; P.total = total; P.t = t;
-	P.anglesIn = anglesIn; P.angles = angles; P.desc = desc; P.white = white; P.perm = perm;
+	P.anglesIn = anglesIn; P.angles = angles; P.desc = desc; P.white = white; P.perm = perm; P.queue = queue;
 	P.bandData = nullptr; P.bandImageStride = P.bandStride = 0; P.nBands = 0;
 	if (planar.nBands > 0) {
 		if (!planar.data) return bhip_fail(ctx, BHIP_ERR_INVALID, "bad planar description request");
@@ -1118,12 +1240,20 @@
 #ifdef BHIP_EXPERIMENTS
 	{ const char* e = getenv("BHIP_DESCRIBE_STOP"); P.stopAfter = e ? atoi(e) : -1; }
 	{ const char* e = getenv("BHIP_DESCRIBE_WSTOP"); P.windowStop = e ? atoi(e) : -1; }
+	{
+		const char* e = getenv("BHIP_DESCRIBE_VARIANT");
+		const char v = e ? e[0] : 0;
+		P.variant = v == 'w' ? (DESC_VAR_ONESHOT | DESC_VAR_SEARCH) : v == 'i' ? DESC_VAR_ONESHOT : 0;
+		const char* sp = getenv("BHIP_DESCRIBE_SPLIT");
+		if (sp && (sp[0] == '1' || sp[0] == '2')) P.variant |= DESC_VAR_ONESHOT;
+	}
 #endif
 	if (t.oriWidth * t.oriWidth > 64 * ORI_EPL_MAX) return bhip_fail(ctx, BHIP_ERR_UNSUPPORTED, "orientation sample grid too large for the GPU path");
 	if (t.widthSubRegion + 2 * (t.stable ? t.overLap : 0) > DESC_ROW_MAX) return bhip_fail(ctx, BHIP_ERR_UNSUPPORTED, "SURF sub-region too wide for the GPU path");
 	if (P.ldsPerWave * 4 > 160 * 1024) return bhip_fail(ctx, BHIP_ERR_UNSUPPORTED, "orientation/descriptor sample grid too large for LDS");
 	const long long blocks = ((((total + 3) / 4) + 7) / 8) * 8;
 	if (blocks > 0x7fffffffLL) return bhip_fail(ctx, BHIP_ERR_INVALID, "too many key points");
+	BHIP_HIP(ctx, hipMemsetAsync(queue, 0, BHIP_DESCRIBE_QUEUE_BYTES, ctx->stream));
 	if ((long long)ii.stride * ii.height > 0x3fffffffLL || ii.stride >= (1 << 17)) return bhip_fail(ctx, BHIP_ERR_UNSUPPORTED, "integral image too large for 32-bit tap offsets");
 #ifdef BHIP_EXPERIMENTS
 	const char* stampPath = getenv("BHIP_DESCRIBE_STAMPS");
@@ -1133,13 +1263,14 @@
 			(void)hipMemsetAsync(dev, 0, (size_t)total * 128, ctx->stream);
 			P.stamps = dev;
 			{
-				const int epl = (t.oriWidth * t.oriWidth + 63) / 64;
-				const int tw = t.widthSubRegion + 2 * (t.stable ? t.overLap : 0);
-				if (bhip_describe_default_cfg(t) == 1) hipLaunchKernelGGL((k_describe<true, 5, 9, float, 1>), dim3((unsigned)blocks), dim3(256), (size_t)P.ldsPerWave * 4, ctx->stream, P);
-				else hipLaunchKernelGGL((k_describe<true, 8, 16, float>), dim3((unsigned)blocks), dim3(256), (size_t)P.ldsPerWave * 4, ctx->stream, P);
+				const void* sfn = bhip_describe_default_cfg(t) == 1 ? (const void*)k_describe<true, 5, 9, float, 1> : (const void*)k_describe<true, 8, 16, float>;
+				void* sargs[] = {(void*)&P};
+				(void)hipLaunchKernel(sfn, dim3(bhip_describe_grid(ctx, sfn, (size_t)P.ldsPerWave * 4, blocks, P)), dim3(256), sargs, (size_t)P.ldsPerWave * 4, ctx->stream);
 			}
 			std::vector<unsigned long long> h((size_t)total * 16);
+			std::vector<KpOrder> hp(P.perm ? (size_t)total : 0);
 			(void)hipMemcpyAsync(h.data(), dev, (size_t)total * 128, hipMemcpyDeviceToHost, ctx->stream);
+			if (P.perm) (void)hipMemcpyAsync(hp.data(), P.perm, (size_t)total * sizeof(KpOrder), hipMemcpyDeviceToHost, ctx->stream);
 			(void)hipStreamSynchronize(ctx->stream);
 			(void)hipFree(dev);
 			double sum[7] = {0}, wsum[6] = {0};
@@ -1152,6 +1283,7 @@
 				cnt++;
 			}
 			FILE* f = fopen(stampPath, "a");
+			if (f) bhip_describe_stamp_queue_summary(f, h, hp, total, P.variant, ii.batch);
 			if (f && cnt) {
 				fprintf(f, "waves %lld  avg cycles: samples %.0f  sort %.0f  window+atan2 %.0f  descSamples %.0f  sums %.0f  norm+laplace %.0f\n", cnt,
 						sum[1] / cnt, sum[2] / cnt, sum[3] / cnt, sum[4] / cnt, sum[5] / cnt, sum[6] / cnt);
@@ -1171,7 +1303,7 @@
 		ProfScope ps(ctx, "k_describe", perKp * (double)total);
 		const int epl = (t.oriWidth * t.oriWidth + 63) / 64;
 		const int tw = t.widthSubRegion + 2 * (t.stable ? t.overLap : 0);
-		const dim3 grid((unsigned)blocks), block(256);
+		const dim3 block(256);
 		size_t ldsBytes = (size_t)P.ldsPerWave * 4;
 #ifdef BHIP_EXPERIMENTS
 		{ const char* e = getenv("BHIP_DESCRIBE_LDSPAD"); if (e) ldsBytes += (size_t)atoi(e); }
@@ -1186,6 +1318,8 @@
 		else fn = ints ? (const void*)k_describe<false, 8, 16, int> : (const void*)k_describe<false, 8, 16, float>;
 		if (ldsBytes > 65536) BHIP_HIP(ctx, hipFuncSetAttribute(fn, hipFuncAttributeMaxDynamicSharedMemorySize, (int)ldsBytes));
 		void* args[] = {(void*)&P};
+		const dim3 grid(bhip_describe_grid(ctx, fn, ldsBytes, blocks, P));
+		if (grid.x == 0) return bhip_fail(ctx, BHIP_ERR_HIP, "k_describe: no workgroup fits a compute unit");
 #ifdef BHIP_EXPERIMENTS
 		{
 			const char* e = getenv("BHIP_DESCRIBE_SPLIT");
@@ -1226,5 +1360,5 @@
 	BHIP_HIP(ctx, hipGetLastError());
 	return BHIP_OK;
 }
-template int bhip_launch_describe_ex(bhip_ctx*, DevImg<const float>, const KeyPoint*, int, const int*, int, long long, SurfTables, const double*, double*, double*,  uint8_t*, const int*, DescPlanar);
-template int bhip_launch_describe_ex(bhip_ctx*, DevImg<const int32_t>, const KeyPoint*, int, const int*, int, long long, SurfTables, const double*, double*, double*,  uint8_t*, const int*, DescPlanar);
+template int bhip_launch_describe_ex(bhip_ctx*, DevImg<const float>, const KeyPoint*, int, const int*, int, long long, SurfTables, const double*, double*, double*,  uint8_t*, const KpOrder*, int*, DescPlanar);
+template int bhip_launch_describe_ex(bhip_ctx*, DevImg<const int32_t>, const KeyPoint*, int, const int*, int, long long, SurfTables, const double*, double*, double*,  uint8_t*, const KpOrder*, int*, DescPlanar);
diff --git a/boofcv_amd/csrc/detect.hip b/boofcv_amd/csrc/detect.hip
--- a/boofcv_amd/csrc/detect.hip
+++ b/boofcv_amd/csrc/detect.hip
@@ -759,7 +759,7 @@
 	hist[img * 64 + lane] = sc - c;
 }
 __global__ __launch_bounds__(256) void k_kp_tile_scatter(const KeyPoint* __restrict__ kps, int cap, const int* __restrict__ start, int W, int H,
-														 int* __restrict__ cursor, int* __restrict__ perm) {
+														 int* __restrict__ cursor, KpOrder* __restrict__ perm) {
 	const int img = blockIdx.y;
 	const int s0 = start[img];
 	const int n = start[img + 1] - s0;
@@ -768,11 +768,11 @@
 	const KeyPoint kp = kps[(long long)img * cap + i];
 	const int tx = min(KPT - 1, max(0, (int)(kp.x * KPT / W))), ty = min(KPT - 1, max(0, (int)(kp.y * KPT / H)));
 	const int pos = atomicAdd(&cursor[img * (KPT * KPT) + ty * KPT + tx], 1);
-	perm[s0 + pos] = s0 + i;
+	perm[s0 + pos] = KpOrder{s0 + i, img, i, 0};
 }
 
 int bhip_launch_kp_spatial_order(bhip_ctx* ctx, const KeyPoint* kps, int cap, const int* start, int batch, int maxCount, int W, int H, int* hist ,
-								 int* perm) {
+								 KpOrder* perm) {
 	if (batch <= 0 || maxCount <= 0) return BHIP_OK;
 	static_assert(KPT * KPT == 64, "k_kp_tile_scan assumes 64 tiles");
 	BHIP_HIP(ctx, hipMemsetAsync(hist, 0, (size_t)batch * 64 * 4, ctx->stream));
```

Result: faster. 16000 frames/s (median of 6 runs) (+2.1%).
